# syzhang092218-source/dgppo

Hardware: AMD Instinct MI355X
Metric: env-steps/sec whole node, LidarSpread n=8 4096 envs, 1/2/4/8 GPUs (higher is better)
Workload: dtype f32

## Files before the change

dgppo_amd/csrc/gae.hip:

```cpp
#include "common.h"

__device__ inline float nanmax(float a, float b) { return (a != a || b != b) ? __builtin_nanf("") : fmaxf(a, b); }

struct GaeArgs {
  const float* costs; const float* rewards; const float* Vh; const float* Vl;
  const float* lam_pow;
  float* Qh; float* Ql;
  int B, T, AH;
  int n, nh;
  float gamma, one_minus_gamma, one_minus_lam;
};

__global__ void gae_kernel(GaeArgs a) {
  extern __shared__ float sm[];
  const int b = blockIdx.x, tid = threadIdx.x, nt = blockDim.x;
  const int T = a.T, AH = a.AH, n = a.n, nh = a.nh;
  float* rowH = sm;
  float* rowL = rowH + (T + 1) * AH;
  float* hcur = rowL + (T + 1);
  float* hdis = hcur + AH;
  const float* costs = a.costs + (size_t)b * T * AH;
  const float* Vh = a.Vh + (size_t)b * (T + 1) * AH;
  const float* Vl = a.Vl + (size_t)b * (T + 1);
  const float* rew = a.rewards + (size_t)b * T;
  for (int i = tid; i < (T + 1) * AH; i += nt) rowH[i] = 0.0f;
  for (int i = tid; i < T + 1; i += nt) rowL[i] = 0.0f;
  __syncthreads();
  for (int i = tid; i < AH; i += nt) rowH[i] = Vh[(size_t)T * AH + i];
  if (tid == 0) rowL[0] = Vl[T];
  __syncthreads();
  for (int ii = 0; ii < T; ++ii) {
    const int t = T - 1 - ii;
    for (int i = tid; i < AH; i += nt) hcur[i] = costs[(size_t)t * AH + i];
    __syncthreads();
    for (int ag = tid; ag < n; ag += nt) {
      float m = hcur[ag * nh];
      for (int h = 1; h < nh; ++h) m = nanmax(m, hcur[ag * nh + h]);
      for (int h = 0; h < nh; ++h) hdis[ag * nh + h] = a.one_minus_gamma * m;
    }
    __syncthreads();
    const float l = -rew[t];
    for (int idx = tid; idx < (ii + 1) * AH; idx += nt) {
      const int c = idx % AH;
      rowH[idx] = nanmax(hcur[c], hdis[c] + a.gamma * rowH[idx]);
    }
    for (int j = tid; j <= ii; j += nt) rowL[j] = l + a.gamma * rowL[j];
    __syncthreads();
    for (int c = tid; c < AH + 1; c += nt) {
      float acc = 0.0f;
      if (c < AH) {
        for (int j = 0; j <= ii; ++j) {
          const float cj = (j == 0) ? a.lam_pow[ii] : a.lam_pow[ii - j] * a.one_minus_lam;
          acc = fmaf(cj, rowH[j * AH + c], acc);
        }
        a.Qh[((size_t)b * T + t) * AH + c] = acc;
      } else {
        for (int j = 0; j <= ii; ++j) {
          const float cj = (j == 0) ? a.lam_pow[ii] : a.lam_pow[ii - j] * a.one_minus_lam;
          acc = fmaf(cj, rowL[j], acc);
        }
        a.Ql[(size_t)b * T + t] = acc;
      }
    }
    __syncthreads();
    for (int i = tid; i < AH; i += nt) rowH[(ii + 1) * AH + i] = Vh[(size_t)t * AH + i];
    if (tid == 0) rowL[ii + 1] = Vl[t];
    __syncthreads();
  }
}


__device__ inline float gae_row16_sum(float v) {
  v += __int_as_float(__builtin_amdgcn_update_dpp(0, __float_as_int(v), 0xB1, 0xf, 0xf, false));
  v += __int_as_float(__builtin_amdgcn_update_dpp(0, __float_as_int(v), 0x4E, 0xf, 0xf, false));
  v += __int_as_float(__builtin_amdgcn_update_dpp(0, __float_as_int(v), 0x141, 0xf, 0xf, false));
  v += __int_as_float(__builtin_amdgcn_update_dpp(0, __float_as_int(v), 0x140, 0xf, 0xf, false));
  return v;
}

template <int AHP>
__global__ void __launch_bounds__(256) gae_rows_kernel(GaeArgs a) {
  extern __shared__ float sm[];
  const int b = blockIdx.x, tid = threadIdx.x, lane = tid & 63;
  const int T = a.T, AH = a.AH, nh = a.nh;
  float* s_cost = sm;
  float* s_Vh = s_cost + T * AH;
  float* s_Vl = s_Vh + (T + 1) * AH;
  float* s_rew = s_Vl + (T + 1);
  float* s_part = s_rew + T;
  const float* costs = a.costs + (size_t)b * T * AH;
  const float* Vh = a.Vh + (size_t)b * (T + 1) * AH;
  for (int i = tid; i < T * AH; i += 256) s_cost[i] = costs[i];
  for (int i = tid; i < (T + 1) * AH; i += 256) s_Vh[i] = Vh[i];
  for (int i = tid; i < T + 1; i += 256) s_Vl[i] = a.Vl[(size_t)b * (T + 1) + i];
  for (int i = tid; i < T; i += 256) s_rew[i] = a.rewards[(size_t)b * T + i];
  __syncthreads();
  const int j = tid;
  float row[AHP];
  float rowl = 0.0f;
#pragma unroll
  for (int c = 0; c < AHP; ++c) row[c] = (j == 0 && c < AH) ? s_Vh[T * AH + c] : 0.0f;
  if (j == 0) rowl = s_Vl[T];
  for (int ii = 0; ii < T; ++ii) {
    const int t = T - 1 - ii;
    const bool act = j <= ii;
    float contrib[AHP];
    float cl = 0.0f;
    const float cj = (j == 0) ? a.lam_pow[ii] : ((j <= ii) ? a.lam_pow[ii - j] * a.one_minus_lam : 0.0f);
    if (act) {
      const float l = -s_rew[t];
      rowl = l + a.gamma * rowl;
      cl = cj * rowl;
    }
#pragma unroll
    for (int ag = 0; ag < AHP; ag += 1) {
      if (ag < AH) {
        const int agent = ag / nh;
        float m = s_cost[t * AH + agent * nh];
        for (int h = 1; h < nh; ++h) m = nanmax(m, s_cost[t * AH + agent * nh + h]);
        if (act) row[ag] = nanmax(s_cost[t * AH + ag], a.one_minus_gamma * m + a.gamma * row[ag]);
        contrib[ag] = act ? cj * row[ag] : 0.0f;
      } else {
        contrib[ag] = 0.0f;
      }
    }
#pragma unroll
    for (int c = 0; c < AHP; ++c) contrib[c] = gae_row16_sum(contrib[c]);
    cl = gae_row16_sum(cl);
    float* part = s_part + (ii & 1) * 16 * (AHP + 1);
    if ((lane & 15) == 0) {
      float* dst = part + (tid >> 4) * (AHP + 1);
#pragma unroll
      for (int c = 0; c < AHP; ++c) dst[c] = contrib[c];
      dst[AHP] = cl;
    }
    if (j == ii + 1) {
#pragma unroll
      for (int c = 0; c < AHP; ++c) row[c] = (c < AH) ? s_Vh[t * AH + c] : 0.0f;
      rowl = s_Vl[t];
    }
    __syncthreads();
    if (tid <= AH) {
      const int c = (tid < AH) ? tid : AHP;
      float q = 0.0f;
#pragma unroll
      for (int rw = 0; rw < 16; ++rw) q += part[rw * (AHP + 1) + c];
      if (tid < AH) a.Qh[((size_t)b * T + t) * AH + tid] = q;
      else a.Ql[(size_t)b * T + t] = q;
    }
  }
}

template <int NRG> __device__ inline float rg_sum(float v) {
  v += __int_as_float(__builtin_amdgcn_update_dpp(0, __float_as_int(v), 0xB1, 0xf, 0xf, false));
  v += __int_as_float(__builtin_amdgcn_update_dpp(0, __float_as_int(v), 0x4E, 0xf, 0xf, false));
  if (NRG == 8) v += __int_as_float(__builtin_amdgcn_update_dpp(0, __float_as_int(v), 0x141, 0xf, 0xf, false));
  return v;
}

template <int RPG, int NRG>
__global__ void __launch_bounds__(256) gae_cols_kernel(GaeArgs a) {
  const int T = a.T, AH = a.AH, nh = a.nh, C = AH + 1;
  const int rg = threadIdx.x % NRG;
  const long item = (long)blockIdx.x * (256 / NRG) + threadIdx.x / NRG;
  const bool valid = item < (long)a.B * C;
  const long it = valid ? item : 0;
  const int b = (int)(it / C), col = (int)(it - (long)b * C);
  const bool is_l = (col == AH);
  const int agent = is_l ? 0 : col / nh;
  const float* costs = a.costs + (size_t)b * T * AH + agent * nh;
  const float* vser = is_l ? a.Vl + (size_t)b * (T + 1) : a.Vh + (size_t)b * (T + 1) * AH + col;
  const int vstr = is_l ? 1 : AH;
  const float* rew = a.rewards + (size_t)b * T;
  const float lam = a.lam_pow[1], inv_lam = 1.0f / lam;
  float w[RPG];
  {
    float p = a.one_minus_lam;
#pragma unroll
    for (int r = 0; r < RPG; ++r) { w[r] = p; p *= inv_lam; }
    if (rg == 0) w[0] = 1.0f;
  }
  float row[RPG];
#pragma unroll
  for (int r = 0; r < RPG; ++r) row[r] = 0.0f;
  const float vT = vser[(size_t)T * vstr];
  if (rg == 0) row[0] = vT;
  float f = 1.0f;
  auto fetch = [&](int t, float& lo, float& k, float& vt) {
    vt = vser[(size_t)t * vstr];
    if (is_l) { lo = -INFINITY; k = -rew[t]; }
    else {
      const float* ct = costs + (size_t)t * AH;
      float m = ct[0];
      for (int h = 1; h < nh; ++h) m = nanmax(m, ct[h]);
      lo = ct[col - agent * nh];
      k = a.one_minus_gamma * m;
    }
  };
  float lo, k, vt;
  fetch(T - 1, lo, k, vt);
  bool poison = vT != vT;
  const int nchunk = (T + RPG - 1) / RPG;
  for (int chunk = 0; chunk < nchunk; ++chunk) {
    const bool g_le = rg <= chunk, g_lt = rg < chunk;
#pragma unroll
    for (int s = 0; s < RPG; ++s) {
      const int ii = chunk * RPG + s;
      if (ii < T) {
        const int t = T - 1 - ii;
        float lo_n = 0.0f, k_n = 0.0f, vt_n = 0.0f;
        if (t > 0) fetch(t - 1, lo_n, k_n, vt_n);
        float q = 0.0f;
#pragma unroll
        for (int r = 0; r < RPG; ++r) {
          const bool act = (r <= s) ? g_le : g_lt;
          const float nv = fmaxf(lo, fmaf(a.gamma, row[r], k));
          row[r] = act ? nv : row[r];
          q = fmaf(w[r], row[r], q);
        }
        poison = poison || (lo != lo) || (k != k);
        float tot = rg_sum<NRG>(q * f);
        tot = poison ? __builtin_nanf("") : tot;
        if (valid && rg == 0) {
          if (is_l) a.Ql[(size_t)b * T + t] = tot;
          else a.Qh[((size_t)b * T + t) * AH + col] = tot;
        }
        poison = poison || (vt != vt);
        if (g_le) f *= lam;
        const int rn = (s + 1) % RPG;
        const bool mine = rg == chunk + ((s + 1) / RPG);
#pragma unroll
        for (int r = 0; r < RPG; ++r)
          if (r == rn) row[r] = mine ? vt : row[r];
        lo = lo_n; k = k_n; vt = vt_n;
      }
    }
  }
}

template <int RPG, int NRG>
static void launch_gae_cols(const GaeArgs& a, hipStream_t st) {
  const long items = (long)a.B * (a.AH + 1);
  const int per_block = 256 / NRG;
  hipLaunchKernelGGL((gae_cols_kernel<RPG, NRG>), dim3((unsigned)((items + per_block - 1) / per_block)), dim3(256), 0, st, a);
}

extern "C" int32_t dgppo_gae(const float* costs, const float* rewards, const float* Vh, const float* Vl,
                             const float* lam_pow, float gamma, float one_minus_gamma, float one_minus_lam, float* Qh,
                             float* Ql, int32_t B, int32_t T, int32_t n, int32_t nh, void* stream) {
  DGPPO_REQUIRE(B >= 0 && T >= 1 && n >= 1 && nh >= 1, "gae: bad sizes");
  if (B == 0) return 0;
  DGPPO_REQUIRE(costs && rewards && Vh && Vl && lam_pow && Qh && Ql, "gae: NULL operand");
  GaeArgs a{costs, rewards, Vh, Vl, lam_pow, Qh, Ql, B, T, n * nh, n, nh, gamma, one_minus_gamma, one_minus_lam};
  if (T <= 256 && one_minus_lam <= 0.5f && one_minus_lam >= 0.0f) {
    hipStream_t st = (hipStream_t)stream;
    if (T <= 32) launch_gae_cols<8, 4>(a, st);
    else if (T <= 64) launch_gae_cols<16, 4>(a, st);
    else if (T <= 128) launch_gae_cols<32, 4>(a, st);
    else launch_gae_cols<32, 8>(a, st);
    DGPPO_LAUNCH_CHECK();
    return 0;
  }
  if (T + 1 <= 256 && a.AH <= 32) {
    const int ahp = a.AH <= 8 ? 8 : (a.AH <= 16 ? 16 : 32);
    const size_t fsm = sizeof(float) * ((size_t)T * a.AH + (size_t)(T + 1) * a.AH + (T + 1) + T + 2 * 16 * (ahp + 1));
    if (fsm <= 64 * 1024) {
      hipStream_t st = (hipStream_t)stream;
      if (ahp == 8) hipLaunchKernelGGL(gae_rows_kernel<8>, dim3(B), dim3(256), fsm, st, a);
      else if (ahp == 16) hipLaunchKernelGGL(gae_rows_kernel<16>, dim3(B), dim3(256), fsm, st, a);
      else hipLaunchKernelGGL(gae_rows_kernel<32>, dim3(B), dim3(256), fsm, st, a);
      DGPPO_LAUNCH_CHECK();
      return 0;
    }
  }
  const size_t smem = sizeof(float) * ((size_t)(T + 1) * a.AH + (T + 1) + 2 * a.AH);
  DGPPO_REQUIRE(smem <= 150 * 1024, "gae: T*n*nh too large for LDS (%zu B)", smem);
  if (smem > 64 * 1024)
    (void)hipFuncSetAttribute((const void*)gae_kernel, hipFuncAttributeMaxDynamicSharedMemorySize, (int)smem);
  hipLaunchKernelGGL(gae_kernel, dim3(B), dim3(256), smem, (hipStream_t)stream, a);
  DGPPO_LAUNCH_CHECK();
  return 0;
}

struct AdvArgs {
  const float* Ql; const float* Vl; const float* Vh;
  float* adv;
  float* stats;
  int B, T, n, nh;
  float inv_dt, alpha, cbf_eps, cbf_weight;
};

__global__ void adv_kernel(AdvArgs a) {
  __shared__ float red[256];
  __shared__ float s_mean, s_std;
  const int b = blockIdx.x, tid = threadIdx.x, nt = blockDim.x;
  const int T = a.T, n = a.n, nh = a.nh;
  const float* Ql = a.Ql + (size_t)b * T;
  const float* Vl = a.Vl + (size_t)b * (T + 1);
  const float* Vh = a.Vh ? a.Vh + (size_t)b * (T + 1) * n * nh : nullptr;
  float acc = 0.0f;
  for (int t = tid; t < T; t += nt) acc += Ql[t] - Vl[t];
  red[tid] = acc;
  __syncthreads();
  for (int o = nt / 2; o > 0; o >>= 1) { if (tid < o) red[tid] += red[tid + o]; __syncthreads(); }
  if (tid == 0) s_mean = red[0] / (float)T;
  __syncthreads();
  const float mean = s_mean;
  acc = 0.0f;
  for (int t = tid; t < T; t += nt) { const float d = (Ql[t] - Vl[t]) - mean; acc += d * d; }
  red[tid] = acc;
  __syncthreads();
  for (int o = nt / 2; o > 0; o >>= 1) { if (tid < o) red[tid] += red[tid + o]; __syncthreads(); }
  if (tid == 0) s_std = sqrtf(red[0] / (float)T);
  __syncthreads();
  const float denom = s_std + 1e-8f;
  float nsafe = 0.0f;
  for (int idx = tid; idx < T * n; idx += nt) {
    const int t = idx / n, ag = idx - t * n;
    const float al = ((Ql[t] - Vl[t]) - mean) / denom;
    bool safe = true;
    float amax = 0.0f;
    for (int h = 0; a.Vh != nullptr && h < nh; ++h) {
      const float v0 = Vh[((size_t)t * n + ag) * nh + h], v1 = Vh[((size_t)(t + 1) * n + ag) * nh + h];
      const float deriv = (v1 - v0) * a.inv_dt + a.alpha * v0;
      const float ac = nanmax(deriv + a.cbf_eps, 0.0f);
      amax = (h == 0) ? ac : nanmax(amax, ac);
      safe = safe && (deriv <= 0.0f);
    }
    const float A = (safe ? al : 0.0f) + amax * a.cbf_weight;
    a.adv[(size_t)b * T * n + idx] = -A;
    nsafe += safe ? 1.0f : 0.0f;
  }
  red[tid] = nsafe;
  __syncthreads();
  for (int o = nt / 2; o > 0; o >>= 1) { if (tid < o) red[tid] += red[tid + o]; __syncthreads(); }
  if (tid == 0) atomicAdd(a.stats, red[0]);
}

extern "C" int32_t dgppo_advantage(const float* Ql, const float* Vl, const float* Vh, float dt, float alpha,
                                   float cbf_eps, float cbf_weight, float* adv, float* stats, int32_t B, int32_t T,
                                   int32_t n, int32_t nh, void* stream) {
  DGPPO_REQUIRE(B >= 0 && T >= 1 && n >= 1 && nh >= 1, "advantage: bad sizes");
  if (B == 0) return 0;
  DGPPO_REQUIRE(Ql && Vl && adv && stats, "advantage: NULL operand");
  AdvArgs a{Ql, Vl, Vh, adv, stats, B, T, n, nh, 1.0f / dt, alpha, cbf_eps, cbf_weight};
  hipLaunchKernelGGL(adv_kernel, dim3(B), dim3(256), 0, (hipStream_t)stream, a);
  DGPPO_LAUNCH_CHECK();
  return 0;
}

__global__ void shaped_reward_kernel(const float* __restrict__ reward, const float* __restrict__ cost, float w,
                                     float* __restrict__ out, long rows, int n, int nh) {
  const long r = (long)blockIdx.x * blockDim.x + threadIdx.x;
  if (r >= rows) return;
  const float* c = cost + r * n * nh;
  float tot = 0.0f;
  for (int i = 0; i < n; ++i) {
    float si = 0.0f;
    for (int h = 0; h < nh; ++h) si += nanmax(c[i * nh + h], 0.0f);
    tot += si;
  }
  out[r] = reward[r] - w * tot;
}

extern "C" int32_t dgppo_shaped_reward(const float* reward, const float* cost, float cost_weight, float* out, int64_t rows,
                                       int32_t n, int32_t nh, void* stream) {
  DGPPO_REQUIRE(rows >= 0 && n >= 1 && nh >= 1, "shaped_reward: bad sizes");
  if (rows == 0) return 0;
  DGPPO_REQUIRE(reward && cost && out, "shaped_reward: NULL operand");
  hipLaunchKernelGGL(shaped_reward_kernel, dim3((unsigned)((rows + 255) / 256)), dim3(256), 0, (hipStream_t)stream, reward,
                     cost, cost_weight, out, (long)rows, n, nh);
  DGPPO_LAUNCH_CHECK();
  return 0;
}

struct AdvLagrArgs {
  const float* Ql; const float* Vl; const float* Qh; const float* Vh; const float* lagr;
  float* adv;
  float* Ah;
  int B, T, n, nh;
};

#define ADV_LAGR_MAX_COLS 192
__global__ void __launch_bounds__(256) adv_lagr_kernel(AdvLagrArgs a) {
  __shared__ float red[256];
  __shared__ float s_mean[1 + ADV_LAGR_MAX_COLS], s_den[1 + ADV_LAGR_MAX_COLS];
  const int b = blockIdx.x, tid = threadIdx.x, nt = blockDim.x;
  const int T = a.T, n = a.n, nh = a.nh, AH = n * nh;
  const float* Ql = a.Ql + (size_t)b * T;
  const float* Vl = a.Vl + (size_t)b * (T + 1);
  const float* Qh = a.Qh + (size_t)b * T * AH;
  const float* Vh = a.Vh + (size_t)b * (T + 1) * AH;
  for (int s0 = 0; s0 < 1 + AH; ++s0) {
    float acc = 0.0f;
    for (int t = tid; t < T; t += nt) acc += (s0 == 0) ? (Ql[t] - Vl[t]) : (Qh[(size_t)t * AH + s0 - 1] - Vh[(size_t)t * AH + s0 - 1]);
    red[tid] = acc;
    __syncthreads();
    for (int o = nt / 2; o > 0; o >>= 1) { if (tid < o) red[tid] += red[tid + o]; __syncthreads(); }
    const float mean = red[0] / (float)T;
    __syncthreads();
    acc = 0.0f;
    for (int t = tid; t < T; t += nt) {
      const float d = ((s0 == 0) ? (Ql[t] - Vl[t]) : (Qh[(size_t)t * AH + s0 - 1] - Vh[(size_t)t * AH + s0 - 1])) - mean;
      acc += d * d;
    }
    red[tid] = acc;
    __syncthreads();
    for (int o = nt / 2; o > 0; o >>= 1) { if (tid < o) red[tid] += red[tid + o]; __syncthreads(); }
    if (tid == 0) { s_mean[s0] = mean; s_den[s0] = sqrtf(red[0] / (float)T) + 1e-8f; }
    __syncthreads();
  }
  for (int idx = tid; idx < T * n; idx += nt) {
    const int t = idx / n, ag = idx - t * n;
    const float al = -(((Ql[t] - Vl[t]) - s_mean[0]) / s_den[0]);
    float acc = 0.0f;
    for (int h = 0; h < nh; ++h) {
      const int c = ag * nh + h;
      const float ah = ((Qh[(size_t)t * AH + c] - Vh[(size_t)t * AH + c]) - s_mean[1 + c]) / s_den[1 + c];
      a.Ah[((size_t)b * T + t) * AH + c] = ah;
      acc += ah * a.lagr[c];
    }
    a.adv[(size_t)b * T * n + idx] = al - acc / (float)nh;
  }
}

extern "C" int32_t dgppo_advantage_lagr(const float* Ql, const float* Vl, const float* Qh, const float* Vh,
                                        const float* lagr, float* adv, float* Ah, int32_t B, int32_t T, int32_t n,
                                        int32_t nh, void* stream) {
  DGPPO_REQUIRE(B >= 0 && T >= 1 && n >= 1 && nh >= 1 && (long)n * nh <= ADV_LAGR_MAX_COLS,
                "advantage_lagr: bad sizes (n * nh <= 192)");
  if (B == 0) return 0;
  DGPPO_REQUIRE(Ql && Vl && Qh && Vh && lagr && adv && Ah, "advantage_lagr: NULL operand");
  AdvLagrArgs a{Ql, Vl, Qh, Vh, lagr, adv, Ah, B, T, n, nh};
  hipLaunchKernelGGL(adv_lagr_kernel, dim3(B), dim3(256), 0, (hipStream_t)stream, a);
  DGPPO_LAUNCH_CHECK();
  return 0;
}

__global__ void __launch_bounds__(256) lagr_sum_kernel(const float* __restrict__ lp_new, const float* __restrict__ lp_old,
                                                       const float* __restrict__ Vh, const float* __restrict__ Ah,
                                                       float* __restrict__ sums, long rows, int n, int nh, int T,
                                                       long vh_env_stride, float one_minus_gamma) {
  extern __shared__ float s_acc[];
  for (int c = threadIdx.x; c < n * nh; c += blockDim.x) s_acc[c] = 0.0f;
  __syncthreads();
  for (long r = (long)blockIdx.x * blockDim.x + threadIdx.x; r < rows; r += (long)gridDim.x * blockDim.x) {
    const int ag = (int)(r % n);
    const long bt = r / n, e = bt / T, t = bt - e * T;
    const float ratio = expf(lp_new[r] - lp_old[r]);
    for (int h = 0; h < nh; ++h) {
      const float vh = Vh[e * vh_env_stride + (t * n + ag) * nh + h];
      atomicAdd(&s_acc[ag * nh + h], vh * one_minus_gamma + ratio * Ah[r * nh + h]);
    }
  }
  __syncthreads();
  for (int c = threadIdx.x; c < n * nh; c += blockDim.x) atomicAdd(&sums[c], s_acc[c]);
}

__global__ void lagr_apply_kernel(float* __restrict__ lagr, float* __restrict__ sums, int count, float inv_bt, float lr) {
  const int c = blockIdx.x * blockDim.x + threadIdx.x;
  if (c >= count) return;
  const float delta = -(sums[c] * inv_bt);
  lagr[c] = fmaxf(lagr[c] - delta * lr, 0.0f);
  sums[c] = 0.0f;
}

extern "C" int32_t dgppo_lagr_update(const float* lp_new, const float* lp_old, const float* Vh, int64_t vh_env_stride,
                                     const float* Ah, float* lagr, float* sums, int32_t n_env, int32_t T, int32_t n,
                                     int32_t nh, float one_minus_gamma, float lr, void* stream) {
  DGPPO_REQUIRE(n_env >= 1 && T >= 1 && n >= 1 && nh >= 1 && n * nh <= 1024, "lagr_update: bad sizes");
  DGPPO_REQUIRE(lp_new && lp_old && Vh && Ah && lagr && sums, "lagr_update: NULL operand");
  const long rows = (long)n_env * T * n;
  const int grid = (int)((rows + 255) / 256 < 512 ? (rows + 255) / 256 : 512);
  hipLaunchKernelGGL(lagr_sum_kernel, dim3(grid), dim3(256), sizeof(float) * n * nh, (hipStream_t)stream, lp_new, lp_old, Vh,
                     Ah, sums, rows, n, nh, T, (long)vh_env_stride, one_minus_gamma);
  hipLaunchKernelGGL(lagr_apply_kernel, dim3((n * nh + 63) / 64), dim3(64), 0, (hipStream_t)stream, lagr, sums, n * nh,
                     1.0f / (float)((long)n_env * T), lr);
  DGPPO_LAUNCH_CHECK();
  return 0;
}

extern "C" int32_t dgppo_lagr_sums(const float* lp_new, const float* lp_old, const float* Vh, int64_t vh_env_stride,
                                   const float* Ah, float* sums, int32_t n_env, int32_t T, int32_t n, int32_t nh,
                                   float one_minus_gamma, void* stream) {
  DGPPO_REQUIRE(n_env >= 1 && T >= 1 && n >= 1 && nh >= 1 && n * nh <= 1024, "lagr_sums: bad sizes");
  DGPPO_REQUIRE(lp_new && lp_old && Vh && Ah && sums, "lagr_sums: NULL operand");
  const long rows = (long)n_env * T * n;
  const int grid = (int)((rows + 255) / 256 < 512 ? (rows + 255) / 256 : 512);
  hipLaunchKernelGGL(lagr_sum_kernel, dim3(grid), dim3(256), sizeof(float) * n * nh, (hipStream_t)stream, lp_new, lp_old, Vh,
                     Ah, sums, rows, n, nh, T, (long)vh_env_stride, one_minus_gamma);
  DGPPO_LAUNCH_CHECK();
  return 0;
}

extern "C" int32_t dgppo_lagr_apply(float* lagr, float* sums, int32_t count, int64_t rows_total, float lr, void* stream) {
  DGPPO_REQUIRE(count >= 1 && count <= 1024 && rows_total >= 1, "lagr_apply: bad sizes");
  DGPPO_REQUIRE(lagr && sums, "lagr_apply: NULL operand");
  hipLaunchKernelGGL(lagr_apply_kernel, dim3((count + 63) / 64), dim3(64), 0, (hipStream_t)stream, lagr, sums, count,
                     1.0f / (float)rows_total, lr);
  DGPPO_LAUNCH_CHECK();
  return 0;
}

__global__ void relu_fwd_kernel(const float* __restrict__ x, float* __restrict__ out, long count) {
  const long i = (long)blockIdx.x * blockDim.x + threadIdx.x;
  if (i < count) out[i] = nanmax(x[i], 0.0f);
}

extern "C" int32_t dgppo_relu_fwd(const float* x, float* out, int64_t count, void* stream) {
  DGPPO_REQUIRE(count >= 0, "relu_fwd: count < 0");
  if (count == 0) return 0;
  DGPPO_REQUIRE(x && out, "relu_fwd: NULL operand");
  hipLaunchKernelGGL(relu_fwd_kernel, dim3((unsigned)((count + 255) / 256)), dim3(256), 0, (hipStream_t)stream, x, out,
                     (long)count);
  DGPPO_LAUNCH_CHECK();
  return 0;
}
```

dgppo_amd/csrc/graph_feats.hip:

```cpp
#include "graph_topo.h"

struct FeatArgs {
  dgppo_env_cfg cfg;
  Topo t;
  const float* agent; long agent_se, agent_st;
  const float* goal;
  const float* obst;
  const float* hits; long hits_se, hits_st;
  const int32_t* env_ids;
  int n_env, n_time;
  float* Xa;
  float* Xo;
  float* efeat;
  float* emask;
  int Fp;
  int vecX, vecM;
  uint32_t rcp_fp, rcp_fq, rcp_S;
};

#define GF_PF 8
#define GF_WAVE_SYNC()                                  \
  do {                                                  \
    __builtin_amdgcn_fence(__ATOMIC_SEQ_CST, "wavefront"); \
    __builtin_amdgcn_wave_barrier();                    \
  } while (0)

struct FeatRec { const float *ag, *go, *ob; };

template <int SD>
__device__ inline float4 feat4(const float* s) {
  if constexpr (SD == 5) {
    float vx = __fmul_rn(s[4], s[2]), vy = __fmul_rn(s[4], s[3]);
    asm volatile("" : "+v"(vx), "+v"(vy));
    return make_float4(s[0], s[1], vx, vy);
  } else {
    return make_float4(s[0], s[1], s[2], s[3]);
  }
}

template <int SD>
__global__ void __launch_bounds__(256) graph_feats_kernel(FeatArgs a) {
  extern __shared__ float sm[];
  const dgppo_env_cfg& c = a.cfg;
  const Topo& t = a.t;
  const int lane = threadIdx.x & 63;
  const int wv = __builtin_amdgcn_readfirstlane(threadIdx.x >> 6), wpb = blockDim.x >> 6;
  const int n = t.n, ng = t.ng, S = t.S, Fp = a.Fp;
  const int n_on = t.Ns - n - ng;
  const int nA = n * SD, nG = ng * SD, nO = n_on * (t.lidar ? 2 : SD), R = nA + nG + nO;
  float* s_ag = sm + (size_t)wv * R;
  float* s_go = s_ag + nA;
  float* s_ob = s_go + nG;
  const long G = (long)a.n_env * a.n_time, stride = (long)gridDim.x * wpb;
  long g = (long)blockIdx.x * wpb + wv;
  if (g >= G) return;
  auto env_of = [&](long gg) { const int e = (int)gg / a.n_time; return a.env_ids ? (int)a.env_ids[e] : e; };
  auto locate = [&](long gg, int env) {
    const int tt = (int)gg % a.n_time;
    FeatRec p;
    p.ag = a.agent + (size_t)env * a.agent_se + (size_t)tt * a.agent_st;
    p.go = a.goal + (size_t)env * nG;
    p.ob = nullptr;
    if (nO > 0) p.ob = t.lidar ? a.hits + (size_t)env * a.hits_se + (size_t)tt * a.hits_st : a.obst + (size_t)env * nO;
    return p;
  };
  auto fetch = [&](const FeatRec& p, int i) { return i < nA ? p.ag[i] : (i < nA + nG ? p.go[i - nA] : p.ob[i - nA - nG]); };
  float r0, r1, r2, r3, r4, r5, r6, r7;
  static_assert(GF_PF == 8, "one register per prefetched dword");
#define GF_EACH(OP) OP(r0, 0) OP(r1, 1) OP(r2, 2) OP(r3, 3) OP(r4, 4) OP(r5, 5) OP(r6, 6) OP(r7, 7)
#define GF_REQUEST(r, j) { const int i = lane + 64 * j; r = 0.0f; if (i < R) r = fetch(p, i); }
#define GF_COMMIT(r, j)  { const int i = lane + 64 * j; if (i < R) s_ag[i] = r; }
  FeatRec p = locate(g, env_of(g));
  GF_EACH(GF_REQUEST)
  long gn = g + stride;
  int env_n = gn < G ? env_of(gn) : 0;
  for (;;) {
    GF_EACH(GF_COMMIT)
    for (int i = GF_PF * 64 + lane; i < R; i += 64) s_ag[i] = fetch(p, i);
    GF_WAVE_SYNC();
    const bool more = gn < G;
    if (more) {
      p = locate(gn, env_n);
      GF_EACH(GF_REQUEST)
      if (gn + stride < G) env_n = env_of(gn + stride);
    }
    auto node_src = [&](int nd, const float*& src, int& ns, int& one) {
      if (nd < n) { src = s_ag + nd * SD; ns = SD; one = SD + 2; }
      else if (nd < n + ng) { src = s_go + (nd - n) * SD; ns = SD; one = SD + 1; }
      else if (t.lidar) { src = s_ob + (nd - n - ng) * 2; ns = 2; one = SD; }
      else { src = s_ob + (nd - n - ng) * SD; ns = SD; one = SD; }
    };
    if (a.vecX) {
      const int Fq = Fp >> 2;
      for (int q = lane; q < t.Ns * Fq; q += 64) {
        const int nd = (int)__umulhi((uint32_t)q, a.rcp_fq), col0 = (q - nd * Fq) * 4;
        const float* src; int ns, one;
        node_src(nd, src, ns, one);
        float v[4];
#pragma unroll
        for (int k = 0; k < 4; ++k) {
          const int col = col0 + k;
          v[k] = (col < ns) ? src[col] : ((col == one) ? 1.0f : 0.0f);
        }
        float* dst = (nd < n) ? a.Xa + ((size_t)g * n + nd) * Fp + col0 : a.Xo + ((size_t)g * (t.Ns - n) + (nd - n)) * Fp + col0;
        *reinterpret_cast<float4*>(dst) = make_float4(v[0], v[1], v[2], v[3]);
      }
    } else {
      for (int idx = lane; idx < t.Ns * Fp; idx += 64) {
        const int nd = (int)__umulhi((uint32_t)idx, a.rcp_fp), col = idx - nd * Fp;
        const float* src; int ns, one;
        node_src(nd, src, ns, one);
        const float v = (col < ns) ? src[col] : ((col == one) ? 1.0f : 0.0f);
        if (nd < n) a.Xa[((size_t)g * n + nd) * Fp + col] = v;
        else a.Xo[((size_t)g * (t.Ns - n) + (nd - n)) * Fp + col] = v;
      }
    }
    const int nE = n * S;
    for (int base = 0; base < nE; base += 64) {
      const int idx = base + lane;
      bool mask = false;
      if (idx < nE) {
        const int i = (int)__umulhi((uint32_t)idx, a.rcp_S), s = idx - i * S;
        float4 f;
        const float4 fi = feat4<SD>(s_ag + i * SD);
        const float px = s_ag[i * SD], py = s_ag[i * SD + 1];
        if (s < n) {
          const float4 fj = feat4<SD>(s_ag + s * SD);
          f = make_float4(__fsub_rn(fi.x, fj.x), __fsub_rn(fi.y, fj.y), __fsub_rn(fi.z, fj.z), __fsub_rn(fi.w, fj.w));
          float d = __fadd_rn(dist_rn(__fsub_rn(px, s_ag[s * SD]), __fsub_rn(py, s_ag[s * SD + 1])), (i == s) ? c.eye_offset : 0.0f);
          mask = d < c.comm_radius;
        } else if (s < n + t.gs) {
          const int gi = t.spread ? (s - n) : i;
          const float4 fg = feat4<SD>(s_go + gi * SD);
          f = make_float4(__fsub_rn(fi.x, fg.x), __fsub_rn(fi.y, fg.y), __fsub_rn(fi.z, fg.z), __fsub_rn(fi.w, fg.w));
          mask = true;
        } else {
          const int m = s - n - t.gs;
          if (t.lidar) {
            const float* hp = s_ob + (i * t.per + m) * 2;
            const float lx = __fsub_rn(px, hp[0]), ly = __fsub_rn(py, hp[1]);
            f = make_float4(lx, ly, 0.0f, 0.0f);
            mask = dist_rn(lx, ly) < c.lidar_mask_radius;
          } else {
            const float* xo = s_ob + m * SD;
            const float* xi = s_ag + i * SD;
            f = make_float4(__fsub_rn(xi[0], xo[0]), __fsub_rn(xi[1], xo[1]), __fsub_rn(xi[2], xo[2]), __fsub_rn(xi[3], xo[3]));
            mask = dist_rn(__fsub_rn(xi[0], xo[0]), __fsub_rn(xi[1], xo[1])) < c.obs_mask_radius;
          }
        }
        reinterpret_cast<float4*>(a.efeat)[(size_t)g * nE + idx] = f;
        if (!a.vecM) a.emask[(size_t)g * nE + idx] = mask ? 1.0f : 0.0f;
      }
      if (a.vecM) {
        const unsigned long long bits = __ballot(mask);
        const int i4 = base + 4 * lane;
        if (lane < 16 && i4 < nE) {
          const unsigned b = (unsigned)(bits >> (4 * lane));
          *reinterpret_cast<float4*>(a.emask + (size_t)g * nE + i4) =
              make_float4((b & 1u) ? 1.0f : 0.0f, (b & 2u) ? 1.0f : 0.0f, (b & 4u) ? 1.0f : 0.0f, (b & 8u) ? 1.0f : 0.0f);
        }
      }
    }
    GF_WAVE_SYNC();
    if (!more) break;
    g = gn;
    gn += stride;
  }
#undef GF_EACH
#undef GF_REQUEST
#undef GF_COMMIT
}

static int feats_grid_cap(const void* fn, int wpb, size_t smem) {
  static thread_local const void* k_fn = nullptr;
  static thread_local int k_wpb = 0, k_cap = 0;
  static thread_local size_t k_smem = 0;
  if (fn == k_fn && wpb == k_wpb && smem == k_smem) return k_cap;
  int per_cu = 0, dev = 0, cus = 256;
  if (hipOccupancyMaxActiveBlocksPerMultiprocessor(&per_cu, fn, 64 * wpb, smem) != hipSuccess || per_cu < 1) per_cu = 1;
  if (hipGetDevice(&dev) != hipSuccess ||
      hipDeviceGetAttribute(&cus, hipDeviceAttributeMultiprocessorCount, dev) != hipSuccess || cus < 1) cus = 256;
  k_fn = fn; k_wpb = wpb; k_smem = smem; k_cap = per_cu * cus;
  return k_cap;
}

extern "C" int32_t dgppo_graph_feats(const dgppo_env_cfg* cfg, const float* agent, int64_t agent_se, int64_t agent_st,
                                     const float* goal, const float* obst, const float* hits, int64_t hits_se,
                                     int64_t hits_st, const int32_t* env_ids, int32_t n_env, int32_t n_time, float* Xa,
                                     float* Xo, float* efeat, float* emask, int32_t Fp, void* stream) {
  int32_t rc = dgppo_validate_cfg(cfg);
  if (rc) return rc;
  DGPPO_REFUSE_VMAS(cfg, "dgppo_graph_feats", "dgppo_vmas_graph_feats");
  DGPPO_REQUIRE(n_env >= 0 && n_time >= 0, "graph_feats: negative counts");
  if (n_env == 0 || n_time == 0) return 0;
  DGPPO_REQUIRE(agent && goal && Xa && efeat && emask, "graph_feats: NULL operand");
  DGPPO_REQUIRE(Fp >= cfg->node_dim && Fp <= 32, "graph_feats: Fp must be in [node_dim, 32]");
  FeatArgs a;
  a.cfg = *cfg; a.t = make_topo(*cfg);
  const int n_on = a.t.Ns - a.t.n - a.t.ng;
  DGPPO_REQUIRE(n_on == 0 || Xo, "graph_feats: Xo is NULL");
  DGPPO_REQUIRE(a.t.Ns == a.t.n || Xo, "graph_feats: Xo is NULL");
  if (n_on > 0) {
    if (a.t.lidar) DGPPO_REQUIRE(hits, "graph_feats: hits is NULL");
    else DGPPO_REQUIRE(obst, "graph_feats: obst is NULL");
  }
  DGPPO_REQUIRE(((uintptr_t)efeat & 15) == 0, "graph_feats: efeat must be 16-byte aligned");
  a.agent = agent; a.agent_se = agent_se; a.agent_st = agent_st; a.goal = goal; a.obst = obst;
  a.hits = hits; a.hits_se = hits_se; a.hits_st = hits_st; a.env_ids = env_ids; a.n_env = n_env; a.n_time = n_time;
  a.Xa = Xa; a.Xo = Xo; a.efeat = efeat; a.emask = emask; a.Fp = Fp;
  a.rcp_fp = (uint32_t)((0x100000000ull + (uint64_t)Fp - 1) / (uint64_t)Fp);
  a.rcp_S = (uint32_t)((0x100000000ull + (uint64_t)a.t.S - 1) / (uint64_t)a.t.S);
  DGPPO_REQUIRE(Fp >= 2 && a.t.S >= 2 && (long)a.t.Ns * Fp < 65536 && (long)a.t.n * a.t.S < 65536, "graph_feats: sizes out of range");
  a.vecX = (Fp % 4 == 0 && ((uintptr_t)Xa & 15) == 0 && ((uintptr_t)Xo & 15) == 0) ? 1 : 0;
  a.vecM = ((a.t.n * a.t.S) % 4 == 0 && ((uintptr_t)emask & 15) == 0) ? 1 : 0;
  a.rcp_fq = a.vecX ? (uint32_t)((0x100000000ull + (uint64_t)(Fp / 4) - 1) / (uint64_t)(Fp / 4)) : 0u;
  const int SD = cfg->state_dim;
  const size_t rec = sizeof(float) * ((size_t)a.t.n * SD + (size_t)a.t.ng * SD + (size_t)n_on * (a.t.lidar ? 2 : SD));
  int wpb = 4;
  while (wpb > 1 && rec * wpb > 65536) wpb >>= 1;
  const long G = (long)n_env * n_time;
  const void* fn = SD == 5 ? reinterpret_cast<const void*>(&graph_feats_kernel<5>) : reinterpret_cast<const void*>(&graph_feats_kernel<4>);
  const int cap = feats_grid_cap(fn, wpb, rec * wpb);
  const long wgs = (G + wpb - 1) / wpb;
  const dim3 grid((unsigned)(wgs < cap ? wgs : cap)), block(64 * wpb);
  if (SD == 5) hipLaunchKernelGGL(graph_feats_kernel<5>, grid, block, rec * wpb, (hipStream_t)stream, a);
  else hipLaunchKernelGGL(graph_feats_kernel<4>, grid, block, rec * wpb, (hipStream_t)stream, a);
  DGPPO_LAUNCH_CHECK();
  return 0;
}
```

dgppo_amd/engine.py:

```python
from __future__ import annotations

import dataclasses
from typing import Callable, Dict, Optional

import numpy as np
import os
import torch

from . import _native as N
from . import nets
from . import ops_algo as OA
from . import ops_env as OE
from . import ops_nn as K
from .utils import checkpoint as CK


@dataclasses.dataclass
class Hyper:
    gamma: float = 0.99
    gae_lambda: float = 0.95
    clip_eps: float = 0.25
    coef_ent: float = 1e-2
    max_grad_norm: float = 2.0
    lr_actor: float = 3e-4
    lr_Vl: float = 1e-3
    lr_Vh: float = 1e-3
    batch_size: int = 16384
    rnn_step: int = 16
    alpha: float = 10.0
    cbf_eps: float = 1e-2
    cbf_weight: float = 1.0
    cbf_schedule: bool = True
    train_steps: int = 100000
    actor_gnn_layers: int = 2
    Vl_gnn_layers: int = 2
    Vh_gnn_layers: int = 1
    use_rnn: bool = True
    use_lstm: bool = False
    rnn_layers: int = 1
    lagr_init: float = 0.78
    lr_lagr: float = 1e-7
    cost_weight: float = 0.0
    cost_schedule: bool = False


class RolloutData:

    def __init__(self, cfg: N.EnvCfg, B: int, T: int, device, stochastic: bool, carry_dim: int = nets.HID):
        n = cfg.n_agents
        self.cfg, self.B, self.T, self.stochastic = cfg, B, T, stochastic
        z = lambda *s: torch.empty(*s, device=device)
        step, env = OE.record_fields(cfg)
        self.step_tm = {k: z(T + 1, B, *shape) for k, shape in step.items()}
        self.env = {k: z(B, *shape) for k, shape in env.items()}
        self.step: Dict[str, torch.Tensor] = {}
        for k in OE.STEP_FIELDS:
            setattr(self, k + "_tm", self.step_tm.get(k))
            setattr(self, k, None)
        for k in OE.ENV_FIELDS:
            setattr(self, k, self.env.get(k))
        self.action_tm = z(T, B, n, 2)
        self.log_pi_tm = z(T, B, n) if stochastic else None
        self.rnn_tm = z(T + 1, B, n, carry_dim)
        self.reward_tm = z(T, B)
        self.cost_tm = z(T, B, n, cfg.n_cost)
        self._env_major = False
        views = {k: v.unbind(0) for k, v in self.step_tm.items()}
        self.states_tm = [OE.State({k: v[t] for k, v in views.items()}, self.env) for t in range(T + 1)]

    def finalize(self):
        if self._env_major:
            return self

        def tr(name, x):
            if x is None:
                return None
            cur = getattr(self, name, None)
            want = (x.shape[1], x.shape[0]) + tuple(x.shape[2:])
            if cur is None or tuple(cur.shape) != want:
                cur = torch.empty(want, device=x.device, dtype=x.dtype)
            cur.copy_(x.transpose(0, 1))
            return cur
        for k, v in self.step_tm.items():
            self.step[k] = tr(k, v)
            setattr(self, k, self.step[k])
        self.actions = tr("actions", self.action_tm)
        self.log_pis = tr("log_pis", self.log_pi_tm) if self.stochastic else None
        T, x = self.T, self.rnn_tm
        want = (x.shape[1], T + 2) + tuple(x.shape[2:])
        cur = getattr(self, "_rnn_em", None)
        if cur is None or tuple(cur.shape) != want:
            cur = torch.empty(want, device=x.device, dtype=x.dtype)
        cur[:, :T + 1].copy_(x.transpose(0, 1))
        self._rnn_em = cur
        self.rnn_states = self._rnn_em[:, :T] if self.stochastic else self._rnn_em[:, 1:T + 1]
        self.rewards = tr("rewards", self.reward_tm)
        self.costs = tr("costs", self.cost_tm)
        self._env_major = True
        return self


class OptState:
    def __init__(self, n: int, device):
        self.m = torch.zeros(n, device=device)
        self.v = torch.zeros(n, device=device)
        self.state = torch.zeros(N.OPT_STATE_FLOATS, device=device)


class Engine:
    def __init__(self, cfg: N.EnvCfg, hyper: Hyper, device, T: int = 128,
                 allreduce: Optional[Callable[[torch.Tensor], None]] = None, world: int = 1, prepass_graphs: int = 1 << 20,
                 use_graphs: bool = False, multi_stream: bool = False, algo: str = "dgppo", rank: int = 0,
                 fused_step: bool = True, lean_attn0: bool = True):
        self.cfg, self.hp, self.device, self.T = cfg, hyper, device, T
        assert algo in ("dgppo", "informarl", "hcbfcrpo", "informarl_lagr"), algo
        self.algo = algo
        self.use_graphs = use_graphs and os.environ.get("DGPPO_HIPGRAPH", "1") != "0"
        self.multi_stream = multi_stream and os.environ.get("DGPPO_MULTI_STREAM", "1") != "0"
        self._side_streams = None
        self.fused_step = bool(fused_step) and OE.act_step_feats_supported(cfg, nets.input_width(cfg), nets.H_HEADS)
        self.lean_attn0 = bool(lean_attn0)
        self._ro_cache: Dict[tuple, dict] = {}
        self._upd_graph: dict = {}
        self.n_cost = cfg.n_cost
        spec = [("policy", "policy", hyper.actor_gnn_layers, 2), ("Vl", "Vl", hyper.Vl_gnn_layers, 1)]
        if algo == "dgppo":
            spec.append(("Vh", "Vh", hyper.Vh_gnn_layers, self.n_cost))
        elif algo == "informarl_lagr":
            spec.append(("Vh", "Vhg", hyper.Vh_gnn_layers, self.n_cost))
        def rnn_kw(name):
            if not hyper.use_rnn:
                return dict(rnn="none", rnn_layers=0)
            if name == "Vh" and algo == "dgppo":
                return dict(rnn="gru", rnn_layers=1)
            return dict(rnn="lstm" if hyper.use_lstm else "gru", rnn_layers=hyper.rnn_layers)
        sizes = [nets.make_layout(kind, cfg.node_dim, layers, n_out, **rnn_kw(k)).size for k, kind, layers, n_out in spec]
        offs, tot = [], 0
        for sz in sizes:
            offs.append(tot)
            tot += (sz + 3) // 4 * 4
        self.flat_grads = torch.zeros(tot + 4 * 8, device=device)
        self.n_reduced = tot + 3 * 8
        self.stats = self.flat_grads[tot:tot + 32].view(4, 8)
        built = {k: nets.Net(kind, cfg, layers, n_out, device, grads=self.flat_grads[o:o + sz], lean_attn0=self.lean_attn0, **rnn_kw(k))
                 for (k, kind, layers, n_out), o, sz in zip(spec, offs, sizes)}
        if algo == "informarl_lagr":
            self.lagr = torch.full((cfg.n_agents, self.n_cost), float(hyper.lagr_init), device=device)
            self.lagr_sums = torch.zeros(cfg.n_agents * self.n_cost, device=device)
        self.policy, self.Vl, self.Vh = built["policy"], built["Vl"], built.get("Vh")
        self.HC = self.policy.carry_dim
        self.opt = {k: OptState(net.layout.size, device) for k, net in self.nets.items()}
        self.arena = nets.Arena(device)
        self.allreduce = allreduce
        self.world, self.rank = int(world), int(rank)
        assert self.world >= 1 and (allreduce is not None or self.world == 1), "world > 1 needs an allreduce"
        assert 0 <= self.rank < self.world, f"rank {rank} outside world {world}"
        self.prepass_graphs = int(os.environ.get("DGPPO_PREPASS_GRAPHS", prepass_graphs))
        self.lam_pow = OA.lam_pow_table(hyper.gae_lambda, T, device)
        self.eps_hat = torch.zeros(cfg.n_agents, 2, device=device)
        self.reset_failed = torch.zeros(1, dtype=torch.int32, device=device)
        self.grad_hook: Optional[Callable[[str, nets.Net, int], None]] = None
        self._mb = 0

    @property
    def nets(self) -> Dict[str, nets.Net]:
        d = {"policy": self.policy, "Vl": self.Vl}
        if self.Vh is not None:
            d["Vh"] = self.Vh
        return d

    def set_entropy_noise(self, seed: int):
        OE.randn(seed, 0, self.eps_hat.view(-1))

    _CFG_IDENTITY = ("kind", "n_agents", "n_obs", "n_rays", "top_k", "node_dim", "n_cost")

    def _identity(self) -> dict:
        ident = {"algo": CK.encode_str(self.algo)}
        ident.update({f"cfg.{k}": int(getattr(self.cfg, k)) for k in self._CFG_IDENTITY})
        for f in dataclasses.fields(Hyper):
            v = getattr(self.hp, f.name)
            ident[f"hyper.{f.name}"] = int(v) if isinstance(v, (bool, int)) else float(v)
        ident["T"], ident["world"] = int(self.T), int(self.world)
        ident.update({f"size.{k}": int(net.layout.size) for k, net in self.nets.items()})
        return ident

    def _state_tensors(self) -> Dict[str, torch.Tensor]:
        t = {}
        for k, net in self.nets.items():
            opt = self.opt[k]
            t.update({f"{k}/params": net.params, f"{k}/m": opt.m, f"{k}/v": opt.v, f"{k}/state": opt.state})
        t["eps_hat"] = self.eps_hat
        if self.algo == "informarl_lagr":
            t["lagr"] = self.lagr
        return t

    def state_dict(self) -> dict:
        out = {"identity": self._identity()}
        for path, x in self._state_tensors().items():
            node = out
            *dirs, leaf = path.split("/")
            for d in dirs:
                node = node.setdefault(d, {})
            node[leaf] = x.detach().cpu().numpy().copy()
        return out

    def load_state_dict(self, d: dict) -> None:
        mine, theirs = self._identity(), d.get("identity", {})
        show = lambda v: repr(CK.decode_str(v)) if isinstance(v, np.ndarray) else repr(v)
        for k, v in mine.items():
            if k not in theirs:
                raise ValueError(f"state dict does not fit this engine: it has no identity field '{k}'")
            if not np.array_equal(np.asarray(v), np.asarray(theirs[k])):
                raise ValueError(f"state dict does not fit this engine: '{k}' is {show(theirs[k])} there, {show(v)} here")
        src = {}
        for path, x in self._state_tensors().items():
            node = d
            for part in path.split("/"):
                node = node.get(part) if isinstance(node, dict) else None
            if not isinstance(node, np.ndarray) or node.dtype != np.float32 or node.shape != tuple(x.shape):
                raise ValueError(f"state dict does not fit this engine: '{path}' is not a float32 array of shape {tuple(x.shape)}")
            src[path] = node
        for path, x in self._state_tensors().items():
            x.copy_(torch.from_numpy(src[path]).to(self.device))
        for net in self.nets.values():
            net.prepare()

    def _feats(self, tag, st: OE.State, n_env, n_time=1, slots=1, env_ids=None):
        f = nets.GraphFeats(self.cfg, n_env * n_time, self.arena, tag)
        return f.compute_record(st.step, slots, st.env, env_ids, n_env, n_time)

    def _rollout_steps(self, ro: RolloutData, eps, B: int, stochastic: bool, start: int = 0):
        cfg, T, n = self.cfg, ro.T, self.cfg.n_agents
        tag = "ro" if stochastic else "rod"
        if self.fused_step:
            pol, R = self.policy, B * n
            feats = self._feats(tag, ro.states_tm[start], B)
            Mcat, cvec = pol.pp("gnn0.Mcat"), pol.pp("gnn0.cvec")
            qt0 = pol.arena.get(f"{tag}.qt0", R, Mcat.shape[1])
            K.dense_fwd(feats.Xa, Mcat, cvec, qt0)
            for t in range(start, T):
                act = pol.forward(feats, n_seq=R, T=1, h0=ro.rnn_tm[t].view(R, self.HC), tag=tag,
                                  hs_out=ro.rnn_tm[t + 1].view(R, self.HC), train=False, qt0=qt0)
                nxt = dict(Xa=feats.Xa, Xo=feats.Xo, efeat=feats.efeat, emask=feats.emask, Fp=feats.Fp, Mcat=Mcat, cvec=cvec,
                           qt0=qt0, H=nets.H_HEADS) if t + 1 < T else {}
                OE.act_step_feats(cfg, ro.states_tm[t], act["ms"], eps[t] if stochastic else None, ro.action_tm[t],
                                  ro.log_pi_tm[t] if stochastic else None, ro.states_tm[t + 1], ro.reward_tm[t], ro.cost_tm[t],
                                  **nxt)
                feats.edges_from_rows = cfg.state_dim == 4
            return
        for t in range(start, T):
            feats = self._feats(tag, ro.states_tm[t], B)
            act = self.policy.forward(feats, n_seq=B * n, T=1, h0=ro.rnn_tm[t].view(B * n, self.HC), tag=tag,
                                      hs_out=ro.rnn_tm[t + 1].view(B * n, self.HC), train=False)
            a_t = ro.action_tm[t].view(B * n, 2)
            if stochastic:
                K.policy_head(act["ms"], eps[t], None, a_t, ro.log_pi_tm[t].view(B * n), None, n, 0)
            else:
                K.policy_head(act["ms"], None, None, a_t, None, None, n, 1)
            OE.step(cfg, ro.states_tm[t], ro.action_tm[t], ro.states_tm[t + 1], ro.reward_tm[t], ro.cost_tm[t])

    def rollout(self, seeds: torch.Tensor, stochastic: bool, noise_seed: int = 0) -> RolloutData:
        cfg, T = self.cfg, self.T
        B = int(seeds.shape[0])
        n = cfg.n_agents
        slot = None
        if self.use_graphs:
            slot = self._ro_cache.setdefault((B, stochastic), {"ro": None, "graph": None, "gen": -1, "calls": 0})
            if slot["ro"] is None:
                slot["ro"] = RolloutData(cfg, B, T, self.device, stochastic, self.HC)
            ro = slot["ro"]
            ro._env_major = False
        else:
            ro = RolloutData(cfg, B, T, self.device, stochastic, self.HC)
        OE.reset(cfg, seeds, ro.states_tm[0], self.reset_failed)
        ro.rnn_tm[0].zero_()
        eps = None
        if stochastic:
            eps = self.arena.get("ro.eps", T, B * n, 2)
            OE.randn_rows(noise_seed, eps.view(T, B * n * 2), self.world * B * n * 2, self.rank * B * n * 2)
        if slot is None:
            self._rollout_steps(ro, eps, B, stochastic)
            return ro
        slot["calls"] += 1
        if slot["graph"] is not None and slot["gen"] != self._arena_generation():
            slot["graph"] = None
        if slot["graph"] is not None:
            slot["graph"].replay()
            K.FLOPS[0] += slot.get("flops", 0.0)
            return ro
        f0 = K.FLOPS[0]
        self._rollout_steps(ro, eps, B, stochastic)
        slot["flops"] = K.FLOPS[0] - f0
        if not slot.get("failed", False):
            graph = torch.cuda.CUDAGraph()
            try:
                f1 = K.FLOPS[0]
                with torch.cuda.graph(graph, capture_error_mode="thread_local"):
                    self._rollout_steps(ro, eps, B, stochastic)
                K.FLOPS[0] = f1 + slot["flops"]
                slot["graph"], slot["gen"] = graph, self._arena_generation()
                graph.replay()
            except Exception as ex:
                slot["failed"] = True
                torch.cuda.synchronize()
                print(f"[dgppo_amd] HIP-graph capture of the rollout loop failed ({type(ex).__name__}: {ex}); "
                      f"continuing with eager launches", flush=True)
        return ro

    def _update_generation(self) -> int:
        return self.arena.generation + sum(net.arena.generation + net.ws_arena.generation for net in self.nets.values())

    def _arena_generation(self) -> int:
        return self.arena.generation + self.policy.arena.generation

    def rollout_pair(self, seeds: torch.Tensor, det_seeds: torch.Tensor, noise_seed: int = 0):
        if not (self.multi_stream and self.device.type == "cuda"):
            return self.rollout(seeds, True, noise_seed), self.rollout(det_seeds, False)
        main = torch.cuda.current_stream(self.device)
        s0, s1 = self._net_streams()[:2]
        out = [None, None]
        for k, (st, sd, stoch) in enumerate(((s0, seeds, True), (s1, det_seeds, False))):
            st.wait_stream(main)
            with torch.cuda.stream(st):
                out[k] = self.rollout(sd, stoch, noise_seed if stoch else 0)
        main.wait_stream(s0)
        main.wait_stream(s1)
        return out[0], out[1]

    def _block_feats(self, tag, ro: RolloutData, e0, Eb, t0, n_time, env_ids=None):
        envs = slice(e0, None) if env_ids is None else slice(None)
        st = OE.State({k: v[envs, t0] for k, v in ro.step.items()}, {k: v[envs] for k, v in ro.env.items()})
        return self._feats(tag, st, Eb, n_time, self.T + 1, env_ids)

    def _vh_carry(self, ro: RolloutData, e0: int, Eb: int) -> torch.Tensor:
        return ro.rnn_states[e0:e0 + Eb][..., :nets.HID]

    def _final_carry(self, ro: RolloutData, e0: int, Eb: int) -> torch.Tensor:
        T, n, HC = self.T, self.cfg.n_agents, self.HC
        fin = self._block_feats("fin", ro, e0, Eb, T, 1)
        h_last = self.arena.get("pre.hlast", Eb * n, HC)
        h_last.view(Eb, n, HC).copy_(ro.rnn_states[e0:e0 + Eb, T - 1])
        hstar = self.arena.get("pre.hstar", Eb * n, HC)
        self.policy.forward(fin, n_seq=Eb * n, T=1, h0=h_last, tag="fin", hs_out=hstar, train=False)
        return hstar

    def values_prepass(self, ro: RolloutData, want_Vl: bool, want_Vh: bool = True):
        cfg, T, B = self.cfg, self.T, ro.B
        n, nh, H = cfg.n_agents, self.n_cost, nets.HID
        kind = "ro" if ro.stochastic else "det"
        Vl_buf = self.arena.get(f"tg.Vl.{kind}", B, T + 1) if want_Vl else None
        Vh_buf = self.arena.get(f"tg.Vh.{kind}", B, T + 1, n, nh) if want_Vh else None
        block = max(1, min(B, self.prepass_graphs // (T + 1)))
        for e0 in range(0, B, block):
            Eb = min(block, B - e0)
            feats = self._block_feats("pre", ro, e0, Eb, 0, T + 1)
            if want_Vl:
                act = self.Vl.forward(feats, n_seq=Eb, T=T + 1, h0=None, tag="pre", train=False)
                Vl_buf[e0:e0 + Eb].copy_(act["v"].view(Eb, T + 1))
            if not want_Vh:
                continue
            HC = self.HC
            hstar = self._final_carry(ro, e0, Eb)
            if not self.hp.use_rnn:
                h0 = None
            elif HC == H:
                s0 = 0 if ro.stochastic else 1
                ro._rnn_em[e0:e0 + Eb, s0 + T].copy_(hstar.view(Eb, n, H))
                h0 = K.H0Blocks(ro._rnn_em[e0, s0], (T + 1) * n, (T + 2) * n * H, Eb)
            else:
                h0_all = self.arena.get("pre.h0all", Eb, T + 1, n, H)
                h0_all[:, :T].copy_(self._vh_carry(ro, e0, Eb))
                h0_all[:, T].copy_(hstar.view(Eb, n, HC)[..., :H])
                h0 = h0_all.view(-1, H)
            act = self.Vh.forward(feats, n_seq=Eb * (T + 1) * n, T=1, h0=h0, tag="pre", train=False)
            Vh_buf[e0:e0 + Eb].copy_(act["v"].view(Eb, T + 1, n, nh))
        return Vl_buf, Vh_buf

    def require_landscape(self, what: str = "vh_landscape"):
        if self.algo != "dgppo":
            why = {"informarl_lagr": "its constraint-value net carries its own scan state, which needs a sequence pass first"}
            raise ValueError(f"{what}: algo '{self.algo}' is not supported: "
                             + why.get(self.algo, "it has no constraint-value network"))
        if self.cfg.is_vmas:
            raise ValueError(f"{what}: VMASReverseTransport is not supported")

    def vh_landscape(self, ro: RolloutData, env_index: int, agent_id: int, frame_ids, xs, ys,
                     events: Optional[list] = None) -> torch.Tensor:
        self.require_landscape()
        cfg, T = self.cfg, self.T
        n, nh, H = cfg.n_agents, self.n_cost, nets.HID
        ro.finalize()
        if not 0 <= int(env_index) < ro.B:
            raise ValueError(f"vh_landscape: env_index {env_index} outside [0, {ro.B})")
        if not 0 <= int(agent_id) < n:
            raise ValueError(f"vh_landscape: agent_id {agent_id} outside [0, {n})")
        frames = np.asarray(frame_ids, dtype=np.int64).reshape(-1)
        if frames.size == 0 or frames.min() < 0 or frames.max() >= T:
            raise ValueError(f"vh_landscape: frame_ids must be a non-empty subset of [0, {T})")
        xs, ys = K.sweep_axis(xs, "xs", self.device), K.sweep_axis(ys, "ys", self.device)
        nx, ny, F = int(xs.numel()), int(ys.numel()), int(frames.size)
        e = int(env_index)
        step = {k: v[e] for k, v in ro.step.items()}
        env = {k: v[e] for k, v in ro.env.items()}
        rc, rs = OE._rays(cfg, self.device)
        carry = self._vh_carry(ro, e, 1)[0] if self.hp.use_rnn else None
        out = torch.empty(F, ny, nx, n, nh, device=self.device)
        ids_dev = torch.from_numpy(frames.astype(np.int32)).to(self.device)
        cap = max(1, self.prepass_graphs)
        fb = max(1, cap // (ny * nx))
        yb = ny if cap >= ny * nx else max(1, cap // nx)
        xb = nx if cap >= nx else cap
        for f0 in range(0, F, fb):
            f1 = min(F, f0 + fb)
            fr = frames[f0:f1]
            for y0 in range(0, ny, yb):
                y1 = min(ny, y0 + yb)
                for x0 in range(0, nx, xb):
                    x1 = min(nx, x0 + xb)
                    P = (y1 - y0) * (x1 - x0)
                    Gb = (f1 - f0) * P
                    feats = nets.GraphFeats(cfg, Gb, self.arena, "land")
                    ev = [torch.cuda.Event(enable_timing=True) for _ in range(3)] if events is not None else None
                    if ev:
                        ev[0].record()
                    feats.compute_sweep(step, env, ids_dev[f0:f1], f1 - f0, agent_id, xs[x0:x1], ys[y0:y1], rc, rs,
                                        frame_max=int(fr.max()))
                    if ev:
                        ev[1].record()
                    h0 = None
                    if carry is not None:
                        h0 = self.arena.get("land.h0", Gb * n, H)
                        for j, t in enumerate(fr):
                            h0.view(f1 - f0, P, n, H)[j].copy_(carry[int(t)].unsqueeze(0).expand(P, n, H))
                    act = self.Vh.forward(feats, n_seq=Gb * n, T=1, h0=h0, tag="land", train=False)
                    out[f0:f1, y0:y1, x0:x1].copy_(act["v"].view(f1 - f0, y1 - y0, x1 - x0, n, nh))
                    if ev:
                        ev[2].record()
                        events.append(tuple(ev))
        return out

    def cost_landscape(self, ro: RolloutData, env_index: int, agent_id: int, frame_ids, xs, ys) -> torch.Tensor:
        cfg, T = self.cfg, self.T
        if cfg.is_vmas:
            raise ValueError("cost_landscape: VMASReverseTransport is not supported")
        n = cfg.n_agents
        ro.finalize()
        if not 0 <= int(env_index) < ro.B:
            raise ValueError(f"cost_landscape: env_index {env_index} outside [0, {ro.B})")
        if not 0 <= int(agent_id) < n:
            raise ValueError(f"cost_landscape: agent_id {agent_id} outside [0, {n})")
        frames = np.asarray(frame_ids, dtype=np.int64).reshape(-1)
        if frames.size == 0 or frames.min() < 0 or frames.max() >= T:
            raise ValueError(f"cost_landscape: frame_ids must be a non-empty subset of [0, {T})")
        xs, ys = K.sweep_axis(xs, "xs", self.device), K.sweep_axis(ys, "ys", self.device)
        nx, ny, F = int(xs.numel()), int(ys.numel()), int(frames.size)
        e = int(env_index)
        step = {k: v[e] for k, v in ro.step.items()}
        env = {k: v[e] for k, v in ro.env.items()}
        rc, rs = OE._rays(cfg, self.device)
        out = torch.empty(F, ny, nx, n, self.n_cost, device=self.device)
        K.cost_sweep(cfg, step["agent"], n * cfg.state_dim, env.get("obst"), step.get("hits"), n * cfg.top_k * 2, rc, rs,
                     frames, F, int(agent_id), xs, ys, out.view(F * ny * nx, n, self.n_cost))
        return out

    def rollout_landscape(self, ro: RolloutData, env_index: int, agent_id: int, frame_ids, xs, ys, horizon: int,
                          events: Optional[list] = None, records: Optional[list] = None):
        cfg, T = self.cfg, self.T
        if cfg.is_vmas:
            raise ValueError("rollout_landscape: VMASReverseTransport is not supported")
        n, nh, HC = cfg.n_agents, self.n_cost, self.HC
        ro.finalize()
        if not 0 <= int(env_index) < ro.B:
            raise ValueError(f"rollout_landscape: env_index {env_index} outside [0, {ro.B})")
        if not 0 <= int(agent_id) < n:
            raise ValueError(f"rollout_landscape: agent_id {agent_id} outside [0, {n})")
        frames = np.asarray(frame_ids, dtype=np.int64).reshape(-1)
        if frames.size == 0 or frames.min() < 0 or frames.max() >= T:
            raise ValueError(f"rollout_landscape: frame_ids must be a non-empty subset of [0, {T})")
        horizon = int(horizon)
        if horizon < 1:
            raise ValueError(f"rollout_landscape: horizon must be >= 1 (got {horizon})")
        xs, ys = K.sweep_axis(xs, "xs", self.device), K.sweep_axis(ys, "ys", self.device)
        nx, ny, F = int(xs.numel()), int(ys.numel()), int(frames.size)
        e = int(env_index)
        step = {k: v[e] for k, v in ro.step.items()}
        env = {k: v[e] for k, v in ro.env.items()}
        carry = ro._rnn_em[e] if self.hp.use_rnn else None
        value = torch.empty(F, ny, nx, n, nh, device=self.device)
        worst = torch.empty(F, ny, nx, n, nh, device=self.device)
        ids_dev = torch.from_numpy(frames.astype(np.int32)).to(self.device)
        cap = max(1, self.prepass_graphs // (horizon + 1))
        fb = max(1, cap // (ny * nx))
        yb = ny if cap >= ny * nx else max(1, cap // nx)
        xb = nx if cap >= nx else cap
        recs: Dict[int, RolloutData] = {}
        for f0 in range(0, F, fb):
            f1 = min(F, f0 + fb)
            fr = frames[f0:f1]
            for y0 in range(0, ny, yb):
                y1 = min(ny, y0 + yb)
                for x0 in range(0, nx, xb):
                    x1 = min(nx, x0 + xb)
                    Gb = (f1 - f0) * (y1 - y0) * (x1 - x0)
                    rec = recs.get(Gb) if records is None else None
                    if rec is None:
                        rec = recs[Gb] = RolloutData(cfg, Gb, horizon, self.device, False, HC)
                    rec._env_major = False
                    ev = [torch.cuda.Event(enable_timing=True) for _ in range(4)] if events is not None else None
                    if ev:
                        ev[0].record()
                    if carry is None:
                        rec.rnn_tm[0].zero_()
                    OE.sweep_fork(cfg, step, env, ids_dev[f0:f1], f1 - f0, int(agent_id), xs[x0:x1], ys[y0:y1], rec.states_tm[0],
                                  carry, n * HC, rec.rnn_tm[0].view(Gb * n, HC) if carry is not None else None,
                                  frame_max=int(fr.max()))
                    if ev:
                        ev[1].record()
                    self._rollout_steps(rec, None, Gb, False)
                    if ev:
                        ev[2].record()
                    val = self.arena.get("rl.value", Gb, n, nh)
                    wor = self.arena.get("rl.worst", Gb, n, nh)
                    OA.constraint_return(rec.cost_tm, self.hp.gamma, val, wor)
                    value[f0:f1, y0:y1, x0:x1].copy_(val.view(f1 - f0, y1 - y0, x1 - x0, n, nh))
                    worst[f0:f1, y0:y1, x0:x1].copy_(wor.view(f1 - f0, y1 - y0, x1 - x0, n, nh))
                    if ev:
                        ev[3].record()
                        events.append(tuple(ev))
                    if records is not None:
                        records.append((f0, f1, y0, y1, x0, x1, rec.finalize()))
        return value, worst

    def action_landscape(self, ro: RolloutData, env_index: int, agent_id: int, frame_ids, us, vs,
                         events: Optional[list] = None):
        self.require_landscape("action_landscape")
        cfg, T = self.cfg, self.T
        n, nh, H = cfg.n_agents, self.n_cost, nets.HID
        ro.finalize()
        if not 0 <= int(env_index) < ro.B:
            raise ValueError(f"action_landscape: env_index {env_index} outside [0, {ro.B})")
        if not 0 <= int(agent_id) < n:
            raise ValueError(f"action_landscape: agent_id {agent_id} outside [0, {n})")
        frames = np.asarray(frame_ids, dtype=np.int64).reshape(-1)
        if frames.size == 0 or frames.min() < 0 or frames.max() >= T:
            raise ValueError(f"action_landscape: frame_ids must be a non-empty subset of [0, {T})")
        us, vs = K.sweep_axis(us, "us", self.device), K.sweep_axis(vs, "vs", self.device)
        nu, nv, F = int(us.numel()), int(vs.numel()), int(frames.size)
        e = int(env_index)
        ids_dev = torch.from_numpy(frames.astype(np.int32)).to(self.device)
        _, Vh_all = self.values_prepass(ro, want_Vl=False)
        Vh = Vh_all[e].index_select(0, ids_dev.long())
        carry = None
        if self.hp.use_rnn:
            carry = torch.empty(T, n, H, device=self.device)
            carry[:T - 1].copy_(self._vh_carry(ro, e, 1)[0, 1:])
            if int(frames.max()) == T - 1:
                carry[T - 1].copy_(self._final_carry(ro, e, 1).view(n, self.HC)[:, :H])
        step = {k: v[e] for k, v in ro.step.items()}
        env = {k: v[e] for k, v in ro.env.items()}
        Vh_next = torch.empty(F, nv, nu, n, nh, device=self.device)
        cap = max(1, self.prepass_graphs)
        fb = max(1, cap // (nv * nu))
        vb = nv if cap >= nv * nu else max(1, cap // nu)
        ub = nu if cap >= nu else cap
        for f0 in range(0, F, fb):
            f1 = min(F, f0 + fb)
            fr = frames[f0:f1]
            for v0 in range(0, nv, vb):
                v1 = min(nv, v0 + vb)
                for u0 in range(0, nu, ub):
                    u1 = min(nu, u0 + ub)
                    P = (v1 - v0) * (u1 - u0)
                    Gb = (f1 - f0) * P
                    feats = nets.GraphFeats(cfg, Gb, self.arena, "act")
                    ev = [torch.cuda.Event(enable_timing=True) for _ in range(3)] if events is not None else None
                    if ev:
                        ev[0].record()
                    feats.compute_action_sweep(step, env, ids_dev[f0:f1], f1 - f0, agent_id, us[u0:u1], vs[v0:v1],
                                               frame_max=int(fr.max()))
                    if ev:
                        ev[1].record()
                    h0 = None
                    if carry is not None:
                        h0 = self.arena.get("act.h0", Gb * n, H)
                        for j, t in enumerate(fr):
                            h0.view(f1 - f0, P, n, H)[j].copy_(carry[int(t)].unsqueeze(0).expand(P, n, H))
                    act = self.Vh.forward(feats, n_seq=Gb * n, T=1, h0=h0, tag="act", train=False)
                    Vh_next[f0:f1, v0:v1, u0:u1].copy_(act["v"].view(f1 - f0, v1 - v0, u1 - u0, n, nh))
                    if ev:
                        ev[2].record()
                        events.append(tuple(ev))
        Vh_b = Vh.view(F, 1, 1, n, nh)
        cbf = (Vh_next - Vh_b) / float(cfg.dt) + float(self.hp.alpha) * Vh_b
        return cbf, Vh_next, Vh.clone()

    def action_rollout_landscape(self, ro: RolloutData, env_index: int, agent_id: int, frame_ids, us, vs, horizon: int,
                                 events: Optional[list] = None, records: Optional[list] = None):
        cfg, T = self.cfg, self.T
        if cfg.is_vmas:
            raise ValueError("action_rollout_landscape: VMASReverseTransport is not supported")
        n, nh, HC = cfg.n_agents, self.n_cost, self.HC
        ro.finalize()
        if not 0 <= int(env_index) < ro.B:
            raise ValueError(f"action_rollout_landscape: env_index {env_index} outside [0, {ro.B})")
        if not 0 <= int(agent_id) < n:
            raise ValueError(f"action_rollout_landscape: agent_id {agent_id} outside [0, {n})")
        frames = np.asarray(frame_ids, dtype=np.int64).reshape(-1)
        if frames.size == 0 or frames.min() < 0 or frames.max() >= T:
            raise ValueError(f"action_rollout_landscape: frame_ids must be a non-empty subset of [0, {T})")
        horizon = int(horizon)
        if horizon < 1:
            raise ValueError(f"action_rollout_landscape: horizon must be >= 1 (got {horizon})")
        us, vs = K.sweep_axis(us, "us", self.device), K.sweep_axis(vs, "vs", self.device)
        nu, nv, F = int(us.numel()), int(vs.numel()), int(frames.size)
        e = int(env_index)
        step = {k: v[e] for k, v in ro.step.items()}
        env = {k: v[e] for k, v in ro.env.items()}
        actions = ro.actions[e]
        carry = ro._rnn_em[e, 1:] if self.hp.use_rnn else None
        if carry is not None and int(frames.max()) == T - 1:
            ro._rnn_em[e, T].copy_(ro.rnn_tm[T, e])
        value = torch.empty(F, nv, nu, n, nh, device=self.device)
        worst = torch.empty(F, nv, nu, n, nh, device=self.device)
        ids_dev = torch.from_numpy(frames.astype(np.int32)).to(self.device)
        cap = max(1, self.prepass_graphs // (horizon + 2))
        fb = max(1, cap // (nv * nu))
        vb = nv if cap >= nv * nu else max(1, cap // nu)
        ub = nu if cap >= nu else cap
        recs: Dict[int, RolloutData] = {}
        for f0 in range(0, F, fb):
            f1 = min(F, f0 + fb)
            fr = frames[f0:f1]
            for v0 in range(0, nv, vb):
                v1 = min(nv, v0 + vb)
                for u0 in range(0, nu, ub):
                    u1 = min(nu, u0 + ub)
                    Gb = (f1 - f0) * (v1 - v0) * (u1 - u0)
                    rec = recs.get(Gb) if records is None else None
                    if rec is None:
                        rec = recs[Gb] = RolloutData(cfg, Gb, horizon + 1, self.device, False, HC)
                    ev = [torch.cuda.Event(enable_timing=True) for _ in range(4)] if events is not None else None
                    if ev:
                        ev[0].record()
                    if carry is None:
                        rec.rnn_tm[1].zero_()
                    OE.action_sweep_fork(cfg, step, env, actions, ids_dev[f0:f1], f1 - f0, int(agent_id), us[u0:u1], vs[v0:v1],
                                         rec.states_tm[0], rec.action_tm[0], carry, n * HC,
                                         rec.rnn_tm[1].view(Gb * n, HC) if carry is not None else None, frame_max=int(fr.max()))
                    OE.step(cfg, rec.states_tm[0], rec.action_tm[0], rec.states_tm[1], rec.reward_tm[0], rec.cost_tm[0])
                    if ev:
                        ev[1].record()
                    self._rollout_steps(rec, None, Gb, False, start=1)
                    if ev:
                        ev[2].record()
                    val = self.arena.get("arl.value", Gb, n, nh)
                    wor = self.arena.get("arl.worst", Gb, n, nh)
                    OA.constraint_return(rec.cost_tm[1:horizon + 1], self.hp.gamma, val, wor)
                    value[f0:f1, v0:v1, u0:u1].copy_(val.view(f1 - f0, v1 - v0, u1 - u0, n, nh))
                    worst[f0:f1, v0:v1, u0:u1].copy_(wor.view(f1 - f0, v1 - v0, u1 - u0, n, nh))
                    if ev:
                        ev[3].record()
                        events.append(tuple(ev))
                    if records is not None:
                        records.append((f0, f1, v0, v1, u0, u1, rec))
        return value, worst

    def rollout_shielded(self, seeds: torch.Tensor, us, vs, margin: float = 0.0, events: Optional[list] = None):
        self.require_landscape("rollout_shielded")
        cfg, T = self.cfg, self.T
        n, nh, H, HC = cfg.n_agents, self.n_cost, nets.HID, self.HC
        us, vs = K.sweep_axis(us, "us", self.device), K.sweep_axis(vs, "vs", self.device)
        margin = float(margin)
        if not np.isfinite(margin):
            raise ValueError("rollout_shielded: margin must be finite")
        nu, nv = int(us.numel()), int(vs.numel())
        P = 1 + nu * nv
        B = int(seeds.shape[0])
        dev = self.device
        ro = RolloutData(cfg, B, T, dev, False, HC)
        OE.reset(cfg, seeds, ro.states_tm[0], self.reset_failed)
        ro.rnn_tm[0].zero_()
        log = dict(policy_action=torch.empty(T, B, n, 2, device=dev), index=torch.empty(T, B, n, dtype=torch.int32, device=dev),
                   flag=torch.empty(T, B, n, dtype=torch.int32, device=dev), h=torch.empty(T, B, n, P, device=dev),
                   Vh=torch.empty(T, B, n, nh, device=dev))
        use_rnn = self.hp.use_rnn
        block = max(1, min(B, max(1, self.prepass_graphs) // (n * P)))
        dt, alpha = float(cfg.dt), float(self.hp.alpha)

        def mark(ev):
            if ev is not None:
                ev.append(torch.cuda.Event(enable_timing=True))
                ev[-1].record()
        for t in range(T):
            st, nst = ro.states_tm[t], ro.states_tm[t + 1]
            ev = [] if events is not None else None
            mark(ev)
            feats = self._feats("sh", st, B)
            h_next = ro.rnn_tm[t + 1].view(B * n, HC)
            act = self.policy.forward(feats, n_seq=B * n, T=1, h0=ro.rnn_tm[t].view(B * n, HC), tag="sh", hs_out=h_next,
                                      train=False)
            a_pol = log["policy_action"][t]
            K.policy_head(act["ms"], None, None, a_pol.view(B * n, 2), None, None, n, 1)
            h0 = None
            if use_rnn:
                h0 = h_next
                if HC != H:
                    h0 = self.arena.get("sh.h0", B * n, H)
                    h0.copy_(h_next[:, :H])
            v = self.Vh.forward(feats, n_seq=B * n, T=1, h0=h0, tag="sh", train=False)["v"]
            Vh_t = log["Vh"][t]
            Vh_t.copy_(v.view(B, n, nh))
            mark(ev)
            OE.step(cfg, st, a_pol, nst, ro.reward_tm[t], ro.cost_tm[t])
            cl0 = None
            if use_rnn:
                cprime = self.arena.get("sh.cprime", B * n, HC)
                self.policy.forward(self._feats("sh", nst, B), n_seq=B * n, T=1, h0=h_next, tag="sh", hs_out=cprime, train=False)
                cl0 = cprime.view(B, n, HC)[..., :H]
            mark(ev)
            for e0 in range(0, B, block):
                Eb = min(block, B - e0)
                sl = slice(e0, e0 + Eb)
                Gb = Eb * n * P
                cut = lambda s: OE.State({k: x[sl] for k, x in s.step.items()}, {k: x[sl] for k, x in s.env.items()})
                wf = nets.GraphFeats(cfg, Gb, self.arena, "shw").compute_team_action_sweep(cut(st), cut(nst), a_pol[sl], us, vs)
                mark(ev)
                hw = None
                if use_rnn:
                    hw = self.arena.get("shw.h0", Gb * n, H)
                    hw.view(Eb, n * P, n, H).copy_(cl0[sl].unsqueeze(1).expand(Eb, n * P, n, H))
                vn = self.Vh.forward(wf, n_seq=Gb * n, T=1, h0=hw, tag="shw", train=False)["v"]
                mark(ev)
                K.shield_select(vn.view(Gb * n, nh), Vh_t[sl], a_pol[sl], us, vs, dt, alpha, margin, ro.action_tm[t][sl],
                                log["index"][t][sl], log["flag"][t][sl], log["h"][t][sl])
                mark(ev)
            OE.step(cfg, st, ro.action_tm[t], nst, ro.reward_tm[t], ro.cost_tm[t])
            mark(ev)
            if ev is not None:
                events.append(tuple(ev))
        return ro, log

    def lookahead_select(self, st: OE.State, carry_next, a_pol, us, vs, horizon: int, margin: float, action, index, flag, s,
                         records: Optional[list] = None, t: int = 0, mark: Optional[Callable[[], None]] = None):
        cfg = self.cfg
        if cfg.is_vmas:
            raise ValueError("lookahead_select: VMASReverseTransport is not supported")
        n, HC = cfg.n_agents, self.HC
        H = int(horizon)
        if H < 1:
            raise ValueError(f"lookahead_select: horizon must be >= 1 (got {horizon})")
        margin = float(margin)
        if not np.isfinite(margin):
            raise ValueError("lookahead_select: margin must be finite")
        if self.hp.use_rnn and carry_next is None:
            raise ValueError("lookahead_select: this engine's policy has a recurrent cell: carry_next is required")
        if not self.hp.use_rnn:
            carry_next = None
        B = int(a_pol.shape[0])
        P = 1 + int(us.numel()) * int(vs.numel())
        block = max(1, min(B, max(1, self.prepass_graphs) // (n * P * (H + 2))))
        cache = self._la_records = getattr(self, "_la_records", {})
        for e0 in range(0, B, block):
            Eb = min(block, B - e0)
            sl = slice(e0, e0 + Eb)
            G = Eb * n * P
            rec = cache.get((G, H)) if records is None else None
            if rec is None:
                rec = RolloutData(cfg, G, H + 1, self.device, False, HC)
                if records is None:
                    if len(cache) >= 2:
                        cache.clear()
                    cache[(G, H)] = rec
            cut = OE.State({k: x[sl] for k, x in st.step.items()}, {k: x[sl] for k, x in st.env.items()})
            if carry_next is None:
                rec.rnn_tm[1].zero_()
            OE.team_action_fork(cfg, cut, a_pol[sl], us, vs, rec.states_tm[0], rec.action_tm[0],
                                carry_next[e0 * n:(e0 + Eb) * n] if carry_next is not None else None,
                                rec.rnn_tm[1].view(G * n, HC) if carry_next is not None else None)
            OE.step(cfg, rec.states_tm[0], rec.action_tm[0], rec.states_tm[1], rec.reward_tm[0], rec.cost_tm[0])
            if mark:
                mark()
            self._rollout_steps(rec, None, G, False, start=1)
            if mark:
                mark()
            K.lookahead_select(rec.cost_tm[1:H + 1], a_pol[sl], us, vs, margin, action[sl], index[sl], flag[sl], s[sl])
            if mark:
                mark()
            if records is not None:
                records.append((int(t), e0, Eb, rec))

    def rollout_lookahead_shielded(self, seeds: torch.Tensor, us, vs, horizon: int, margin: float = 0.0,
                                   events: Optional[list] = None, records: Optional[list] = None):
        cfg, T = self.cfg, self.T
        if cfg.is_vmas:
            raise ValueError("rollout_lookahead_shielded: VMASReverseTransport is not supported")
        n, HC = cfg.n_agents, self.HC
        H = int(horizon)
        if H < 1:
            raise ValueError(f"rollout_lookahead_shielded: horizon must be >= 1 (got {horizon})")
        margin = float(margin)
        if not np.isfinite(margin):
            raise ValueError("rollout_lookahead_shielded: margin must be finite")
        us, vs = K.sweep_axis(us, "us", self.device), K.sweep_axis(vs, "vs", self.device)
        P = 1 + int(us.numel()) * int(vs.numel())
        B = int(seeds.shape[0])
        dev = self.device
        ro = RolloutData(cfg, B, T, dev, False, HC)
        OE.reset(cfg, seeds, ro.states_tm[0], self.reset_failed)
        ro.rnn_tm[0].zero_()
        log = dict(policy_action=torch.empty(T, B, n, 2, device=dev), index=torch.empty(T, B, n, dtype=torch.int32, device=dev),
                   flag=torch.empty(T, B, n, dtype=torch.int32, device=dev), s=torch.empty(T, B, n, P, device=dev))
        for t in range(T):
            st = ro.states_tm[t]
            ev = [] if events is not None else None

            def mark():
                if ev is not None:
                    ev.append(torch.cuda.Event(enable_timing=True))
                    ev[-1].record()
            mark()
            feats = self._feats("la", st, B)
            h_next = ro.rnn_tm[t + 1].view(B * n, HC)
            act = self.policy.forward(feats, n_seq=B * n, T=1, h0=ro.rnn_tm[t].view(B * n, HC), tag="la", hs_out=h_next,
                                      train=False)
            a_pol = log["policy_action"][t]
            K.policy_head(act["ms"], None, None, a_pol.view(B * n, 2), None, None, n, 1)
            mark()
            self.lookahead_select(st, h_next if self.hp.use_rnn else None, a_pol, us, vs, H, margin, ro.action_tm[t],
                                  log["index"][t], log["flag"][t], log["s"][t], records=records, t=t, mark=mark)
            OE.step(cfg, st, ro.action_tm[t], ro.states_tm[t + 1], ro.reward_tm[t], ro.cost_tm[t])
            mark()
            if ev is not None:
                events.append(tuple(ev))
        return ro, log

    def cbf_weight_at(self, step: int) -> float:
        hp = self.hp
        w = hp.cbf_weight
        if hp.cbf_schedule:
            if step >= int(hp.train_steps * 0.5):
                w *= 2
            if step >= int(hp.train_steps * 0.75):
                w *= 2
        return w

    def cost_weight_at(self, step: int) -> float:
        hp = self.hp
        w = hp.cost_weight
        if hp.cost_schedule:
            if step >= int(hp.train_steps * 0.5):
                w *= 5
            if step >= int(hp.train_steps * 0.75):
                w *= 5
        return w

    def targets_hcbfcrpo(self, ro: RolloutData, step: int):
        cfg, T, B, hp = self.cfg, self.T, ro.B, self.hp
        n, nh, dev = cfg.n_agents, self.n_cost, self.device
        Vl, _ = self.values_prepass(ro, want_Vl=True, want_Vh=False)
        fin = OE.State({k: v[:, T].contiguous() for k, v in ro.step.items()}, ro.env)
        A = self.arena
        fin_cost = A.get("tg.fin_cost", B, n, nh)
        OE.step(cfg, fin, torch.zeros(B, n, 2, device=dev), fin.like(), torch.empty(B, device=dev), fin_cost)
        Vh = A.get("tg.Vh.crafted", B, T + 1, n, nh)
        Vh[:, :T].copy_(ro.costs)
        Vh[:, T].copy_(fin_cost)
        Qh = A.get("tg.Qh", B, T, n, nh)
        Ql = A.get("tg.Ql", B, T)
        OA.gae(ro.costs, ro.rewards, Vh, Vl, self.lam_pow, hp.gamma, hp.gae_lambda, Qh, Ql)
        adv = A.get("tg.adv", B, T, n)
        self.stats.zero_()
        OA.advantage(Ql, Vl, Vh, cfg.dt, hp.alpha, hp.cbf_eps, self.cbf_weight_at(step), adv, self.stats[3])
        return dict(Vl=Vl, Vh=Vh, Ql=Ql, Qh=Qh, adv=adv)

    def targets_informarl(self, ro: RolloutData, step: int):
        cfg, T, B, hp = self.cfg, self.T, ro.B, self.hp
        n, nh, dev = cfg.n_agents, self.n_cost, self.device
        Vl, _ = self.values_prepass(ro, want_Vl=True, want_Vh=False)
        A = self.arena
        Vh = A.get("tg.Vh.bcast", B, T + 1, n, nh)
        Vh.copy_(Vl.view(B, T + 1, 1, 1).expand(B, T + 1, n, nh))
        shaped = A.get("tg.shaped", B, T)
        OA.shaped_reward(ro.rewards, ro.costs, self.cost_weight_at(step), shaped)
        Qh = A.get("tg.Qh", B, T, n, nh)
        Ql = A.get("tg.Ql", B, T)
        OA.gae(ro.costs, shaped, Vh, Vl, self.lam_pow, hp.gamma, hp.gae_lambda, Qh, Ql)
        adv = A.get("tg.adv", B, T, n)
        self.stats.zero_()
        OA.advantage(Ql, Vl, None, cfg.dt, 0.0, 0.0, 0.0, adv, self.stats[3])
        return dict(Vl=Vl, Ql=Ql, Qh=Qh, adv=adv)

    def targets_lagr(self, ro: RolloutData, step: int):
        cfg, T, B, hp = self.cfg, self.T, ro.B, self.hp
        n, nh, A = cfg.n_agents, self.n_cost, self.arena
        Vl, _ = self.values_prepass(ro, want_Vl=True, want_Vh=False)
        Vh = A.get("tg.Vh.lagr", B, T + 1, n, nh)
        block = max(1, min(B, self.prepass_graphs // (T + 1)))
        for e0 in range(0, B, block):
            Eb = min(block, B - e0)
            feats = self._block_feats("pre", ro, e0, Eb, 0, T + 1)
            act = self.Vh.forward(feats, n_seq=Eb * n, T=T + 1, h0=None, tag="pre", train=False)
            Vh[e0:e0 + Eb].copy_(act["v"].view(Eb, T + 1, n, nh))
        cpos = A.get("tg.costs_pos", B, T, n, nh)
        OA.relu_fwd(ro.costs, cpos)
        Qh = A.get("tg.Qh", B, T, n, nh)
        Ql = A.get("tg.Ql", B, T)
        OA.gae(cpos, ro.rewards, Vh, Vl, self.lam_pow, hp.gamma, hp.gae_lambda, Qh, Ql)
        adv = A.get("tg.adv", B, T, n)
        Ah = A.get("tg.Ah", B, T, n, nh)
        self.stats.zero_()
        OA.advantage_lagr(Ql, Vl, Qh, Vh, self.lagr, adv, Ah)
        return dict(Vl=Vl, Vh=Vh, Ql=Ql, Qh=Qh, adv=adv, Ah=Ah)

    def _net_streams(self):
        if self._side_streams is None:
            self._side_streams = [torch.cuda.Stream(self.device) for _ in range(3)]
        return self._side_streams

    def _opt_step(self, name: str, lr: float):
        net, opt = self.nets[name], self.opt[name]
        if self.grad_hook is not None:
            self.grad_hook(name, net, self._mb)
        OA.clip_adam_step(net.params, net.grads, opt.m, opt.v, opt.state, lr, self.hp.max_grad_norm,
                          grad_scale=1.0 / self.world)
        net.prepare()

    def targets(self, ro: RolloutData, det: RolloutData, step: int):
        cfg, T, B, hp = self.cfg, self.T, ro.B, self.hp
        n, nh = cfg.n_agents, self.n_cost
        Vl, Vh = self.values_prepass(ro, want_Vl=True)
        _, Vh_det = self.values_prepass(det, want_Vl=False)
        A = self.arena
        Qh = A.get("tg.Qh", B, T, n, nh)
        Ql = A.get("tg.Ql", B, T)
        OA.gae(ro.costs, ro.rewards, Vh, Vl, self.lam_pow, hp.gamma, hp.gae_lambda, Qh, Ql)
        Qh_det = A.get("tg.Qh_det", B, T, n, nh)
        Ql_det = A.get("tg.Ql_det", B, T)
        OA.gae(det.costs, det.rewards, Vh_det, Vl, self.lam_pow, hp.gamma, hp.gae_lambda, Qh_det, Ql_det)
        adv = A.get("tg.adv", B, T, n)
        self.stats.zero_()
        OA.advantage(Ql, Vl, Vh, cfg.dt, hp.alpha, hp.cbf_eps, self.cbf_weight_at(step), adv, self.stats[3])
        return dict(Vl=Vl, Vh=Vh, Vh_det=Vh_det, Ql=Ql, Qh=Qh, Qh_det=Qh_det, adv=adv)

    def update(self, ro: RolloutData, det: RolloutData, step: int, perm: np.ndarray) -> dict:
        cfg, T, B, hp = self.cfg, self.T, ro.B, self.hp
        n, nh, H = cfg.n_agents, self.n_cost, nets.HID
        informarl = self.algo in ("informarl", "hcbfcrpo")
        lagr = self.algo == "informarl_lagr"
        import time as _time
        th = [_time.perf_counter()]
        ro.finalize()
        if self.algo == "dgppo":
            det.finalize()
        assert B * T >= hp.batch_size, "n_env_train * T must be >= batch_size (dgppo.py:153)"
        Eb = hp.batch_size // T
        assert B % Eb == 0 and T % hp.rnn_step == 0, "B % (batch_size // T) == 0 and T % rnn_step == 0 required (SURVEY A.11)"
        C = T // hp.rnn_step
        tg = (self.targets_informarl(ro, step) if self.algo == "informarl" else
              self.targets_hcbfcrpo(ro, step) if self.algo == "hcbfcrpo" else
              self.targets_lagr(ro, step) if lagr else self.targets(ro, det, step))
        th.append(_time.perf_counter())
        perm = np.asarray(perm)
        assert perm.size == 0 or (0 <= int(perm.min()) and int(perm.max()) < B), "perm holds env ids outside [0, B)"
        idx_all = torch.from_numpy(np.ascontiguousarray(perm.astype(np.int32))).to(self.device)
        n_mb = B // Eb
        G = Eb * T
        R = G * n
        is_cuda = self.device.type == "cuda"
        reduce = self.allreduce is not None
        A = self.arena
        mb_idx32 = A.get("mb.idx32", Eb, dtype=torch.int32)
        Ql_mb = A.get("mb.Ql", Eb, T)
        act_mb = A.get("mb.act", Eb, T, n, 2)
        lp_old_mb = A.get("mb.lp_old", Eb, T, n)
        adv_mb = A.get("mb.adv", Eb, T, n)
        if self.algo == "dgppo":
            h0_det = A.get("mb.h0_det", Eb, T, n, H)
            Qh_det_mb = A.get("mb.Qh_det", Eb, T, n, nh)
        if lagr:
            Qh_mb = A.get("mb.Qh", Eb, T, n, nh)
            Vh_mb = A.get("mb.Vh", Eb, T + 1, n, nh)
            Ah_mb = A.get("mb.Ah", Eb, T, n, nh)

        ctx = {}

        def lagr_step(apply_now: bool):
            full = self.policy.forward(ctx["feats"], n_seq=Eb * n, T=T, h0=None, tag="lg", train=False)
            lp_full = A.get("mb.lp_full", R)
            K.policy_head(full["ms"], self.eps_hat, act_mb.view(R, 2), None, lp_full, A.get("mb.ent_full", R), n, 2)
            if apply_now:
                OA.lagr_update(lp_full.view(Eb, T, n), lp_old_mb, Vh_mb, Ah_mb, self.lagr, self.lagr_sums, hp.gamma, hp.lr_lagr)
            else:
                OA.lagr_sums(lp_full.view(Eb, T, n), lp_old_mb, Vh_mb, Ah_mb, self.lagr_sums, hp.gamma)

        def body_pre():
            main = torch.cuda.current_stream(self.device) if is_cuda else None
            side = self._net_streams() if (self.multi_stream and main is not None) else None
            self.stats[:3].zero_()
            feats = ctx["feats"] = self._block_feats("mb", ro, 0, Eb, 0, T, env_ids=mb_idx32)
            pairs = [(tg["Ql"], Ql_mb)]
            if self.algo == "dgppo":
                feats_det = self._block_feats("mbd", det, 0, Eb, 0, T, env_ids=mb_idx32)
                full = None
                if self.HC == H:
                    pairs.append((det.rnn_states, h0_det))
                else:
                    full = A.get("mb.h0_det_full", Eb, T, n, self.HC)
                    pairs.append((det.rnn_states, full))
                pairs.append((tg["Qh_det"], Qh_det_mb))
            if lagr:
                pairs += [(tg["Qh"], Qh_mb), (tg["Vh"], Vh_mb), (tg["Ah"], Ah_mb)]
            pairs += [(ro.actions, act_mb), (ro.log_pis, lp_old_mb), (tg["adv"], adv_mb)]
            K.gather_rows(pairs, mb_idx32)
            if self.algo == "dgppo" and full is not None:
                h0_det.copy_(full[..., :H])

            def update_Vl():
                act = self.Vl.forward(feats, n_seq=Eb * C, T=hp.rnn_step, h0=None, tag="tr")
                dv = A.get("mb.dv", G, 1)
                K.value_loss(act["v"], Ql_mb.view(G, 1), dv, self.stats[0])
                self.Vl.zero_grads()
                self.Vl.backward(act, dv)
                if not reduce:
                    self._opt_step("Vl", hp.lr_Vl)

            def update_Vh():
                if lagr:
                    act = self.Vh.forward(feats, n_seq=Eb * C * n, T=hp.rnn_step, h0=None, tag="tr")
                    target = Qh_mb
                else:
                    act = self.Vh.forward(feats_det, n_seq=R, T=1, h0=h0_det.view(R, H) if hp.use_rnn else None, tag="tr")
                    target = Qh_det_mb
                dvh = A.get("mb.dvh", R, nh)
                K.value_loss(act["v"], target.view(R, nh), dvh, self.stats[1])
                self.Vh.zero_grads()
                self.Vh.backward(act, dvh)
                if not reduce:
                    self._opt_step("Vh", hp.lr_Vh)

            def update_policy():
                act = self.policy.forward(feats, n_seq=Eb * C * n, T=hp.rnn_step, h0=None, tag="tr")
                lp = A.get("mb.lp", R)
                ent = A.get("mb.ent", R)
                dms = A.get("mb.dms", R, 4)
                K.policy_head(act["ms"], self.eps_hat, act_mb.view(R, 2), None, lp, ent, n, 2, lp_old_mb.view(R),
                              adv_mb.view(R), dms, self.stats[2], hp.clip_eps, hp.coef_ent)
                self.policy.zero_grads()
                self.policy.backward(act, dms)
                if not reduce:
                    self._opt_step("policy", hp.lr_actor)
                if lagr and not reduce:
                    lagr_step(apply_now=True)

            if informarl:
                update_Vh = lambda: None
            if side is None:
                update_Vl(); update_Vh(); update_policy()
            else:
                ready = main.record_event()
                for fn, st in ((update_policy, side[0]), (update_Vl, side[1]), (update_Vh, side[2])):
                    with torch.cuda.stream(st):
                        st.wait_event(ready)
                        fn()
                for st in side:
                    main.wait_stream(st)

        def body_post():
            self._opt_step("Vl", hp.lr_Vl)
            if not informarl:
                self._opt_step("Vh", hp.lr_Vh)
            self._opt_step("policy", hp.lr_actor)
            if lagr:
                lagr_step(apply_now=False)

        def exchange_lagr():
            self.allreduce(self.lagr_sums)
            OA.lagr_apply(self.lagr, self.lagr_sums, self.world * Eb * T, hp.lr_lagr)

        def exchange():
            self.allreduce(self.flat_grads[:self.n_reduced])

        def step_body():
            body_pre()
            if reduce:
                exchange()
                body_post()
                if lagr:
                    exchange_lagr()

        slot = None
        if self.use_graphs and is_cuda and self.grad_hook is None:
            key = (self.algo, B, Eb, ro.agent.data_ptr(), det.agent.data_ptr() if det is not None else 0,
                   tg["adv"].data_ptr(), tg["Ql"].data_ptr(), mb_idx32.data_ptr(), self._update_generation())
            slot = self._upd_graph
            if slot.get("key") != key:
                slot.clear()
                slot["key"] = key
        for mb in range(n_mb):
            self._mb = mb
            mb_idx32.copy_(idx_all[mb * Eb:(mb + 1) * Eb])
            if slot is not None and slot.get("graph") is not None:
                slot["graph"].replay()
                if reduce:
                    exchange()
                    slot["graph_post"].replay()
                    if lagr:
                        exchange_lagr()
                K.FLOPS[0] += slot["flops"]
                continue
            f0 = K.FLOPS[0]
            step_body()
            if slot is not None and not slot.get("failed", False):
                slot["flops"] = K.FLOPS[0] - f0
                if slot.get("key")[-1] != self._update_generation():
                    slot["key"] = slot["key"][:-1] + (self._update_generation(),)
                    continue
                graph = torch.cuda.CUDAGraph()
                try:
                    f1 = K.FLOPS[0]
                    with torch.cuda.graph(graph, capture_error_mode="thread_local"):
                        body_pre()
                    if reduce:
                        gpost = torch.cuda.CUDAGraph()
                        with torch.cuda.graph(gpost, capture_error_mode="thread_local"):
                            body_post()
                        slot["graph_post"] = gpost
                    K.FLOPS[0] = f1
                    slot["graph"] = graph
                except Exception as ex:
                    slot["failed"] = True
                    torch.cuda.synchronize()
                    print(f"[dgppo_amd] HIP-graph capture of the minibatch step failed ({type(ex).__name__}: {ex}); "
                          f"continuing with eager launches", flush=True)
        th.append(_time.perf_counter())
        self._last = dict(Ql_mb=Ql_mb, G=G, R=R, nh=nh, B=B, Qh_mb=Qh_mb if lagr else None)
        out = self.info(ro)
        th.append(_time.perf_counter())
        self.host_ms = {"issue_targets": 1e3 * (th[1] - th[0]), "issue_minibatches": 1e3 * (th[2] - th[1]),
                        "wait_device": 1e3 * (th[3] - th[2])}
        return out

    def info(self, ro: RolloutData) -> dict:
        from . import dist as D
        L = self._last
        s = self.stats.cpu().numpy().copy()
        n_bad = int(self.reset_failed.item())
        if n_bad:
            self.reset_failed.zero_()
            raise RuntimeError(f"env reset: {n_bad} environment(s) of the last rollouts got no valid scene within the kernels' "
                               f"rejection-loop bounds (too many agents / obstacles for the area?) — the batch is invalid")
        s[:3] /= self.world
        G, R, nh, B = L["G"], L["R"], L["nh"], L["B"]
        o = {k: self.opt[k].state[:8].cpu().numpy() for k in self.opt}
        pol_loss = s[2, 0] / R - self.hp.coef_ent * s[2, 1] / R
        lagr = self.algo == "informarl_lagr"
        ext = [float(L["Ql_mb"].max()), -float(L["Ql_mb"].min()), -float(ro.log_pis.min())]
        if lagr:
            ext += [float(L["Qh_mb"].max()), -float(L["Qh_mb"].min())]
        ext = D.host_allreduce(np.asarray(ext, np.float64), "max", self.world)
        safe = float(D.host_allreduce(np.asarray([s[3, 0]], np.float64), "sum", self.world)[0])
        out = {
            "Vl/loss": float(s[0, 0] / G), "Vl/grad_norm": float(o["Vl"][4]), "Vl/has_nan": float(o["Vl"][5]),
            "Vl/max_target": float(ext[0]), "Vl/min_target": float(-ext[1]),
            "policy/loss": float(pol_loss), "policy/grad_norm": float(o["policy"][4]), "policy/has_nan": float(o["policy"][5]),
            "policy/log_pi_min": float(-ext[2]), "policy/clip_frac": float(s[2, 2] / R),
            "policy/entropy": float(s[2, 1] / R), "policy/total_variation_dist": float(0.5 * s[2, 3] / R),
        }
        if lagr:
            out.update({"Vh/loss": float(s[1, 0] / (R * nh)), "Vh/grad_norm": float(o["Vh"][4]), "Vh/has_nan": float(o["Vh"][5]),
                        "Vh/max_target": float(ext[3]), "Vh/min_target": float(-ext[4]),
                        "policy/lagr_mean": float(self.lagr.mean())})
        if self.algo == "dgppo":
            out.update({"Vh/loss_Vh": float(s[1, 0] / (R * nh)), "Vh/grad_Vh_norm": float(o["Vh"][4]),
                        "Vh/grad_Vh_has_nan": float(o["Vh"][5])})
        if self.algo in ("dgppo", "hcbfcrpo"):
            out["eval/safe_data"] = safe / (self.world * B * self.T * self.cfg.n_agents)
        return out
```

dgppo_amd/nets.py:

```python
from __future__ import annotations

import math
from typing import Dict, List, Optional, Tuple

import numpy as np
import torch

from . import _native as N
from . import ops_nn as K

H_HEADS = 3
MSG_DIM = 32
OUT_DIM = 64
HID = 64


def _ceil4(x):
    return (x + 3) // 4 * 4


class Layout:
    def __init__(self):
        self.entries: Dict[str, Tuple[int, Tuple[int, ...]]] = {}
        self.size = 0

    def add(self, name, *shape):
        n = int(np.prod(shape))
        self.size = (self.size + 3) // 4 * 4
        self.entries[name] = (self.size, tuple(shape))
        self.size += n

    def view(self, flat: torch.Tensor, name: str) -> torch.Tensor:
        off, shape = self.entries[name]
        return flat[off:off + math.prod(shape)].view(shape)


def make_layout(kind: str, node_dim: int, gnn_layers: int, n_out: int, rnn: str = "gru", rnn_layers: int = 1) -> Layout:
    L = Layout()
    f = node_dim
    for l in range(gnn_layers):
        d = OUT_DIM if l == gnn_layers - 1 else MSG_DIM
        hd = H_HEADS * d
        for nm, shp in (("Wq", (f, hd)), ("bq", (hd,)), ("Wk", (f, hd)), ("bk", (hd,)), ("Wv", (f, hd)), ("bv", (hd,)),
                        ("We", (4, hd)), ("Wu", (f, d)), ("bu", (d,))):
            L.add(f"gnn{l}.{nm}", *shp)
        f = d
    for i in (1, 2):
        L.add(f"mlp.W{i}", 2 * HID if (kind == "Vhg" and i == 1) else HID, HID)
        L.add(f"mlp.b{i}", HID)
        L.add(f"mlp.g{i}", HID)
        L.add(f"mlp.be{i}", HID)
    assert rnn in ("gru", "lstm", "none"), rnn
    for l in range(rnn_layers if rnn == "lstm" else 0):
        L.add(f"lstm{l}.Wi", HID, 4 * HID)
        L.add(f"lstm{l}.Wh", HID, 4 * HID)
        L.add(f"lstm{l}.bh", 4 * HID)
    for l in range(rnn_layers if rnn == "gru" else 0):
        pre = "gru" if l == 0 else f"gru{l}"
        L.add(f"{pre}.Wi", HID, 3 * HID)
        L.add(f"{pre}.bi", 3 * HID)
        L.add(f"{pre}.Wh", HID, 3 * HID)
        L.add(f"{pre}.bhn", HID)
    if kind == "policy":
        L.add("head.Ws", HID, HID)
        L.add("head.bs", HID)
        L.add("head.Wms", HID, 2 * n_out)
        L.add("head.bms", 2 * n_out)
    else:
        L.add("head.Wo", HID, n_out)
        L.add("head.bo", n_out)
    return L


class Arena:

    def __init__(self, device):
        self.device = device
        self.bufs: Dict[str, torch.Tensor] = {}
        self.generation = 0

    def get(self, name: str, *shape, dtype=torch.float32, zero=False) -> torch.Tensor:
        n = math.prod(shape)
        b = self.bufs.get(name)
        if b is None or b.numel() < n or b.dtype != dtype:
            if b is not None:
                self.generation += 1
            b = torch.empty(max(n, 1), dtype=dtype, device=self.device)
            self.bufs[name] = b
        v = b[:n].view(shape)
        if zero:
            v.zero_()
        return v


class GraphFeats:

    def __init__(self, cfg: N.EnvCfg, G: int, arena: Arena, tag: str):
        self.cfg, self.G = cfg, G
        n, S = cfg.n_agents, cfg.fan_in
        self.n_other = cfg.num_nodes - 1 - n
        self.Fp = input_width(cfg)
        self.Xa = arena.get(f"{tag}.Xa0", G * n, self.Fp)
        self.Xo = arena.get(f"{tag}.Xo0", max(G * self.n_other, 1), self.Fp)[:G * self.n_other]
        self.efeat = arena.get(f"{tag}.efeat", G * n, S, 4)
        self.emask = arena.get(f"{tag}.emask", G * n, S)
        self.edges_from_rows = False

    def compute(self, agent, agent_se, agent_st, goal, obst, hits, hits_se, hits_st, env_ids, n_env, n_time):
        assert n_env * n_time == self.G
        K.graph_feats(self.cfg, agent, agent_se, agent_st, goal, obst, hits, hits_se, hits_st, env_ids, n_env, n_time,
                      self.Xa, self.Xo if self.n_other > 0 else None, self.efeat, self.emask, self.Fp)
        self.edges_from_rows = self.cfg.state_dim == 4
        return self

    def compute_record(self, step, slots: int, env, env_ids, n_env, n_time):
        cfg, n = self.cfg, self.cfg.n_agents
        se, st = slots, int(slots > 1)
        if cfg.is_vmas:
            return self.compute_vmas(step["agent"], se * n * 4, st * n * 4, step["body"], se * 4, st * 4, env["scene"], env_ids,
                                     n_env, n_time)
        ia, ih = n * cfg.state_dim, n * cfg.top_k * 2
        return self.compute(step["agent"], se * ia, st * ia, env["goal"], env.get("obst"), step.get("hits"), se * ih, st * ih,
                            env_ids, n_env, n_time)

    def compute_sweep(self, step, env, frame_ids, n_frames, agent_id, xs, ys, ray_cos=None, ray_sin=None, hits_out=None,
                      frame_max=None):
        cfg, n = self.cfg, self.cfg.n_agents
        if cfg.is_vmas:
            raise ValueError("compute_sweep: VMASReverseTransport has no sweep entry point")
        K.graph_feats_sweep(cfg, step["agent"], n * cfg.state_dim, env["goal"], env.get("obst"), step.get("hits"),
                            n * cfg.top_k * 2, ray_cos, ray_sin, frame_ids, n_frames, agent_id, xs, ys, self.Xa,
                            self.Xo if self.n_other > 0 else None, self.efeat, self.emask, self.Fp, hits_out, frame_max)
        self.edges_from_rows = False
        return self

    def compute_action_sweep(self, step, env, frame_ids, n_frames, agent_id, us, vs, frame_max=None):
        cfg, n = self.cfg, self.cfg.n_agents
        if cfg.is_vmas:
            raise ValueError("compute_action_sweep: VMASReverseTransport has no sweep entry point")
        K.graph_feats_action_sweep(cfg, step["agent"], n * cfg.state_dim, env["goal"], env.get("obst"), step.get("hits"),
                                   n * cfg.top_k * 2, frame_ids, n_frames, agent_id, us, vs, self.Xa,
                                   self.Xo if self.n_other > 0 else None, self.efeat, self.emask, self.Fp, frame_max)
        self.edges_from_rows = False
        return self

    def compute_team_action_sweep(self, st, nst, a_pol, us, vs):
        if self.cfg.is_vmas:
            raise ValueError("compute_team_action_sweep: VMASReverseTransport has no sweep entry point")
        K.graph_feats_team_action_sweep(self.cfg, st.step["agent"], nst.step["agent"], st.env["goal"], st.env.get("obst"),
                                        nst.step.get("hits"), a_pol, us, vs, self.Xa, self.Xo if self.n_other > 0 else None,
                                        self.efeat, self.emask, self.Fp)
        self.edges_from_rows = False
        return self

    def compute_vmas(self, agent, agent_se, agent_st, body, body_se, body_st, scene, env_ids, n_env, n_time):
        assert n_env * n_time == self.G
        K.vmas_graph_feats(self.cfg, agent, agent_se, agent_st, body, body_se, body_st, scene, env_ids, n_env, n_time,
                           self.Xa, self.efeat, self.emask, self.Fp)
        self.edges_from_rows = False
        return self


def input_width(cfg: N.EnvCfg) -> int:
    return _ceil4(cfg.node_dim) if cfg.is_vmas else 8


class Net:

    def __init__(self, kind: str, cfg: N.EnvCfg, gnn_layers: int, n_out: int, device, grads: Optional[torch.Tensor] = None,
                 rnn: str = "gru", rnn_layers: int = 1, lean_attn0: bool = True):
        assert kind in ("policy", "Vl", "Vh", "Vhg")
        self.kind, self.cfg, self.gnn_layers, self.n_out, self.device = kind, cfg, gnn_layers, n_out, device
        self.rnn, self.rnn_layers = rnn, (rnn_layers if rnn != "none" else 0)
        self.lean_attn0 = bool(lean_attn0) and K.attn_rows_supported(cfg, input_width(cfg), H_HEADS)
        self.carry_dim = HID * max(self.rnn_layers, 1) * (2 if rnn == "lstm" else 1)
        self.layout = make_layout(kind, cfg.node_dim, gnn_layers, n_out, rnn, rnn_layers)
        self.params = torch.zeros(self.layout.size, device=device)
        if grads is None:
            grads = torch.zeros(self.layout.size, device=device)
        assert grads.shape == (self.layout.size,) and grads.is_contiguous() and grads.data_ptr() % 16 == 0
        self.grads = grads
        self.arena = Arena(device)
        self.ws_arena = Arena(device)
        self._views: Dict[tuple, torch.Tensor] = {}
        self.dims = []
        f = cfg.node_dim
        for l in range(gnn_layers):
            d = OUT_DIM if l == gnn_layers - 1 else MSG_DIM
            fp = input_width(cfg) if l == 0 else f
            kp = _ceil4(fp + H_HEADS * (fp + 4) + 1)
            self.dims.append((f, fp, d, kp))
            f = d
        self.prep_layout = Layout()
        for l, (f, fp, d, kp) in enumerate(self.dims):
            self.prep_layout.add(f"gnn{l}.Mcat", fp, H_HEADS * fp)
            self.prep_layout.add(f"gnn{l}.cvec", H_HEADS * fp)
            self.prep_layout.add(f"gnn{l}.Wout", kp, d)
        self.prep = torch.zeros(self.prep_layout.size, device=device)
        self.prep_grads = torch.zeros(self.prep_layout.size, device=device)

    def _cached(self, kind: str, layout, flat, name):
        key = (kind, name)
        v = self._views.get(key)
        if v is None:
            v = self._views[key] = layout.view(flat, name)
        return v

    def p(self, name):
        return self._cached("p", self.layout, self.params, name)

    def g(self, name):
        return self._cached("g", self.layout, self.grads, name)

    def pp(self, name):
        return self._cached("pp", self.prep_layout, self.prep, name)

    def pg(self, name):
        return self._cached("pg", self.prep_layout, self.prep_grads, name)

    def prepare(self):
        for l, (f, fp, d, kp) in enumerate(self.dims):
            q = lambda nm: self.p(f"gnn{l}.{nm}")
            K.gnn_prep(q("Wq"), q("bq"), q("Wk"), q("Wv"), q("bv"), q("We"), q("Wu"), self.pp(f"gnn{l}.Mcat"),
                       self.pp(f"gnn{l}.cvec"), self.pp(f"gnn{l}.Wout"), f, fp, d, H_HEADS, kp)

    def _xo_fusable(self, l: int) -> bool:
        if l != 0 or self.gnn_layers != 2:
            return False
        key = "_xo_ok"
        if not hasattr(self, key):
            f1, fp1, d1, kp1 = self.dims[1]
            setattr(self, key, self.dims[0][1] == 8 and self.dims[0][2] == 32 and fp1 == 32 and
                    K.attn_xo_supported(self.cfg, fp1, H_HEADS, kp1))
        return getattr(self, key)

    def zero_grads(self):
        self.grads.zero_()

    def forward(self, feats: GraphFeats, n_seq: int, T: int, h0: Optional[torch.Tensor], tag: str = "f",
                hs_out: Optional[torch.Tensor] = None, train: bool = True, qt0: Optional[torch.Tensor] = None):
        cfg, G, A = self.cfg, feats.G, self.arena
        n = cfg.n_agents
        R = G * n
        Ro = G * feats.n_other
        act = {"feats": feats, "G": G, "n_seq": n_seq, "T": T}
        Xa, Xo = feats.Xa, feats.Xo
        xo_fused = None
        for l, (f, fp, d, kp) in enumerate(self.dims):
            if l == 0 and qt0 is not None:
                assert tuple(qt0.shape) == (R, H_HEADS * fp), (tuple(qt0.shape), R, H_HEADS * fp)
                qt = qt0
            else:
                qt = A.get(f"{tag}.qt{l}", R, H_HEADS * fp)
                K.dense_fwd(Xa, self.pp(f"gnn{l}.Mcat"), self.pp(f"gnn{l}.cvec"), qt)
            zcat = A.get(f"{tag}.zcat{l}", R, kp)
            lean = l == 0 and self.lean_attn0 and feats.edges_from_rows
            attn = A.get(f"{tag}.attn{l}", R, cfg.fan_in, H_HEADS) if train and not lean else None
            if lean:
                K.attn_fwd_rows(cfg, fp, H_HEADS, kp, qt, Xa, Xo if Ro > 0 else None, feats.emask, zcat, None, G)
            elif xo_fused is not None:
                K.attn_fwd_xo(cfg, fp, H_HEADS, kp, qt, Xa, xo_fused[0], xo_fused[1], xo_fused[2], feats.efeat, feats.emask, zcat, attn, G)
            else:
                K.attn_fwd(cfg, fp, H_HEADS, kp, qt, Xa, Xo if Ro > 0 else None, feats.efeat, feats.emask, zcat, attn, G)
            act[f"xo_fused{l}"] = xo_fused
            xo_fused = None
            Xa_n = A.get(f"{tag}.Xa{l + 1}", R, d)
            K.dense_fwd(zcat, self.pp(f"gnn{l}.Wout"), self.p(f"gnn{l}.bu"), Xa_n, act=1)
            act[f"Xa{l}"], act[f"Xo{l}"], act[f"qt{l}"], act[f"zcat{l}"], act[f"attn{l}"] = Xa, Xo, qt, zcat, attn
            act[f"lean{l}"] = lean
            if l < self.gnn_layers - 1 and Ro > 0:
                if self._xo_fusable(l):
                    xo_fused = (Xo, self.pp(f"gnn{l}.Wout")[:fp], self.p(f"gnn{l}.bu"))
                    Xo = None
                else:
                    Xo_n = A.get(f"{tag}.Xo{l + 1}", Ro, d)
                    K.dense_fwd(Xo, self.pp(f"gnn{l}.Wout")[:fp], self.p(f"gnn{l}.bu"), Xo_n, act=1)
                    Xo = Xo_n
            Xa = Xa_n
        act[f"Xa{self.gnn_layers}"] = Xa
        if self.kind == "Vl":
            pooled = A.get(f"{tag}.pool", G, OUT_DIM)
            K.mean_agents(Xa, pooled, G, n, OUT_DIM)
            x, Rh, n_inner = pooled, G, 1
        else:
            x, Rh, n_inner = Xa, R, n
        if self.kind == "Vhg":
            pooled = A.get(f"{tag}.pool", G, OUT_DIM)
            K.mean_agents(Xa, pooled, G, n, OUT_DIM)
            xcat = A.get(f"{tag}.xcat", R, 2 * OUT_DIM)
            xcat[:, :OUT_DIM].copy_(Xa)
            xcat.view(G, n, 2 * OUT_DIM)[:, :, OUT_DIM:].copy_(pooled.view(G, 1, OUT_DIM).expand(G, n, OUT_DIM))
            x = xcat
        act["Rh"], act["n_inner"], act["mlp_in"] = Rh, n_inner, x
        gi = A.get(f"{tag}.gi", Rh, 3 * HID)
        if self.kind == "Vhg" or self.rnn != "gru":
            sv = {nm: A.get(f"{tag}.{nm}", Rh, w) for nm, w in (("p1", HID), ("y1", HID), ("st1", 2), ("p2", HID), ("y2", HID), ("st2", 2))}
            K.dense_fwd(x, self.p("mlp.W1"), self.p("mlp.b1"), sv["p1"])
            K.ln_relu_fwd(sv["p1"], self.p("mlp.g1"), self.p("mlp.be1"), sv["y1"], sv["st1"])
            K.dense_fwd(sv["y1"], self.p("mlp.W2"), self.p("mlp.b2"), sv["p2"])
            K.ln_relu_fwd(sv["p2"], self.p("mlp.g2"), self.p("mlp.be2"), sv["y2"], sv["st2"])
            if self.rnn == "gru":
                K.dense_fwd(sv["y2"], self.p("gru.Wi"), self.p("gru.bi"), gi)
            act.update(sv)
        else:
            saves = None
            if train:
                saves = tuple(A.get(f"{tag}.{nm}{i}", Rh, w) for i in (1, 2) for nm, w in (("p", HID), ("y", HID), ("st", 2)))
                for i in (1, 2):
                    act[f"p{i}"], act[f"y{i}"], act[f"st{i}"] = saves[3 * (i - 1):3 * i]
            K.mlp_gi_fwd(x, self.p("mlp.W1"), self.p("mlp.b1"), self.p("mlp.g1"), self.p("mlp.be1"), self.p("mlp.W2"),
                         self.p("mlp.b2"), self.p("mlp.g2"), self.p("mlp.be2"), self.p("gru.Wi"), self.p("gru.bi"), gi, saves)
        assert n_seq * T == Rh, (n_seq, T, Rh)
        L, CD = self.rnn_layers, self.carry_dim
        h0_blocks = isinstance(h0, K.H0Blocks)
        if h0_blocks:
            assert self.rnn == "gru" and L == 1 and T == 1 and not train and self.kind != "policy", \
                "a blocked h0 serves the one-cell GRU value nets' T = 1 inference pass"
        elif h0 is not None:
            assert tuple(h0.shape) == (n_seq, CD), (tuple(h0.shape), n_seq, CD)
        if hs_out is not None:
            assert tuple(hs_out.shape) == (Rh, CD), (tuple(hs_out.shape), Rh, CD)
        act["gi"] = gi
        simple = (self.rnn == "gru" and L == 1)
        if simple:
            hs = hs_out if hs_out is not None else A.get(f"{tag}.hs", Rh, HID)
            hprev_is_h0 = train and T == 1 and h0 is not None and self.kind != "policy"
            hprev = A.get(f"{tag}.hprev", Rh, HID) if (train and not hprev_is_h0) else None
            gates = A.get(f"{tag}.gates", Rh, 4 * HID) if train else None
            feat = hs
            act["hs"], act["hprev"], act["gates"] = hs, hprev, gates
        fused_tail = (simple and T == 1 and self.kind == "policy")
        if simple and not fused_tail:
            if h0_blocks:
                K.gru_fwd_h0_blocks(gi, self.p("gru.Wh"), self.p("gru.bhn"), h0, hs, hprev, gates, n_seq, T, n_inner)
            else:
                K.gru_fwd(gi, self.p("gru.Wh"), self.p("gru.bhn"), h0, hs, hprev, gates, n_seq, T, n_inner)
            if hprev_is_h0:
                act["hprev"] = act["h0"] = h0
        if self.rnn == "none":
            feat = act["y2"]
            if hs_out is not None:
                if h0 is not None and T == 1:
                    hs_out.copy_(h0)
                else:
                    hs_out.zero_()
        elif self.rnn == "lstm":
            x_l = act["y2"]
            act["stack"] = []
            for l in range(L):
                zi = A.get(f"{tag}.zi{l}", Rh, 4 * HID)
                for half in (slice(0, 2 * HID), slice(2 * HID, 4 * HID)):
                    K.dense_fwd(x_l, self.p(f"lstm{l}.Wi")[:, half], None, zi[:, half])
                c0_l = h0_l = None
                if h0 is not None:
                    c0_l, h0_l = A.get(f"{tag}.c0_{l}", n_seq, HID), A.get(f"{tag}.h0_{l}", n_seq, HID)
                    c0_l.copy_(h0[:, (2 * l) * HID:(2 * l + 1) * HID])
                    h0_l.copy_(h0[:, (2 * l + 1) * HID:(2 * l + 2) * HID])
                cs_l, hs_l = A.get(f"{tag}.cs{l}", Rh, HID), A.get(f"{tag}.hs{l}", Rh, HID)
                cprev_l = A.get(f"{tag}.cprev{l}", Rh, HID) if train else None
                hprev_l = A.get(f"{tag}.hprev{l}", Rh, HID) if train else None
                gates_l = A.get(f"{tag}.gates{l}", Rh, 4 * HID) if train else None
                K.lstm_fwd(zi, self.p(f"lstm{l}.Wh"), self.p(f"lstm{l}.bh"), c0_l, h0_l, cs_l, hs_l, cprev_l, hprev_l, gates_l,
                           n_seq, T, n_inner)
                if hs_out is not None:
                    hs_out[:, (2 * l) * HID:(2 * l + 1) * HID].copy_(cs_l)
                    hs_out[:, (2 * l + 1) * HID:(2 * l + 2) * HID].copy_(hs_l)
                act["stack"].append(dict(x=x_l, hs=hs_l, cprev=cprev_l, hprev=hprev_l, gates=gates_l))
                x_l = hs_l
            feat = x_l
        elif not simple:
            x_l = None
            act["stack"] = []
            for l in range(L):
                pre = "gru" if l == 0 else f"gru{l}"
                gi_l = gi if l == 0 else A.get(f"{tag}.gi{l}", Rh, 3 * HID)
                if l > 0:
                    K.dense_fwd(x_l, self.p(f"{pre}.Wi"), self.p(f"{pre}.bi"), gi_l)
                h0_l = None
                if h0 is not None:
                    h0_l = A.get(f"{tag}.h0_{l}", n_seq, HID)
                    h0_l.copy_(h0[:, l * HID:(l + 1) * HID])
                hs_l = A.get(f"{tag}.hs{l}", Rh, HID)
                hprev_l = A.get(f"{tag}.hprev{l}", Rh, HID) if train else None
                gates_l = A.get(f"{tag}.gates{l}", Rh, 4 * HID) if train else None
                K.gru_fwd(gi_l, self.p(f"{pre}.Wh"), self.p(f"{pre}.bhn"), h0_l, hs_l, hprev_l, gates_l, n_seq, T, n_inner)
                if hs_out is not None:
                    hs_out[:, l * HID:(l + 1) * HID].copy_(hs_l)
                act["stack"].append(dict(x=x_l, gi=gi_l, hs=hs_l, hprev=hprev_l, gates=gates_l))
                x_l = hs_l
            feat = x_l
        act["feat"] = feat
        if self.kind == "policy":
            u = A.get(f"{tag}.u", Rh, HID) if (train or not fused_tail) else None
            ms = A.get(f"{tag}.ms", Rh, 4)
            if fused_tail:
                K.gru1_head_fwd(gi, self.p("gru.Wh"), self.p("gru.bhn"), h0, self.p("head.Ws"), self.p("head.bs"),
                                self.p("head.Wms"), self.p("head.bms"), hs, hprev, gates, u, ms)
            else:
                K.dense_fwd(feat, self.p("head.Ws"), self.p("head.bs"), u)
                K.dense_fwd(u, self.p("head.Wms"), self.p("head.bms"), ms)
            act["u"], act["ms"] = u, ms
        else:
            v = A.get(f"{tag}.v", Rh, self.n_out)
            K.dense_fwd(feat, self.p("head.Wo"), self.p("head.bo"), v)
            act["v"] = v
        return act

    def backward(self, act, dout: torch.Tensor, tag: str = "b"):
        A = self.arena
        ws_floats = getattr(self, "_bwdw_floats", 16 << 20)

        def _alloc(n_floats):
            self._bwdw_floats = max(ws_floats, n_floats)
            return self.ws_arena.get(f"{tag}.bwdw_ws", self._bwdw_floats)
        batch = K.BwdWBatch(self.device, _alloc) if dout.is_cuda else None
        if batch is not None:
            batch.__enter__()
        try:
            self._backward_body(act, dout, tag)
        except BaseException:
            if batch is not None:
                batch.__exit__(RuntimeError, None, None)
            raise
        if batch is not None:
            batch.__exit__(None, None, None)
        for l, (f, fp, d, kp) in enumerate(self.dims):
            q = lambda nm: self.p(f"gnn{l}.{nm}")
            gq = lambda nm: self.g(f"gnn{l}.{nm}")
            K.gnn_unprep(self.pg(f"gnn{l}.Mcat"), self.pg(f"gnn{l}.cvec"), self.pg(f"gnn{l}.Wout"), q("Wq"), q("bq"), q("Wk"),
                         gq("Wq"), gq("bq"), gq("Wk"), gq("Wv"), gq("bv"), gq("We"), gq("Wu"), f, fp, d, H_HEADS, kp)
        self.prep_grads.zero_()

    @staticmethod
    def _gru_t1_in_pass(act, T, row_operands) -> bool:
        return (T == 1 and act.get("h0") is not None and act["hprev"] is act["h0"]
                and all(t.is_cuda and t.data_ptr() % 16 == 0 for t in row_operands))

    def _backward_body(self, act, dout: torch.Tensor, tag: str):
        cfg, A = self.cfg, self.arena
        G, Rh, n_inner, n_seq, T = act["G"], act["Rh"], act["n_inner"], act["n_seq"], act["T"]
        n = cfg.n_agents
        R = G * n
        feats: GraphFeats = act["feats"]
        Ro = G * feats.n_other
        feat = act["feat"]
        fused_trunk = self.rnn == "gru" and self.rnn_layers == 1 and self.kind != "Vhg" and dout.is_cuda
        dgi0 = None
        dhs = A.get(f"{tag}.dhs", Rh, HID)
        if dout.is_cuda:
            if self.kind == "policy":
                K.head_bwd(feat, act["u"], dout, self.p("head.Ws"), self.p("head.Wms"), dhs, self.g("head.Ws"), self.g("head.bs"),
                           self.g("head.Wms"), self.g("head.bms"))
            else:
                K.head_bwd(feat, None, dout, self.p("head.Wo"), None, dhs, self.g("head.Wo"), self.g("head.bo"))
        elif self.kind == "policy":
            K.dense_bwd_w(act["u"], dout, self.g("head.Wms"), self.g("head.bms"))
            du = A.get(f"{tag}.du", Rh, HID)
            K.dense_fwd(dout, self.p("head.Wms"), None, du, trans_w=True)
            K.dense_bwd_w(feat, du, self.g("head.Ws"), self.g("head.bs"))
            K.dense_fwd(du, self.p("head.Ws"), None, dhs, trans_w=True)
        else:
            K.dense_bwd_w(feat, dout, self.g("head.Wo"), self.g("head.bo"))
            K.dense_fwd(dout, self.p("head.Wo"), None, dhs, trans_w=True)
        if self.rnn == "none":
            dy = dhs
        elif self.rnn == "lstm":
            stack = act["stack"]
            for l in range(len(stack) - 1, -1, -1):
                st = stack[l]
                dz = A.get(f"{tag}.dz_lstm{l}", Rh, 4 * HID)
                K.lstm_bwd(dhs, self.p(f"lstm{l}.Wh"), st["cprev"], st["gates"], dz, n_seq, T, n_inner)
                for half in (slice(0, 2 * HID), slice(2 * HID, 4 * HID)):
                    K.dense_bwd_w(st["hprev"], dz[:, half], self.g(f"lstm{l}.Wh")[:, half], self.g(f"lstm{l}.bh")[half])
                    K.dense_bwd_w(st["x"], dz[:, half], self.g(f"lstm{l}.Wi")[:, half], None)
                dx = A.get(f"{tag}.dy" if l == 0 else f"{tag}.dx{l}", Rh, HID)
                K.dense_fwd(dz, self.p(f"lstm{l}.Wi"), None, dx, trans_w=True)
                dhs = dx
            dy = dhs
        else:
            stack = act.get("stack") or [dict(x=None, gi=act["gi"], hs=act["hs"], hprev=act["hprev"], gates=act["gates"])]
            if act.get("stack") is None and dout.is_cuda:
                st = stack[0]
                dgi = A.get(f"{tag}.dgi0", Rh, 3 * HID)
                gW = (self.g("gru.Wi"), self.g("gru.bi"), self.g("gru.Wh"), self.g("gru.bhn"))
                if self._gru_t1_in_pass(act, T, (act["y2"], st["hprev"], dhs, st["gates"], dgi)):
                    K.gru_bwd_w_t1(act["y2"], st["hprev"], dhs, st["gates"], dgi, *gW)
                else:
                    dhn = A.get(f"{tag}.dhn0", Rh, HID)
                    K.gru_bwd_dhn(dhs, self.p("gru.Wh"), st["hprev"], st["gates"], dgi, dhn, n_seq, T, n_inner)
                    K.gru_bwd_w(act["y2"], st["hprev"], dgi, dhn, *gW)
                if fused_trunk:
                    dgi0 = dgi
                else:
                    dhs = A.get(f"{tag}.dy", Rh, HID)
                    K.dense_fwd(dgi, self.p("gru.Wi"), None, dhs, trans_w=True)
                stack = []
            for l in range(len(stack) - 1, -1, -1):
                st = stack[l]
                pre = "gru" if l == 0 else f"gru{l}"
                dgi = A.get(f"{tag}.dgi{l}", Rh, 3 * HID)
                dgh = A.get(f"{tag}.dgh{l}", Rh, 3 * HID)
                K.gru_bwd(dhs, self.p(f"{pre}.Wh"), st["hprev"], st["gates"], dgi, dgh, n_seq, T, n_inner)
                K.dense_bwd_w(st["hprev"], dgh[:, :2 * HID], self.g(f"{pre}.Wh")[:, :2 * HID], None)
                K.dense_bwd_w(st["hprev"], dgh[:, 2 * HID:], self.g(f"{pre}.Wh")[:, 2 * HID:], self.g(f"{pre}.bhn"))
                x_l = act["y2"] if l == 0 else st["x"]
                K.dense_bwd_w(x_l, dgi, self.g(f"{pre}.Wi"), self.g(f"{pre}.bi"))
                if l == 0 and fused_trunk:
                    dgi0 = dgi
                    break
                dx = A.get(f"{tag}.dy" if l == 0 else f"{tag}.dx{l}", Rh, HID)
                K.dense_fwd(dgi, self.p(f"{pre}.Wi"), None, dx, trans_w=True)
                dhs = dx
            dy = dhs
        x_in = {1: act["mlp_in"], 2: act["y1"]}
        top = act[f"Xa{self.gnn_layers}"]
        if fused_trunk:
            dy = A.get(f"{tag}.dyy1", Rh, HID)
            K.mlp_gi_bwd_w(dgi0, self.p("gru.Wi"), self.p("mlp.W2"), self.p("mlp.W1"), self.p("mlp.g2"), self.p("mlp.g1"),
                           act["p2"], act["y2"], act["st2"], act["p1"], act["y1"], act["st1"], x_in[1],
                           top if self.kind in ("policy", "Vh") else None, dy,
                           self.g("mlp.g2"), self.g("mlp.be2"), self.g("mlp.g1"), self.g("mlp.be1"),
                           self.g("mlp.W2"), self.g("mlp.b2"), self.g("mlp.W1"), self.g("mlp.b1"))
        for i in (() if fused_trunk else (2, 1)):
            dpre = A.get(f"{tag}.dpre{i}", Rh, HID)
            K.ln_relu_bwd(act[f"p{i}"], act[f"y{i}"], act[f"st{i}"], self.p(f"mlp.g{i}"), dy, dpre, self.g(f"mlp.g{i}"),
                          self.g(f"mlp.be{i}"))
            K.dense_bwd_w(x_in[i], dpre, self.g(f"mlp.W{i}"), self.g(f"mlp.b{i}"))
            dy = A.get(f"{tag}.dyy{i}", Rh, HID if not (self.kind == "Vhg" and i == 1) else 2 * HID)
            K.dense_fwd(dpre, self.p(f"mlp.W{i}"), None, dy, trans_w=True,
                        relu_mask=top if (i == 1 and self.kind in ("policy", "Vh")) else None)
        if self.kind == "Vl":
            dXa = A.get(f"{tag}.dXaL", R, OUT_DIM)
            K.mean_agents(dy, dXa, G, n, OUT_DIM, backward=True, relu_mask=top)
        elif self.kind == "Vhg":
            dXa = A.get(f"{tag}.dXaL", R, OUT_DIM)
            dXa.copy_(dy[:, :OUT_DIM])
            dglob = A.get(f"{tag}.dglob", R, OUT_DIM)
            dglob.copy_(dy[:, OUT_DIM:])
            dpool = A.get(f"{tag}.dpool", G, OUT_DIM)
            K.mean_agents(dglob, dpool, G, n, OUT_DIM)
            K.mean_agents(dpool, dXa, G, n, OUT_DIM, backward=2, relu_mask=top)
        else:
            dXa = dy
        dXo = None
        for l in range(self.gnn_layers - 1, -1, -1):
            f, fp, d, kp = self.dims[l]
            dz = A.get(f"{tag}.dz{l}", R, kp)
            K.dense_bwd_xw(act[f"zcat{l}"], dXa, self.pp(f"gnn{l}.Wout"), dz, self.pg(f"gnn{l}.Wout"), self.g(f"gnn{l}.bu"))
            if dXo is not None:
                K.dense_bwd_w(act[f"Xo{l}"], dXo, self.pg(f"gnn{l}.Wout")[:fp], self.g(f"gnn{l}.bu"))
            dqt = A.get(f"{tag}.dqt{l}", R, H_HEADS * fp)
            need_dx = l > 0
            dXa_l = A.get(f"{tag}.dXa{l}", R, fp) if need_dx else None
            dXo_prev = dXo
            dXo_l = A.get(f"{tag}.dXo{l}", Ro, fp) if (need_dx and Ro > 0) else None
            more_dXo = dXo_prev is not None and dXo_l is not None
            xf = act.get(f"xo_fused{l}")
            if act.get(f"lean{l}"):
                K.attn_bwd_rows(cfg, fp, H_HEADS, kp, dz, None, act[f"qt{l}"], feats.emask, act[f"Xa{l}"],
                                act[f"Xo{l}"] if Ro > 0 else None, dqt, G)
            elif xf is not None and dXa_l is not None and not more_dXo:
                ws = A.get(f"{tag}.xo_ws", K.attn_xo_workspace_floats(G), 1).view(-1)
                K.attn_bwd_xo_dw(cfg, fp, H_HEADS, kp, dz, act[f"attn{l}"], act[f"qt{l}"], act[f"Xa{l}"], xf[0], xf[1], xf[2],
                                 feats.efeat, dqt, dXa_l, self.pg(f"gnn{l - 1}.Wout")[:self.dims[l - 1][1]], self.g(f"gnn{l - 1}.bu"), ws, G)
                dXo_l = None
            elif xf is not None:
                K.attn_bwd_xo(cfg, fp, H_HEADS, kp, dz, act[f"attn{l}"], act[f"qt{l}"], act[f"Xa{l}"], xf[0], xf[1], xf[2],
                              feats.efeat, dqt, dXa_l, dXo_l, G, relu_xo=(dXo_l is not None and not more_dXo))
            else:
                K.attn_bwd(cfg, fp, H_HEADS, kp, dz, act[f"attn{l}"], act[f"qt{l}"], act[f"Xa{l}"],
                           act[f"Xo{l}"] if Ro > 0 else None, feats.efeat, dqt, dXa_l, dXo_l, G,
                           relu_xo=(dXo_l is not None and not more_dXo))
            if need_dx:
                K.dense_bwd_xw(act[f"Xa{l}"], dqt, self.pp(f"gnn{l}.Mcat"), dXa_l, self.pg(f"gnn{l}.Mcat"), self.pg(f"gnn{l}.cvec"),
                               accumulate_mask=True)
            else:
                K.dense_bwd_w(act[f"Xa{l}"], dqt, self.pg(f"gnn{l}.Mcat"), self.pg(f"gnn{l}.cvec"))
            if need_dx:
                if more_dXo:
                    K.dense_fwd(dXo_prev, self.pp(f"gnn{l}.Wout")[:fp], None, dXo_l, accumulate=True, trans_w=True,
                                relu_mask=act[f"Xo{l}"])
            dXa, dXo = dXa_l, dXo_l

    def load_tree(self, tree: dict):
        t = tree["params"]
        to = lambda x: torch.as_tensor(np.asarray(x), dtype=torch.float32).to(self.device)
        if self.kind == "policy":
            base, gnn, head_name = t["PolicyNet_0"], t["PolicyNet_0"]["GraphTransformerGNN_0"], "PolicyGNNHead"
        else:
            base, gnn, head_name = t, t["GraphTransformerGNN_0"], "ValueGNNHead"
        for l in range(self.gnn_layers):
            gl = gnn[f"GraphTransformer_{l}"]
            for nm, dn, key in (("Wq", "Dense_0", "kernel"), ("bq", "Dense_0", "bias"), ("Wk", "Dense_1", "kernel"),
                                ("bk", "Dense_1", "bias"), ("Wv", "Dense_2", "kernel"), ("bv", "Dense_2", "bias"),
                                ("We", "Dense_3", "kernel"), ("Wu", "Dense_4", "kernel"), ("bu", "Dense_4", "bias")):
                self.p(f"gnn{l}.{nm}").copy_(to(gl[dn][key]))
        hd = base[head_name]
        for i in (1, 2):
            self.p(f"mlp.W{i}").copy_(to(hd[f"Dense_{i - 1}"]["kernel"]))
            self.p(f"mlp.b{i}").copy_(to(hd[f"Dense_{i - 1}"]["bias"]))
            self.p(f"mlp.g{i}").copy_(to(hd[f"LayerNorm_{i - 1}"]["scale"]))
            self.p(f"mlp.be{i}").copy_(to(hd[f"LayerNorm_{i - 1}"]["bias"]))
        for l in range(self.rnn_layers if self.rnn == "lstm" else 0):
            lc = base["RNN_0"][f"LSTMCell_{3 * l + 2}"]
            self.p(f"lstm{l}.Wi").copy_(torch.cat([to(lc[k]["kernel"]) for k in ("ii", "if", "ig", "io")], dim=1))
            self.p(f"lstm{l}.Wh").copy_(torch.cat([to(lc[k]["kernel"]) for k in ("hi", "hf", "hg", "ho")], dim=1))
            self.p(f"lstm{l}.bh").copy_(torch.cat([to(lc[k]["bias"]) for k in ("hi", "hf", "hg", "ho")]))
        for l in range(self.rnn_layers if self.rnn == "gru" else 0):
            pre = "gru" if l == 0 else f"gru{l}"
            gr = base["RNN_0"][f"GRUCell_{2 * l + 1}"]
            self.p(f"{pre}.Wi").copy_(torch.cat([to(gr[k]["kernel"]) for k in ("ir", "iz", "in")], dim=1))
            self.p(f"{pre}.bi").copy_(torch.cat([to(gr[k]["bias"]) for k in ("ir", "iz", "in")]))
            self.p(f"{pre}.Wh").copy_(torch.cat([to(gr[k]["kernel"]) for k in ("hr", "hz", "hn")], dim=1))
            self.p(f"{pre}.bhn").copy_(to(gr["hn"]["bias"]))
        if self.kind == "policy":
            self.p("head.Ws").copy_(to(t["ScaleHid"]["kernel"]))
            self.p("head.bs").copy_(to(t["ScaleHid"]["bias"]))
            self.p("head.Wms").copy_(torch.cat([to(t["OutputDenseMean"]["kernel"]), to(t["OutputDenseStdTrans"]["kernel"])], 1))
            self.p("head.bms").copy_(torch.cat([to(t["OutputDenseMean"]["bias"]), to(t["OutputDenseStdTrans"]["bias"])]))
        else:
            self.p("head.Wo").copy_(to(t["Dense_0"]["kernel"]))
            self.p("head.bo").copy_(to(t["Dense_0"]["bias"]))
        self.prepare()

    def to_tree(self, flat: Optional[torch.Tensor] = None) -> dict:
        flat = self.params if flat is None else flat
        v = lambda nm: self.layout.view(flat, nm).detach().cpu().numpy().copy()
        gnn = {}
        for l in range(self.gnn_layers):
            gnn[f"GraphTransformer_{l}"] = {
                "Dense_0": {"kernel": v(f"gnn{l}.Wq"), "bias": v(f"gnn{l}.bq")},
                "Dense_1": {"kernel": v(f"gnn{l}.Wk"), "bias": v(f"gnn{l}.bk")},
                "Dense_2": {"kernel": v(f"gnn{l}.Wv"), "bias": v(f"gnn{l}.bv")},
                "Dense_3": {"kernel": v(f"gnn{l}.We")},
                "Dense_4": {"kernel": v(f"gnn{l}.Wu"), "bias": v(f"gnn{l}.bu")},
            }
        head = {}
        for i in (1, 2):
            head[f"Dense_{i - 1}"] = {"kernel": v(f"mlp.W{i}"), "bias": v(f"mlp.b{i}")}
            head[f"LayerNorm_{i - 1}"] = {"scale": v(f"mlp.g{i}"), "bias": v(f"mlp.be{i}")}
        rnn = {}
        for l in range(self.rnn_layers if self.rnn == "lstm" else 0):
            Wi, Wh, bh = v(f"lstm{l}.Wi"), v(f"lstm{l}.Wh"), v(f"lstm{l}.bh")
            cell = {}
            for q, g_ in enumerate("ifgo"):
                cell["i" + g_] = {"kernel": Wi[:, q * 64:(q + 1) * 64]}
                cell["h" + g_] = {"kernel": Wh[:, q * 64:(q + 1) * 64], "bias": bh[q * 64:(q + 1) * 64]}
            rnn[f"LSTMCell_{3 * l + 2}"] = cell
        for l in range(self.rnn_layers if self.rnn == "gru" else 0):
            pre = "gru" if l == 0 else f"gru{l}"
            Wi, bi, Wh = v(f"{pre}.Wi"), v(f"{pre}.bi"), v(f"{pre}.Wh")
            rnn[f"GRUCell_{2 * l + 1}"] = {
                "ir": {"kernel": Wi[:, :64], "bias": bi[:64]}, "iz": {"kernel": Wi[:, 64:128], "bias": bi[64:128]},
                "in": {"kernel": Wi[:, 128:], "bias": bi[128:]}, "hr": {"kernel": Wh[:, :64]}, "hz": {"kernel": Wh[:, 64:128]},
                "hn": {"kernel": Wh[:, 128:], "bias": v(f"{pre}.bhn")}}
        if self.kind == "policy":
            Wms, bms = v("head.Wms"), v("head.bms")
            k = self.n_out
            return {"params": {
                "PolicyNet_0": dict({"GraphTransformerGNN_0": gnn, "PolicyGNNHead": head}, **({"RNN_0": rnn} if rnn else {})),
                "ScaleHid": {"kernel": v("head.Ws"), "bias": v("head.bs")},
                "OutputDenseMean": {"kernel": Wms[:, :k], "bias": bms[:k]},
                "OutputDenseStdTrans": {"kernel": Wms[:, k:], "bias": bms[k:]}}}
        return {"params": dict({"GraphTransformerGNN_0": gnn, "ValueGNNHead": head, "Dense_0": {"kernel": v("head.Wo"), "bias": v("head.bo")}},
                               **({"RNN_0": rnn} if rnn else {}))}
```

dgppo_amd/ops_algo.py:

```python
from __future__ import annotations

import ctypes as C

import numpy as np
import torch

from . import _native as N


def lam_pow_table(gae_lambda: float, T: int, device) -> torch.Tensor:
    return torch.from_numpy((np.float64(gae_lambda) ** np.arange(T + 1)).astype(np.float32)).to(device)


def gae(costs, rewards, Vh, Vl, lam_pow, gamma: float, gae_lambda: float, Qh, Ql):
    B, T, n, nh = costs.shape
    N.expect_shape(rewards, (B, T), "rewards")
    N.expect_shape(Vh, (B, T + 1, n, nh), "Vh")
    N.expect_shape(Vl, (B, T + 1), "Vl")
    N.expect_shape(lam_pow, (T + 1,), "lam_pow")
    N.expect_shape(Qh, (B, T, n, nh), "Qh")
    N.expect_shape(Ql, (B, T), "Ql")
    rc = N.lib().dgppo_gae(N.ptr(costs), N.ptr(rewards), N.ptr(Vh), N.ptr(Vl), N.ptr(lam_pow), C.c_float(gamma),
                           C.c_float(1 - gamma), C.c_float(1 - gae_lambda), N.ptr(Qh), N.ptr(Ql), B, T, n, nh,
                           N.stream_ptr())
    N.check(rc, "dgppo_gae")


def constraint_return(cost_tm, gamma: float, value, worst):
    if cost_tm.ndim != 4:
        raise ValueError(f"constraint_return: cost_tm must be [K, G, n, nh], got {tuple(cost_tm.shape)}")
    K_, G, n, nh = cost_tm.shape
    if K_ < 1:
        raise ValueError("constraint_return: K must be >= 1")
    if not cost_tm[0].is_contiguous():
        raise ValueError("constraint_return: every step of cost_tm must be dense")
    N.expect_shape(value, (G, n, nh), "value")
    N.expect_shape(worst, (G, n, nh), "worst")
    rc = N.lib().dgppo_constraint_return(N.ptr(cost_tm[0], name="cost"), int(cost_tm.stride(0)), K_, G, n, nh, float(gamma),
                                         float(1 - gamma), N.ptr(value, name="value"), N.ptr(worst, name="worst"),
                                         N.stream_ptr())
    N.check(rc, "dgppo_constraint_return")


def shaped_reward(reward, cost, cost_weight: float, out):
    B, T, n, nh = cost.shape
    N.expect_shape(reward, (B, T), "reward")
    N.expect_shape(out, (B, T), "out")
    rc = N.lib().dgppo_shaped_reward(N.ptr(reward), N.ptr(cost), C.c_float(cost_weight), N.ptr(out), C.c_int64(B * T), n, nh,
                                     N.stream_ptr())
    N.check(rc, "dgppo_shaped_reward")


def advantage(Ql, Vl, Vh, dt, alpha, cbf_eps, cbf_weight, adv, stats):
    if Vh is None:
        B, T, n = adv.shape
        nh = 1
    else:
        B, T1, n, nh = Vh.shape
        T = T1 - 1
    N.expect_shape(Ql, (B, T), "Ql")
    N.expect_shape(Vl, (B, T + 1), "Vl")
    N.expect_shape(adv, (B, T, n), "adv")
    rc = N.lib().dgppo_advantage(N.ptr(Ql), N.ptr(Vl), N.ptr(Vh), C.c_float(dt), C.c_float(alpha), C.c_float(cbf_eps),
                                 C.c_float(cbf_weight), N.ptr(adv), N.ptr(stats), B, T, n, nh, N.stream_ptr())
    N.check(rc, "dgppo_advantage")


def clip_adam_step(params, grads, m, v, state, lr, max_norm, b1=0.9, b2=0.999, eps=1e-8, grad_scale=1.0):
    n = params.numel()
    for t, nm in ((grads, "grads"), (m, "m"), (v, "v")):
        N.expect_shape(t, (n,), nm)
    N.expect_shape(state, (N.OPT_STATE_FLOATS,), "state")
    rc = N.lib().dgppo_clip_adam_step(N.ptr(params), N.ptr(grads), N.ptr(m), N.ptr(v), C.c_int64(n), N.ptr(state),
                                      C.c_float(lr), C.c_float(b1), C.c_float(b2), C.c_float(eps), C.c_float(max_norm),
                                      C.c_float(grad_scale), N.stream_ptr())
    N.check(rc, "dgppo_clip_adam_step")


def advantage_lagr(Ql, Vl, Qh, Vh, lagr, adv, Ah):
    B, T, n, nh = Qh.shape
    N.expect_shape(Ql, (B, T), "Ql"); N.expect_shape(Vl, (B, T + 1), "Vl"); N.expect_shape(Vh, (B, T + 1, n, nh), "Vh")
    N.expect_shape(lagr, (n, nh), "lagr"); N.expect_shape(adv, (B, T, n), "adv"); N.expect_shape(Ah, (B, T, n, nh), "Ah")
    rc = N.lib().dgppo_advantage_lagr(N.ptr(Ql), N.ptr(Vl), N.ptr(Qh), N.ptr(Vh), N.ptr(lagr), N.ptr(adv), N.ptr(Ah), B, T, n, nh,
                                      N.stream_ptr())
    N.check(rc, "dgppo_advantage_lagr")


def lagr_update(lp_new, lp_old, Vh_mb, Ah_mb, lagr, sums, gamma: float, lr: float):
    Eb, T, n, nh = Ah_mb.shape
    N.expect_shape(lp_new, (Eb, T, n), "lp_new"); N.expect_shape(lp_old, (Eb, T, n), "lp_old")
    N.expect_shape(Vh_mb, (Eb, T + 1, n, nh), "Vh"); N.expect_shape(lagr, (n, nh), "lagr"); N.expect_shape(sums, (n * nh,), "sums")
    rc = N.lib().dgppo_lagr_update(N.ptr(lp_new), N.ptr(lp_old), N.ptr(Vh_mb), C.c_int64((T + 1) * n * nh), N.ptr(Ah_mb),
                                   N.ptr(lagr), N.ptr(sums), Eb, T, n, nh, C.c_float(1.0 - gamma), C.c_float(lr), N.stream_ptr())
    N.check(rc, "dgppo_lagr_update")


def lagr_sums(lp_new, lp_old, Vh_mb, Ah_mb, sums, gamma: float):
    Eb, T, n, nh = Ah_mb.shape
    N.expect_shape(lp_new, (Eb, T, n), "lp_new"); N.expect_shape(lp_old, (Eb, T, n), "lp_old")
    N.expect_shape(Vh_mb, (Eb, T + 1, n, nh), "Vh"); N.expect_shape(sums, (n * nh,), "sums")
    rc = N.lib().dgppo_lagr_sums(N.ptr(lp_new), N.ptr(lp_old), N.ptr(Vh_mb), C.c_int64((T + 1) * n * nh), N.ptr(Ah_mb),
                                 N.ptr(sums), Eb, T, n, nh, C.c_float(1.0 - gamma), N.stream_ptr())
    N.check(rc, "dgppo_lagr_sums")


def lagr_apply(lagr, sums, rows_total: int, lr: float):
    N.expect_shape(sums, (lagr.numel(),), "sums")
    rc = N.lib().dgppo_lagr_apply(N.ptr(lagr), N.ptr(sums), lagr.numel(), C.c_int64(rows_total), C.c_float(lr), N.stream_ptr())
    N.check(rc, "dgppo_lagr_apply")


def relu_fwd(x, out):
    rc = N.lib().dgppo_relu_fwd(N.ptr(x), N.ptr(out), C.c_int64(x.numel()), N.stream_ptr())
    N.check(rc, "dgppo_relu_fwd")
```

dgppo_amd/ops_nn.py:

```python
from __future__ import annotations

import ctypes as C
from typing import Optional

import numpy as np
import torch

from . import _native as N

FLOPS = [0.0]


def _mat(t: torch.Tensor, name: str):
    if t.dim() != 2:
        raise ValueError(f"{name} must be 2-D, got {tuple(t.shape)}")
    if not t.is_cuda:
        raise RuntimeError(f"{name} must live on the GPU (the HIP path has no CPU fallback)")
    if t.dtype != torch.float32:
        raise TypeError(f"{name} must be float32")
    if t.shape[1] > 1 and t.stride(1) != 1:
        raise ValueError(f"{name} must have unit inner stride")
    ld = t.stride(0) if t.shape[0] > 1 else max(t.shape[1], t.stride(0))
    return C.c_void_p(t.data_ptr()), int(ld), int(t.shape[0]), int(t.shape[1])


def _p(t: Optional[torch.Tensor], name="tensor", dtype=torch.float32):
    return N.ptr(t, dtype, name)


def dense_fwd(X, W, bias, Y, act: int = 0, accumulate: bool = False, trans_w: bool = False, relu_mask=None):
    xp, ldx, M, K = _mat(X, "X")
    wp, ldw, wr, wc = _mat(W, "W")
    yp, ldy, My, Ncol = _mat(Y, "Y")
    Kw, Nw = (wc, wr) if trans_w else (wr, wc)
    if Kw != K or Nw != Ncol or My != M:
        raise ValueError(f"dense_fwd: shape mismatch X{tuple(X.shape)} W{tuple(W.shape)} trans={trans_w} Y{tuple(Y.shape)}")
    if bias is not None:
        N.expect_shape(bias, (Ncol,), "bias")
    mp, ldm = C.c_void_p(0), 0
    if relu_mask is not None:
        mp, ldm, Mm, Nm = _mat(relu_mask, "relu_mask")
        if (Mm, Nm) != (M, Ncol):
            raise ValueError(f"dense_fwd: relu_mask {tuple(relu_mask.shape)} does not match Y {tuple(Y.shape)}")
    FLOPS[0] += 2.0 * M * K * Ncol
    rc = N.lib().dgppo_dense_fwd(xp, ldx, wp, ldw, _p(bias, "bias"), yp, ldy, M, K, Ncol, int(act), int(accumulate),
                                 int(trans_w), mp, ldm, N.stream_ptr())
    N.check(rc, "dgppo_dense_fwd")


def mlp_gi_fwd(X, W1, b1, g1, be1, W2, b2, g2, be2, Wi, bi, gi, saves=None):
    xp, ldx, M, K = _mat(X, "X")
    if K != 64:
        raise ValueError(f"mlp_gi_fwd: X must be [M, 64], got {tuple(X.shape)}")
    for t, shp, nm in ((W1, (64, 64), "W1"), (W2, (64, 64), "W2"), (Wi, (64, 192), "Wi"), (b1, (64,), "b1"), (g1, (64,), "g1"),
                       (be1, (64,), "be1"), (b2, (64,), "b2"), (g2, (64,), "g2"), (be2, (64,), "be2"), (bi, (192,), "bi"),
                       (gi, (M, 192), "gi")):
        N.expect_shape(t, shp, nm)
    sv = [None] * 6
    if saves is not None:
        for t, shp, nm in zip(saves, ((M, 64), (M, 64), (M, 2), (M, 64), (M, 64), (M, 2)), ("p1", "y1", "st1", "p2", "y2", "st2")):
            N.expect_shape(t, shp, nm)
        sv = list(saves)
    FLOPS[0] += 2.0 * M * (64 * 64 * 2 + 64 * 192)
    rc = N.lib().dgppo_mlp_gi_fwd(xp, ldx, _p(W1), _p(b1), _p(g1), _p(be1), _p(W2), _p(b2), _p(g2), _p(be2), _p(Wi), _p(bi),
                                  *[_p(t) for t in sv], _p(gi), M, N.stream_ptr())
    N.check(rc, "dgppo_mlp_gi_fwd")


def mlp_gi_bwd(dgi, Wi, W2, W1, g2, g1, p2, y2, st2, p1, y1, st1, relu_mask, dpre2, dpre1, dx, dg2, db2, dg1, db1):
    M = dgi.shape[0]
    N.expect_shape(dgi, (M, 192), "dgi")
    for t, shp, nm in ((Wi, (64, 192), "Wi"), (W2, (64, 64), "W2"), (W1, (64, 64), "W1"), (g2, (64,), "g2"), (g1, (64,), "g1"),
                       (p2, (M, 64), "p2"), (y2, (M, 64), "y2"), (st2, (M, 2), "st2"), (p1, (M, 64), "p1"), (y1, (M, 64), "y1"),
                       (st1, (M, 2), "st1"), (dpre2, (M, 64), "dpre2"), (dpre1, (M, 64), "dpre1"), (dx, (M, 64), "dx"),
                       (dg2, (64,), "dg2"), (db2, (64,), "db2"), (dg1, (64,), "dg1"), (db1, (64,), "db1")):
        N.expect_shape(t, shp, nm)
    mp, ldm = (None, 0)
    if relu_mask is not None:
        mp, ldm, Mm, Km = _mat(relu_mask, "relu_mask")
        if (Mm, Km) != (M, 64):
            raise ValueError(f"mlp_gi_bwd: relu_mask must be [M, 64], got {tuple(relu_mask.shape)}")
    FLOPS[0] += 2.0 * M * (64 * 64 * 2 + 64 * 192)
    rc = N.lib().dgppo_mlp_gi_bwd(_p(dgi), _p(Wi), _p(W2), _p(W1), _p(g2), _p(g1), _p(p2), _p(y2), _p(st2), _p(p1), _p(y1), _p(st1),
                                  mp if mp is not None else C.c_void_p(0), ldm, _p(dpre2), _p(dpre1), _p(dx), 64,
                                  _p(dg2), _p(db2), _p(dg1), _p(db1), M, N.stream_ptr())
    N.check(rc, "dgppo_mlp_gi_bwd")


def gru1_head_fwd(gi, Wh, bhn, h0, W1, b1, W2, b2, hs, hprev, gates, u, out):
    M = gi.shape[0]
    n_out = out.shape[1]
    N.expect_shape(gi, (M, 192), "gi"); N.expect_shape(Wh, (64, 192), "Wh"); N.expect_shape(bhn, (64,), "bhn")
    N.expect_shape(hs, (M, 64), "hs"); N.expect_shape(out, (M, n_out), "out")
    if h0 is not None:
        N.expect_shape(h0, (M, 64), "h0")
    if W2 is not None:
        N.expect_shape(W1, (64, 64), "W1"); N.expect_shape(b1, (64,), "b1")
        N.expect_shape(W2, (64, n_out), "W2"); N.expect_shape(b2, (n_out,), "b2")
    else:
        N.expect_shape(W1, (64, n_out), "W1"); N.expect_shape(b1, (n_out,), "b1")
    for t, shp, nm in ((hprev, (M, 64), "hprev"), (gates, (M, 256), "gates"), (u, (M, 64), "u")):
        if t is not None:
            N.expect_shape(t, shp, nm)
    FLOPS[0] += 2.0 * M * (64 * 192 + (64 * 64 + 64 * n_out if W2 is not None else 64 * n_out))
    rc = N.lib().dgppo_gru1_head_fwd(_p(gi), _p(Wh), _p(bhn), _p(h0), _p(W1), _p(b1), _p(W2), _p(b2), _p(hs), _p(hprev),
                                     _p(gates), _p(u), _p(out), M, n_out, N.stream_ptr())
    N.check(rc, "dgppo_gru1_head_fwd")


_WS: dict = {}


def _bwd_w_workspace(device, K: int, Ncol: int) -> torch.Tensor:
    lib = N.lib()
    lib.dgppo_dense_bwd_w_workspace_bytes.restype = C.c_int64
    need = int(lib.dgppo_dense_bwd_w_workspace_bytes(C.c_int32(K), C.c_int32(Ncol)))
    need = min(need, 64 << 20)
    key = (device.index, torch.cuda.current_stream(device).cuda_stream)
    ws = _WS.get(key)
    if ws is None or ws.numel() * 4 < need:
        ws = torch.empty(need // 4, dtype=torch.float32, device=device)
        _WS[key] = ws
    return ws


class ReduceDesc(C.Structure):
    _fields_ = [("part", C.c_void_p), ("dW", C.c_void_p), ("db", C.c_void_p), ("part_stride", C.c_int32), ("slabs", C.c_int32),
                ("ldw", C.c_int32), ("K", C.c_int32), ("N", C.c_int32), ("pending", C.c_int32)]


class BwdWBatch:
    _active = {}

    def __init__(self, device, alloc):
        self.device, self.alloc = device, alloc
        self.key = None
        self.descs = []
        self.offset = 0
        self.ws = None

    def __enter__(self):
        self.key = (self.device.index, torch.cuda.current_stream(self.device).cuda_stream)
        if self.key in BwdWBatch._active:
            raise RuntimeError("BwdWBatch: nested batches on one stream")
        BwdWBatch._active[self.key] = self
        return self

    def region(self, nbytes: int):
        nbytes = (nbytes + 255) & ~255
        if self.ws is None or self.ws.numel() * 4 < self.offset + nbytes:
            if self.descs:
                self.flush()
            self.ws = self.alloc(max(self.offset + nbytes, 2 * (self.ws.numel() * 4 if self.ws is not None else 0)) // 4)
        view = self.ws[self.offset // 4:(self.offset + nbytes) // 4]
        self.offset += nbytes
        return view

    def flush(self):
        if self.descs:
            arr = (ReduceDesc * len(self.descs))(*self.descs)
            N.check(N.lib().dgppo_dense_bwd_w_reduce_batch(arr, C.c_int32(len(self.descs)), N.stream_ptr()),
                    "dgppo_dense_bwd_w_reduce_batch")
        self.descs = []
        self.offset = 0

    def __exit__(self, *exc):
        try:
            if exc[0] is None:
                self.flush()
        finally:
            BwdWBatch._active.pop(self.key, None)
        return False


def dense_bwd_w(X, dY, dW, db=None):
    xp, ldx, M, K = _mat(X, "X")
    yp, ldy, My, Ncol = _mat(dY, "dY")
    wp, ldw, Kw, Nw = _mat(dW, "dW")
    if My != M or Kw != K or Nw != Ncol:
        raise ValueError(f"dense_bwd_w: shape mismatch X{tuple(X.shape)} dY{tuple(dY.shape)} dW{tuple(dW.shape)}")
    if db is not None:
        N.expect_shape(db, (Ncol,), "db")
    FLOPS[0] += 2.0 * M * K * Ncol
    batch = BwdWBatch._active.get((X.device.index, torch.cuda.current_stream(X.device).cuda_stream)) if X.is_cuda else None
    if batch is not None:
        lib = N.lib()
        lib.dgppo_dense_bwd_w_workspace_bytes.restype = C.c_int64
        need = min(int(lib.dgppo_dense_bwd_w_workspace_bytes(C.c_int32(K), C.c_int32(Ncol))), 64 << 20)
        ws = batch.region(need)
        d = ReduceDesc()
        rc = lib.dgppo_dense_bwd_w_deferred(xp, ldx, yp, ldy, wp, ldw, _p(db, "db"), M, K, Ncol, _p(ws, "workspace"),
                                            C.c_int64(ws.numel() * 4), C.byref(d), N.stream_ptr())
        N.check(rc, "dgppo_dense_bwd_w_deferred")
        if d.pending:
            batch.descs.append(d)
        return
    ws = _bwd_w_workspace(X.device, K, Ncol)
    rc = N.lib().dgppo_dense_bwd_w(xp, ldx, yp, ldy, wp, ldw, _p(db, "db"), M, K, Ncol, _p(ws, "workspace"),
                                   C.c_int64(ws.numel() * 4), N.stream_ptr())
    N.check(rc, "dgppo_dense_bwd_w")


def dense_bwd_xw(X, dY, W, dX, dW, db=None, accumulate_mask: bool = False):
    xp, ldx, M, K = _mat(X, "X")
    yp, ldy, My, Ncol = _mat(dY, "dY")
    pp, ldp, Kp, Np = _mat(W, "W")
    dxp, lddx, Mx, Kx = _mat(dX, "dX")
    wp, ldw, Kw, Nw = _mat(dW, "dW")
    if My != M or (Kw, Nw) != (K, Ncol) or (Kp, Np) != (K, Ncol) or (Mx, Kx) != (M, K):
        raise ValueError(f"dense_bwd_xw: shape mismatch X{tuple(X.shape)} dY{tuple(dY.shape)} W{tuple(W.shape)} "
                         f"dX{tuple(dX.shape)} dW{tuple(dW.shape)}")
    if db is not None:
        N.expect_shape(db, (Ncol,), "db")
    FLOPS[0] += 4.0 * M * K * Ncol
    batch = BwdWBatch._active.get((X.device.index, torch.cuda.current_stream(X.device).cuda_stream))
    lib = N.lib()
    if batch is not None:
        lib.dgppo_dense_bwd_w_workspace_bytes.restype = C.c_int64
        ws = batch.region(min(int(lib.dgppo_dense_bwd_w_workspace_bytes(C.c_int32(K), C.c_int32(Ncol))), 64 << 20))
        d = ReduceDesc()
        pend = C.byref(d)
    else:
        ws = _bwd_w_workspace(X.device, K, Ncol)
        pend = None
    rc = lib.dgppo_dense_bwd_xw(xp, ldx, yp, ldy, pp, ldp, dxp, lddx, int(bool(accumulate_mask)), wp, ldw, _p(db, "db"), M, K,
                                Ncol, _p(ws, "workspace"), C.c_int64(ws.numel() * 4), pend, N.stream_ptr())
    N.check(rc, "dgppo_dense_bwd_xw")
    if batch is not None and d.pending:
        batch.descs.append(d)


def _check_strided(fn: str, name: str, t_, se: int, st: int, inner: tuple, env_ids, n_env: int, n_time: int):
    if not (t_.is_cuda and t_.dtype == torch.float32):
        raise ValueError(f"{fn}: {name} must be a float32 CUDA tensor")
    want, acc = [], 1
    for d in reversed(inner):
        want.append(acc)
        acc *= d
    if tuple(t_.shape[-len(inner):]) != tuple(inner) or list(t_.stride()[-len(inner):]) != want[::-1]:
        raise ValueError(f"{fn}: the trailing {inner} block of {name} must be dense (got shape {tuple(t_.shape)}, "
                         f"strides {t_.stride()})")
    avail = t_.untyped_storage().nbytes() // 4 - t_.storage_offset()
    if env_ids is None and (n_env - 1) * se + (n_time - 1) * st + acc > avail:
        raise ValueError(f"{fn}: {name}: the strides reach beyond its storage")


def graph_feats(cfg: N.EnvCfg, agent, agent_se, agent_st, goal, obst, hits, hits_se, hits_st, env_ids, n_env, n_time,
                Xa, Xo, efeat, emask, Fp):
    G = n_env * n_time
    n, S = cfg.n_agents, cfg.fan_in
    n_other = cfg.num_nodes - 1 - n
    N.expect_shape(Xa, (G * n, Fp), "Xa")
    if n_other > 0:
        N.expect_shape(Xo, (G * n_other, Fp), "Xo")
    N.expect_shape(efeat, (G * n, S, 4), "efeat")
    N.expect_shape(emask, (G * n, S), "emask")
    _check_strided("graph_feats", "agent", agent, agent_se, agent_st, (n, cfg.state_dim), env_ids, n_env, n_time)
    if hits is not None:
        _check_strided("graph_feats", "hits", hits, hits_se, hits_st, (n, cfg.top_k, 2), env_ids, n_env, n_time)
    rc = N.lib().dgppo_graph_feats(
        C.byref(cfg), C.c_void_p(agent.data_ptr()), C.c_int64(agent_se), C.c_int64(agent_st), _p(goal, "goal"),
        _p(obst, "obst") if (obst is not None and not cfg.is_lidar) else C.c_void_p(0),
        C.c_void_p(hits.data_ptr()) if hits is not None else C.c_void_p(0), C.c_int64(hits_se), C.c_int64(hits_st),
        _p(env_ids, "env_ids", torch.int32), C.c_int32(n_env), C.c_int32(n_time), _p(Xa, "Xa"), _p(Xo, "Xo"),
        _p(efeat, "efeat"), _p(emask, "emask"), C.c_int32(Fp), N.stream_ptr())
    N.check(rc, "dgppo_graph_feats")


def sweep_axis(x, name: str, device) -> torch.Tensor:
    if torch.is_tensor(x):
        t_ = x.to(device=device, dtype=torch.float32).contiguous()
        ok = t_.ndim == 1 and t_.numel() > 0 and bool(torch.isfinite(t_).all())
    else:
        a = np.ascontiguousarray(np.asarray(x, dtype=np.float32))
        ok = a.ndim == 1 and a.size > 0 and bool(np.isfinite(a).all())
        t_ = torch.from_numpy(a).to(device) if ok else None
    if not ok:
        raise ValueError(f"graph_feats_sweep: {name} must be a non-empty 1-D array of finite coordinates")
    return t_


def _sweep_grid(fn: str, cfg: N.EnvCfg, frame_ids, n_frames, agent_id, xs, ys, frame_max, names=("xs", "ys")):
    n = cfg.n_agents
    if not 0 <= int(agent_id) < n:
        raise ValueError(f"{fn}: agent_id {agent_id} outside [0, {n})")
    for name, t_ in zip(names, (xs, ys)):
        if not (torch.is_tensor(t_) and t_.is_cuda and t_.dtype == torch.float32 and t_.ndim == 1 and t_.is_contiguous()):
            raise ValueError(f"{fn}: {name} must be a dense 1-D float32 CUDA tensor (sweep_axis)")
        if t_.numel() == 0:
            raise ValueError(f"{fn}: {name} is empty")
    ids = ids_dev = None
    if torch.is_tensor(frame_ids):
        if frame_max is None or n_frames < 1 or tuple(frame_ids.shape) != (n_frames,):
            raise ValueError(f"{fn}: a device frame_ids needs its shape (n_frames,) and frame_max")
        ids_dev, last = frame_ids, int(frame_max)
    elif frame_ids is not None:
        ids = np.asarray(frame_ids, dtype=np.int64).reshape(-1)
        if ids.size != n_frames or n_frames == 0 or ids.min() < 0:
            raise ValueError(f"{fn}: frame_ids must hold n_frames >= 1 frame numbers >= 0")
        last = int(ids.max())
    else:
        if n_frames < 1:
            raise ValueError(f"{fn}: n_frames must be >= 1")
        last = n_frames - 1
    return int(xs.numel()), int(ys.numel()), ids, ids_dev, last


def _sweep_record(fn: str, cfg: N.EnvCfg, agent, agent_st, obst, hits, hits_st, ray_cos, ray_sin, last, hits_out, G) -> bool:
    n = cfg.n_agents
    _check_strided(fn, "agent", agent, 0, agent_st, (n, cfg.state_dim), None, 1, last + 1)
    cast = cfg.is_lidar and cfg.n_obs > 0
    if cfg.n_obs > 0:
        if obst is None:
            raise ValueError(f"{fn}: obst is required when n_obs > 0")
        N.expect_shape(obst, (cfg.n_obs, cfg.obst_stride), "obst")
    if cast:
        if hits is None:
            raise ValueError(f"{fn}: hits is required for a LiDAR kind with obstacles")
        _check_strided(fn, "hits", hits, 0, hits_st, (n, cfg.top_k, 2), None, 1, last + 1)
        N.expect_shape(ray_cos, (cfg.n_rays,), "ray_cos")
        N.expect_shape(ray_sin, (cfg.n_rays,), "ray_sin")
        if hits_out is not None:
            N.expect_shape(hits_out, (G, cfg.top_k, 2), "hits_out")
    return cast


def graph_feats_sweep(cfg: N.EnvCfg, agent, agent_st, goal, obst, hits, hits_st, ray_cos, ray_sin, frame_ids, n_frames,
                      agent_id, xs, ys, Xa, Xo, efeat, emask, Fp, hits_out=None, frame_max=None):
    fn = "graph_feats_sweep"
    n, S = cfg.n_agents, cfg.fan_in
    nx, ny, ids, ids_dev, last = _sweep_grid(fn, cfg, frame_ids, n_frames, agent_id, xs, ys, frame_max)
    G = n_frames * ny * nx
    n_other = cfg.num_nodes - 1 - n
    N.expect_shape(Xa, (G * n, Fp), "Xa")
    if n_other > 0:
        N.expect_shape(Xo, (G * n_other, Fp), "Xo")
    N.expect_shape(efeat, (G * n, S, 4), "efeat")
    N.expect_shape(emask, (G * n, S), "emask")
    N.expect_shape(goal, (cfg.n_goals, cfg.state_dim), "goal")
    cast = _sweep_record(fn, cfg, agent, agent_st, obst, hits, hits_st, ray_cos, ray_sin, last, hits_out, G)
    if ids is not None:
        ids_dev = torch.from_numpy(ids.astype(np.int32)).to(agent.device)
    null = C.c_void_p(0)
    rc = N.lib().dgppo_graph_feats_sweep(
        C.byref(cfg), C.c_void_p(agent.data_ptr()), C.c_int64(agent_st), _p(goal, "goal"),
        _p(obst, "obst") if cfg.n_obs > 0 else null, C.c_void_p(hits.data_ptr()) if cast else null, C.c_int64(hits_st),
        _p(ray_cos, "ray_cos") if cast else null, _p(ray_sin, "ray_sin") if cast else null,
        _p(ids_dev, "frame_ids", torch.int32), C.c_int32(n_frames), C.c_int32(int(agent_id)), _p(xs, "xs"), C.c_int32(nx),
        _p(ys, "ys"), C.c_int32(ny), _p(Xa, "Xa"), _p(Xo, "Xo") if n_other > 0 else null, _p(efeat, "efeat"), _p(emask, "emask"),
        _p(hits_out, "hits_out") if (cast and hits_out is not None) else null, C.c_int32(Fp), N.stream_ptr())
    N.check(rc, "dgppo_graph_feats_sweep")


def cost_sweep(cfg: N.EnvCfg, agent, agent_st, obst, hits, hits_st, ray_cos, ray_sin, frame_ids, n_frames, agent_id, xs, ys,
               cost, hits_out=None, frame_max=None):
    fn = "cost_sweep"
    if cfg.is_vmas:
        raise ValueError(f"{fn}: VMASReverseTransport has no sweep entry point")
    if hits_out is not None and not (cfg.is_lidar and cfg.n_obs > 0):
        raise ValueError(f"{fn}: hits_out needs a LiDAR kind with obstacles (nothing is cast here)")
    nx, ny, ids, ids_dev, last = _sweep_grid(fn, cfg, frame_ids, n_frames, agent_id, xs, ys, frame_max)
    G = n_frames * ny * nx
    N.expect_shape(cost, (G, cfg.n_agents, cfg.n_cost), "cost")
    cast = _sweep_record(fn, cfg, agent, agent_st, obst, hits, hits_st, ray_cos, ray_sin, last, hits_out, G)
    if ids is not None:
        ids_dev = torch.from_numpy(ids.astype(np.int32)).to(agent.device)
    null = C.c_void_p(0)
    rc = N.lib().dgppo_cost_sweep(
        C.byref(cfg), C.c_void_p(agent.data_ptr()), C.c_int64(agent_st), _p(obst, "obst") if cfg.n_obs > 0 else null,
        C.c_void_p(hits.data_ptr()) if cast else null, C.c_int64(hits_st), _p(ray_cos, "ray_cos") if cast else null,
        _p(ray_sin, "ray_sin") if cast else null, _p(ids_dev, "frame_ids", torch.int32), C.c_int32(n_frames),
        C.c_int32(int(agent_id)), _p(xs, "xs"), C.c_int32(nx), _p(ys, "ys"), C.c_int32(ny), _p(cost, "cost"),
        _p(hits_out, "hits_out") if cast and hits_out is not None else null, N.stream_ptr())
    N.check(rc, "dgppo_cost_sweep")


ACTION_SWEEP_TILE = 64


def graph_feats_action_sweep(cfg: N.EnvCfg, agent, agent_st, goal, obst, hits, hits_st, frame_ids, n_frames, agent_id, us, vs,
                             Xa, Xo, efeat, emask, Fp, frame_max=None):
    fn = "graph_feats_action_sweep"
    if cfg.is_vmas:
        raise ValueError(f"{fn}: VMASReverseTransport has no sweep entry point")
    n, S = cfg.n_agents, cfg.fan_in
    nu, nv, ids, ids_dev, last = _sweep_grid(fn, cfg, frame_ids, n_frames, agent_id, us, vs, frame_max, ("us", "vs"))
    G = n_frames * nv * nu
    n_other = cfg.num_nodes - 1 - n
    N.expect_shape(Xa, (G * n, Fp), "Xa")
    if n_other > 0:
        N.expect_shape(Xo, (G * n_other, Fp), "Xo")
    N.expect_shape(efeat, (G * n, S, 4), "efeat")
    N.expect_shape(emask, (G * n, S), "emask")
    N.expect_shape(goal, (cfg.n_goals, cfg.state_dim), "goal")
    _check_strided(fn, "agent", agent, 0, agent_st, (n, cfg.state_dim), None, 1, last + 2)
    rec_hits = cfg.is_lidar and cfg.n_obs > 0
    discs = (not cfg.is_lidar) and cfg.n_obs > 0
    if rec_hits:
        if hits is None:
            raise ValueError(f"{fn}: hits is required for a LiDAR kind with obstacles")
        _check_strided(fn, "hits", hits, 0, hits_st, (n, cfg.top_k, 2), None, 1, last + 2)
    if discs:
        if obst is None:
            raise ValueError(f"{fn}: obst is required when n_obs > 0")
        N.expect_shape(obst, (cfg.n_obs, cfg.obst_stride), "obst")
    if ids is not None:
        ids_dev = torch.from_numpy(ids.astype(np.int32)).to(agent.device)
    null = C.c_void_p(0)
    rc = N.lib().dgppo_graph_feats_action_sweep(
        C.byref(cfg), C.c_void_p(agent.data_ptr()), C.c_int64(agent_st), _p(goal, "goal"), _p(obst, "obst") if discs else null,
        C.c_void_p(hits.data_ptr()) if rec_hits else null, C.c_int64(hits_st), _p(ids_dev, "frame_ids", torch.int32),
        C.c_int32(n_frames), C.c_int32(int(agent_id)), _p(us, "us"), C.c_int32(nu), _p(vs, "vs"), C.c_int32(nv), _p(Xa, "Xa"),
        _p(Xo, "Xo") if n_other > 0 else null, _p(efeat, "efeat"), _p(emask, "emask"), C.c_int32(Fp), N.stream_ptr())
    N.check(rc, "dgppo_graph_feats_action_sweep")


def _dense(fn: str, name: str, t_, shape, dtype=torch.float32):
    if not (torch.is_tensor(t_) and t_.is_cuda and t_.dtype == dtype and t_.is_contiguous()):
        raise ValueError(f"{fn}: {name} must be a contiguous {dtype} CUDA tensor")
    if tuple(t_.shape) != tuple(shape):
        raise ValueError(f"{fn}: {name}: expected shape {tuple(shape)}, got {tuple(t_.shape)}")


def _shield_axes(fn: str, us, vs):
    for name, t_ in (("us", us), ("vs", vs)):
        if not (torch.is_tensor(t_) and t_.is_cuda and t_.dtype == torch.float32 and t_.ndim == 1 and t_.is_contiguous()):
            raise ValueError(f"{fn}: {name} must be a dense 1-D float32 CUDA tensor (sweep_axis)")
        if t_.numel() == 0:
            raise ValueError(f"{fn}: {name} is empty")
    return int(us.numel()), int(vs.numel())


def graph_feats_team_action_sweep(cfg: N.EnvCfg, agent, next_agent, goal, obst, next_hits, a_pol, us, vs, Xa, Xo, efeat, emask,
                                  Fp):
    fn = "graph_feats_team_action_sweep"
    if cfg.is_vmas:
        raise ValueError(f"{fn}: VMASReverseTransport has no sweep entry point")
    n, S, sd = cfg.n_agents, cfg.fan_in, cfg.state_dim
    nu, nv = _shield_axes(fn, us, vs)
    if not (torch.is_tensor(agent) and agent.ndim == 3):
        raise ValueError(f"{fn}: agent must be a [B, n, state_dim] tensor")
    B = int(agent.shape[0])
    G = B * n * (1 + nu * nv)
    n_other = cfg.num_nodes - 1 - n
    _dense(fn, "agent", agent, (B, n, sd))
    _dense(fn, "next_agent", next_agent, (B, n, sd))
    _dense(fn, "goal", goal, (B, cfg.n_goals, sd))
    _dense(fn, "a_pol", a_pol, (B, n, 2))
    _dense(fn, "Xa", Xa, (G * n, Fp))
    if n_other > 0:
        _dense(fn, "Xo", Xo, (G * n_other, Fp))
    _dense(fn, "efeat", efeat, (G * n, S, 4))
    _dense(fn, "emask", emask, (G * n, S))
    rec_hits = cfg.is_lidar and cfg.n_obs > 0
    discs = (not cfg.is_lidar) and cfg.n_obs > 0
    if rec_hits:
        if next_hits is None:
            raise ValueError(f"{fn}: next_hits is required for a LiDAR kind with obstacles")
        _dense(fn, "next_hits", next_hits, (B, n, cfg.top_k, 2))
    if discs:
        if obst is None:
            raise ValueError(f"{fn}: obst is required when n_obs > 0")
        _dense(fn, "obst", obst, (B, cfg.n_obs, cfg.obst_stride))
    null = C.c_void_p(0)
    rc = N.lib().dgppo_graph_feats_team_action_sweep(
        C.byref(cfg), _p(agent, "agent"), _p(next_agent, "next_agent"), _p(goal, "goal"), _p(obst, "obst") if discs else null,
        _p(next_hits, "next_hits") if rec_hits else null, _p(a_pol, "a_pol"), C.c_int32(B), _p(us, "us"), C.c_int32(nu),
        _p(vs, "vs"), C.c_int32(nv), _p(Xa, "Xa"), _p(Xo, "Xo") if n_other > 0 else null, _p(efeat, "efeat"), _p(emask, "emask"),
        C.c_int32(Fp), N.stream_ptr())
    N.check(rc, "dgppo_graph_feats_team_action_sweep")


def shield_select(Vh_next, Vh_t, a_pol, us, vs, dt: float, alpha: float, margin: float, action, index, flag, h=None):
    fn = "shield_select"
    nu, nv = _shield_axes(fn, us, vs)
    P = 1 + nu * nv
    if not (torch.is_tensor(Vh_t) and Vh_t.ndim == 3):
        raise ValueError(f"{fn}: Vh_t must be a [E, n, n_cost] tensor")
    E, n, nh = (int(s) for s in Vh_t.shape)
    if n < 1 or nh < 1:
        raise ValueError(f"{fn}: Vh_t must have at least one agent and one cost component")
    for name, v in (("dt", dt), ("alpha", alpha), ("margin", margin)):
        if not np.isfinite(float(v)):
            raise ValueError(f"{fn}: {name} must be finite")
    if not float(dt) > 0.0:
        raise ValueError(f"{fn}: dt must be > 0")
    _dense(fn, "Vh_t", Vh_t, (E, n, nh))
    _dense(fn, "Vh_next", Vh_next, (E * n * P * n, nh))
    _dense(fn, "a_pol", a_pol, (E, n, 2))
    _dense(fn, "action", action, (E, n, 2))
    _dense(fn, "index", index, (E, n), torch.int32)
    _dense(fn, "flag", flag, (E, n), torch.int32)
    if h is not None:
        _dense(fn, "h", h, (E, n, P))
    rc = N.lib().dgppo_shield_select(
        _p(Vh_next, "Vh_next"), _p(Vh_t, "Vh_t"), _p(a_pol, "a_pol"), C.c_int32(E), C.c_int32(n), C.c_int32(nh), _p(us, "us"),
        C.c_int32(nu), _p(vs, "vs"), C.c_int32(nv), C.c_float(float(dt)), C.c_float(float(alpha)), C.c_float(float(margin)),
        _p(action, "action"), _p(index, "index", torch.int32), _p(flag, "flag", torch.int32), _p(h, "h"), N.stream_ptr())
    N.check(rc, "dgppo_shield_select")


def _shaped(fn: str, operands):
    for name, t_, shape, *_ in operands:
        if not torch.is_tensor(t_) or tuple(t_.shape) != tuple(shape):
            got = tuple(t_.shape) if torch.is_tensor(t_) else type(t_).__name__
            raise ValueError(f"{fn}: {name}: expected shape {tuple(shape)}, got {got}")
    for name, t_, shape, *dtype in operands:
        _dense(fn, name, t_, shape, *dtype)


def lookahead_select(cost_tm, a_pol, us, vs, margin: float, action, index, flag, s=None):
    fn = "lookahead_select"
    if not (torch.is_tensor(a_pol) and a_pol.ndim == 3 and a_pol.shape[2] == 2 and a_pol.shape[1] >= 1):
        raise ValueError(f"{fn}: a_pol must be a [E, n, 2] tensor")
    E, n = int(a_pol.shape[0]), int(a_pol.shape[1])
    if not (torch.is_tensor(cost_tm) and cost_tm.ndim == 4):
        raise ValueError(f"{fn}: cost_tm must be a [K, G, n, nh] tensor")
    K_, nh = int(cost_tm.shape[0]), int(cost_tm.shape[3])
    if K_ < 1:
        raise ValueError(f"{fn}: K must be >= 1")
    if not 1 <= nh <= 3:
        raise ValueError(f"{fn}: n_cost {nh} outside [1, 3]")
    for name, t_ in (("us", us), ("vs", vs)):
        if not (torch.is_tensor(t_) and t_.ndim == 1 and t_.numel() > 0):
            raise ValueError(f"{fn}: {name} must be a non-empty 1-D tensor (sweep_axis)")
    P = 1 + int(us.numel()) * int(vs.numel())
    G = E * n * P
    if tuple(cost_tm.shape[1:]) != (G, n, nh):
        raise ValueError(f"{fn}: cost_tm: expected shape (K, {G}, {n}, {nh}), got {tuple(cost_tm.shape)}")
    if np.isnan(float(margin)):
        raise ValueError(f"{fn}: margin must not be NaN")
    _shaped(fn, [("a_pol", a_pol, (E, n, 2)), ("cost_tm[0]", cost_tm[0], (G, n, nh)), ("action", action, (E, n, 2)),
                 ("index", index, (E, n), torch.int32), ("flag", flag, (E, n), torch.int32)]
            + ([("s", s, (E, n, P))] if s is not None else []))
    nu, nv = _shield_axes(fn, us, vs)
    cost_st = int(cost_tm.stride(0)) if K_ > 1 else G * n * nh
    if cost_st < G * n * nh:
        raise ValueError(f"{fn}: the steps of cost_tm overlap (stride {cost_st} < {G * n * nh})")
    rc = N.lib().dgppo_lookahead_select(
        _p(cost_tm[0], "cost"), cost_st, K_, E, n, nh, _p(a_pol, "a_pol"), _p(us, "us"), nu, _p(vs, "vs"), nv, float(margin),
        _p(action, "action"), _p(index, "index", torch.int32), _p(flag, "flag", torch.int32), _p(s, "s"), N.stream_ptr())
    N.check(rc, "dgppo_lookahead_select")


def vmas_graph_feats(cfg: N.EnvCfg, agent, agent_se, agent_st, body, body_se, body_st, scene, env_ids, n_env, n_time,
                     Xa, efeat, emask, Fp):
    G = n_env * n_time
    n = cfg.n_agents
    N.expect_shape(Xa, (G * n, Fp), "Xa")
    N.expect_shape(efeat, (G * n, n, 4), "efeat")
    N.expect_shape(emask, (G * n, n), "emask")
    _check_strided("vmas_graph_feats", "agent", agent, agent_se, agent_st, (n, 4), env_ids, n_env, n_time)
    _check_strided("vmas_graph_feats", "body", body, body_se, body_st, (4,), env_ids, n_env, n_time)
    rc = N.lib().dgppo_vmas_graph_feats(
        C.byref(cfg), C.c_void_p(agent.data_ptr()), C.c_int64(agent_se), C.c_int64(agent_st), C.c_void_p(body.data_ptr()),
        C.c_int64(body_se), C.c_int64(body_st), _p(scene, "scene"), _p(env_ids, "env_ids", torch.int32), C.c_int32(n_env),
        C.c_int32(n_time), _p(Xa, "Xa"), _p(efeat, "efeat"), _p(emask, "emask"), C.c_int32(Fp), N.stream_ptr())
    N.check(rc, "dgppo_vmas_graph_feats")
# ... 435 lines not shown
```

Before: 4.653 million.

## Skip unused GAE columns and edge features in value-only feature passes

GAE now accepts a null Qh or Ql and skips the corresponding column computation, loads and reductions. The training path requests only the Ql of the stochastic rollout and only the Qh of the deterministic one. Graph features can also be built without the edge-feature tensor when the Vh network's lean first layer never reads it, so that write is templated out. This reduces memory traffic and compute in the prepass and minibatch feature construction, at the cost of extra null-handling paths.

```diff
diff --git a/dgppo_amd/csrc/gae.hip b/dgppo_amd/csrc/gae.hip
--- a/dgppo_amd/csrc/gae.hip
+++ b/dgppo_amd/csrc/gae.hip
@@ -19,34 +19,36 @@
   float* rowL = rowH + (T + 1) * AH;
   float* hcur = rowL + (T + 1);
   float* hdis = hcur + AH;
+  const bool doL = a.Ql != nullptr;
+  const int AHc = a.Qh != nullptr ? AH : 0;
   const float* costs = a.costs + (size_t)b * T * AH;
   const float* Vh = a.Vh + (size_t)b * (T + 1) * AH;
   const float* Vl = a.Vl + (size_t)b * (T + 1);
   const float* rew = a.rewards + (size_t)b * T;
-  for (int i = tid; i < (T + 1) * AH; i += nt) rowH[i] = 0.0f;
+  for (int i = tid; i < (T + 1) * AHc; i += nt) rowH[i] = 0.0f;
   for (int i = tid; i < T + 1; i += nt) rowL[i] = 0.0f;
   __syncthreads();
-  for (int i = tid; i < AH; i += nt) rowH[i] = Vh[(size_t)T * AH + i];
-  if (tid == 0) rowL[0] = Vl[T];
+  for (int i = tid; i < AHc; i += nt) rowH[i] = Vh[(size_t)T * AH + i];
+  if (tid == 0 && doL) rowL[0] = Vl[T];
   __syncthreads();
   for (int ii = 0; ii < T; ++ii) {
     const int t = T - 1 - ii;
-    for (int i = tid; i < AH; i += nt) hcur[i] = costs[(size_t)t * AH + i];
-    __syncthreads();
-    for (int ag = tid; ag < n; ag += nt) {
+    for (int i = tid; i < AHc; i += nt) hcur[i] = costs[(size_t)t * AH + i];
+    __syncthreads();
+    for (int ag = tid; ag < (AHc ? n : 0); ag += nt) {
       float m = hcur[ag * nh];
       for (int h = 1; h < nh; ++h) m = nanmax(m, hcur[ag * nh + h]);
       for (int h = 0; h < nh; ++h) hdis[ag * nh + h] = a.one_minus_gamma * m;
     }
     __syncthreads();
-    const float l = -rew[t];
-    for (int idx = tid; idx < (ii + 1) * AH; idx += nt) {
+    const float l = doL ? -rew[t] : 0.0f;
+    for (int idx = tid; idx < (ii + 1) * AHc; idx += nt) {
       const int c = idx % AH;
       rowH[idx] = nanmax(hcur[c], hdis[c] + a.gamma * rowH[idx]);
     }
-    for (int j = tid; j <= ii; j += nt) rowL[j] = l + a.gamma * rowL[j];
-    __syncthreads();
-    for (int c = tid; c < AH + 1; c += nt) {
+    for (int j = tid; j <= (doL ? ii : -1); j += nt) rowL[j] = l + a.gamma * rowL[j];
+    __syncthreads();
+    for (int c = tid + (AHc ? 0 : AH); c < AH + (doL ? 1 : 0); c += nt) {
       float acc = 0.0f;
       if (c < AH) {
         for (int j = 0; j <= ii; ++j) {
@@ -63,8 +65,8 @@
       }
     }
     __syncthreads();
-    for (int i = tid; i < AH; i += nt) rowH[(ii + 1) * AH + i] = Vh[(size_t)t * AH + i];
-    if (tid == 0) rowL[ii + 1] = Vl[t];
+    for (int i = tid; i < AHc; i += nt) rowH[(ii + 1) * AH + i] = Vh[(size_t)t * AH + i];
+    if (tid == 0 && doL) rowL[ii + 1] = Vl[t];
     __syncthreads();
   }
 }
@@ -90,31 +92,36 @@
   float* s_part = s_rew + T;
   const float* costs = a.costs + (size_t)b * T * AH;
   const float* Vh = a.Vh + (size_t)b * (T + 1) * AH;
-  for (int i = tid; i < T * AH; i += 256) s_cost[i] = costs[i];
-  for (int i = tid; i < (T + 1) * AH; i += 256) s_Vh[i] = Vh[i];
-  for (int i = tid; i < T + 1; i += 256) s_Vl[i] = a.Vl[(size_t)b * (T + 1) + i];
-  for (int i = tid; i < T; i += 256) s_rew[i] = a.rewards[(size_t)b * T + i];
+  const bool doH = a.Qh != nullptr, doL = a.Ql != nullptr;
+  if (doH) {
+    for (int i = tid; i < T * AH; i += 256) s_cost[i] = costs[i];
+    for (int i = tid; i < (T + 1) * AH; i += 256) s_Vh[i] = Vh[i];
+  }
+  if (doL) {
+    for (int i = tid; i < T + 1; i += 256) s_Vl[i] = a.Vl[(size_t)b * (T + 1) + i];
+    for (int i = tid; i < T; i += 256) s_rew[i] = a.rewards[(size_t)b * T + i];
+  }
   __syncthreads();
   const int j = tid;
   float row[AHP];
   float rowl = 0.0f;
 #pragma unroll
-  for (int c = 0; c < AHP; ++c) row[c] = (j == 0 && c < AH) ? s_Vh[T * AH + c] : 0.0f;
-  if (j == 0) rowl = s_Vl[T];
+  for (int c = 0; c < AHP; ++c) row[c] = (doH && j == 0 && c < AH) ? s_Vh[T * AH + c] : 0.0f;
+  if (doL && j == 0) rowl = s_Vl[T];
   for (int ii = 0; ii < T; ++ii) {
     const int t = T - 1 - ii;
     const bool act = j <= ii;
     float contrib[AHP];
     float cl = 0.0f;
     const float cj = (j == 0) ? a.lam_pow[ii] : ((j <= ii) ? a.lam_pow[ii - j] * a.one_minus_lam : 0.0f);
-    if (act) {
+    if (act && doL) {
       const float l = -s_rew[t];
       rowl = l + a.gamma * rowl;
       cl = cj * rowl;
     }
 #pragma unroll
     for (int ag = 0; ag < AHP; ag += 1) {
-      if (ag < AH) {
+      if (doH && ag < AH) {
         const int agent = ag / nh;
         float m = s_cost[t * AH + agent * nh];
         for (int h = 1; h < nh; ++h) m = nanmax(m, s_cost[t * AH + agent * nh + h]);
@@ -124,23 +131,29 @@
         contrib[ag] = 0.0f;
       }
     }
-#pragma unroll
-    for (int c = 0; c < AHP; ++c) contrib[c] = gae_row16_sum(contrib[c]);
-    cl = gae_row16_sum(cl);
+    if (doH) {
+#pragma unroll
+      for (int c = 0; c < AHP; ++c) contrib[c] = gae_row16_sum(contrib[c]);
+    }
+    if (doL) cl = gae_row16_sum(cl);
     float* part = s_part + (ii & 1) * 16 * (AHP + 1);
     if ((lane & 15) == 0) {
       float* dst = part + (tid >> 4) * (AHP + 1);
-#pragma unroll
-      for (int c = 0; c < AHP; ++c) dst[c] = contrib[c];
-      dst[AHP] = cl;
+      if (doH) {
+#pragma unroll
+        for (int c = 0; c < AHP; ++c) dst[c] = contrib[c];
+      }
+      if (doL) dst[AHP] = cl;
     }
     if (j == ii + 1) {
-#pragma unroll
-      for (int c = 0; c < AHP; ++c) row[c] = (c < AH) ? s_Vh[t * AH + c] : 0.0f;
-      rowl = s_Vl[t];
-    }
-    __syncthreads();
-    if (tid <= AH) {
+      if (doH) {
+#pragma unroll
+        for (int c = 0; c < AHP; ++c) row[c] = (c < AH) ? s_Vh[t * AH + c] : 0.0f;
+      }
+      if (doL) rowl = s_Vl[t];
+    }
+    __syncthreads();
+    if (tid < AH ? doH : (tid == AH && doL)) {
       const int c = (tid < AH) ? tid : AHP;
       float q = 0.0f;
 #pragma unroll
@@ -160,12 +173,13 @@
 
 template <int RPG, int NRG>
 __global__ void __launch_bounds__(256) gae_cols_kernel(GaeArgs a) {
-  const int T = a.T, AH = a.AH, nh = a.nh, C = AH + 1;
+  const int T = a.T, AH = a.AH, nh = a.nh;
+  const int c0 = a.Qh != nullptr ? 0 : AH, C = AH + (a.Ql != nullptr ? 1 : 0) - c0;
   const int rg = threadIdx.x % NRG;
   const long item = (long)blockIdx.x * (256 / NRG) + threadIdx.x / NRG;
   const bool valid = item < (long)a.B * C;
   const long it = valid ? item : 0;
-  const int b = (int)(it / C), col = (int)(it - (long)b * C);
+  const int b = (int)(it / C), col = c0 + (int)(it - (long)b * C);
   const bool is_l = (col == AH);
   const int agent = is_l ? 0 : col / nh;
   const float* costs = a.costs + (size_t)b * T * AH + agent * nh;
@@ -240,7 +254,7 @@
 
 template <int RPG, int NRG>
 static void launch_gae_cols(const GaeArgs& a, hipStream_t st) {
-  const long items = (long)a.B * (a.AH + 1);
+  const long items = (long)a.B * ((a.Qh ? a.AH : 0) + (a.Ql ? 1 : 0));
   const int per_block = 256 / NRG;
   hipLaunchKernelGGL((gae_cols_kernel<RPG, NRG>), dim3((unsigned)((items + per_block - 1) / per_block)), dim3(256), 0, st, a);
 }
@@ -250,7 +264,8 @@
                              float* Ql, int32_t B, int32_t T, int32_t n, int32_t nh, void* stream) {
   DGPPO_REQUIRE(B >= 0 && T >= 1 && n >= 1 && nh >= 1, "gae: bad sizes");
   if (B == 0) return 0;
-  DGPPO_REQUIRE(costs && rewards && Vh && Vl && lam_pow && Qh && Ql, "gae: NULL operand");
+  DGPPO_REQUIRE(Qh || Ql, "gae: Qh and Ql are both NULL: nothing to compute");
+  DGPPO_REQUIRE(lam_pow && (!Qh || (costs && Vh)) && (!Ql || (rewards && Vl)), "gae: NULL operand");
   GaeArgs a{costs, rewards, Vh, Vl, lam_pow, Qh, Ql, B, T, n * nh, n, nh, gamma, one_minus_gamma, one_minus_lam};
   if (T <= 256 && one_minus_lam <= 0.5f && one_minus_lam >= 0.0f) {
     hipStream_t st = (hipStream_t)stream;
diff --git a/dgppo_amd/csrc/graph_feats.hip b/dgppo_amd/csrc/graph_feats.hip
--- a/dgppo_amd/csrc/graph_feats.hip
+++ b/dgppo_amd/csrc/graph_feats.hip
@@ -38,7 +38,7 @@
   }
 }
 
-template <int SD>
+template <int SD, bool EF>
 __global__ void __launch_bounds__(256) graph_feats_kernel(FeatArgs a) {
   extern __shared__ float sm[];
   const dgppo_env_cfg& c = a.cfg;
@@ -148,7 +148,7 @@
             mask = dist_rn(__fsub_rn(xi[0], xo[0]), __fsub_rn(xi[1], xo[1])) < c.obs_mask_radius;
           }
         }
-        reinterpret_cast<float4*>(a.efeat)[(size_t)g * nE + idx] = f;
+        if constexpr (EF) reinterpret_cast<float4*>(a.efeat)[(size_t)g * nE + idx] = f;
         if (!a.vecM) a.emask[(size_t)g * nE + idx] = mask ? 1.0f : 0.0f;
       }
       if (a.vecM) {
@@ -193,7 +193,7 @@
   DGPPO_REFUSE_VMAS(cfg, "dgppo_graph_feats", "dgppo_vmas_graph_feats");
   DGPPO_REQUIRE(n_env >= 0 && n_time >= 0, "graph_feats: negative counts");
   if (n_env == 0 || n_time == 0) return 0;
-  DGPPO_REQUIRE(agent && goal && Xa && efeat && emask, "graph_feats: NULL operand");
+  DGPPO_REQUIRE(agent && goal && Xa && emask, "graph_feats: NULL operand");
   DGPPO_REQUIRE(Fp >= cfg->node_dim && Fp <= 32, "graph_feats: Fp must be in [node_dim, 32]");
   FeatArgs a;
   a.cfg = *cfg; a.t = make_topo(*cfg);
@@ -219,12 +219,13 @@
   int wpb = 4;
   while (wpb > 1 && rec * wpb > 65536) wpb >>= 1;
   const long G = (long)n_env * n_time;
-  const void* fn = SD == 5 ? reinterpret_cast<const void*>(&graph_feats_kernel<5>) : reinterpret_cast<const void*>(&graph_feats_kernel<4>);
+  void (*kern)(FeatArgs) = SD == 5 ? (efeat ? graph_feats_kernel<5, true> : graph_feats_kernel<5, false>)
+                                   : (efeat ? graph_feats_kernel<4, true> : graph_feats_kernel<4, false>);
+  const void* fn = reinterpret_cast<const void*>(kern);
   const int cap = feats_grid_cap(fn, wpb, rec * wpb);
   const long wgs = (G + wpb - 1) / wpb;
   const dim3 grid((unsigned)(wgs < cap ? wgs : cap)), block(64 * wpb);
-  if (SD == 5) hipLaunchKernelGGL(graph_feats_kernel<5>, grid, block, rec * wpb, (hipStream_t)stream, a);
-  else hipLaunchKernelGGL(graph_feats_kernel<4>, grid, block, rec * wpb, (hipStream_t)stream, a);
+  hipLaunchKernelGGL(kern, grid, block, rec * wpb, (hipStream_t)stream, a);
   DGPPO_LAUNCH_CHECK();
   return 0;
 }
diff --git a/dgppo_amd/engine.py b/dgppo_amd/engine.py
--- a/dgppo_amd/engine.py
+++ b/dgppo_amd/engine.py
@@ -111,7 +111,7 @@
     def __init__(self, cfg: N.EnvCfg, hyper: Hyper, device, T: int = 128,
                  allreduce: Optional[Callable[[torch.Tensor], None]] = None, world: int = 1, prepass_graphs: int = 1 << 20,
                  use_graphs: bool = False, multi_stream: bool = False, algo: str = "dgppo", rank: int = 0,
-                 fused_step: bool = True, lean_attn0: bool = True):
+                 fused_step: bool = True, lean_attn0: bool = True, vh_lean: bool = True):
         self.cfg, self.hp, self.device, self.T = cfg, hyper, device, T
         assert algo in ("dgppo", "informarl", "hcbfcrpo", "informarl_lagr"), algo
         self.algo = algo
@@ -120,6 +120,7 @@
         self._side_streams = None
         self.fused_step = bool(fused_step) and OE.act_step_feats_supported(cfg, nets.input_width(cfg), nets.H_HEADS)
         self.lean_attn0 = bool(lean_attn0)
+        self.vh_lean = bool(vh_lean)
         self._ro_cache: Dict[tuple, dict] = {}
         self._upd_graph: dict = {}
         self.n_cost = cfg.n_cost
@@ -225,8 +226,8 @@
         for net in self.nets.values():
             net.prepare()
 
-    def _feats(self, tag, st: OE.State, n_env, n_time=1, slots=1, env_ids=None):
-        f = nets.GraphFeats(self.cfg, n_env * n_time, self.arena, tag)
+    def _feats(self, tag, st: OE.State, n_env, n_time=1, slots=1, env_ids=None, efeat=True):
+        f = nets.GraphFeats(self.cfg, n_env * n_time, self.arena, tag, efeat=efeat)
         return f.compute_record(st.step, slots, st.env, env_ids, n_env, n_time)
 
     def _rollout_steps(self, ro: RolloutData, eps, B: int, stochastic: bool, start: int = 0):
@@ -327,10 +328,15 @@
         main.wait_stream(s1)
         return out[0], out[1]
 
-    def _block_feats(self, tag, ro: RolloutData, e0, Eb, t0, n_time, env_ids=None):
+    def _vh_only_feats_need_efeat(self) -> bool:
+        if not (self.vh_lean and self.algo == "dgppo") or self.cfg.is_vmas:
+            return True
+        return self.Vh.kind != "Vh" or self.Vh.reads_efeat(self.cfg.state_dim == 4)
+
+    def _block_feats(self, tag, ro: RolloutData, e0, Eb, t0, n_time, env_ids=None, efeat=True):
         envs = slice(e0, None) if env_ids is None else slice(None)
         st = OE.State({k: v[envs, t0] for k, v in ro.step.items()}, {k: v[envs] for k, v in ro.env.items()})
-        return self._feats(tag, st, Eb, n_time, self.T + 1, env_ids)
+        return self._feats(tag, st, Eb, n_time, self.T + 1, env_ids, efeat)
 
     def _vh_carry(self, ro: RolloutData, e0: int, Eb: int) -> torch.Tensor:
         return ro.rnn_states[e0:e0 + Eb][..., :nets.HID]
@@ -351,9 +357,10 @@
         Vl_buf = self.arena.get(f"tg.Vl.{kind}", B, T + 1) if want_Vl else None
         Vh_buf = self.arena.get(f"tg.Vh.{kind}", B, T + 1, n, nh) if want_Vh else None
         block = max(1, min(B, self.prepass_graphs // (T + 1)))
+        efeat = want_Vl or self._vh_only_feats_need_efeat()
         for e0 in range(0, B, block):
             Eb = min(block, B - e0)
-            feats = self._block_feats("pre", ro, e0, Eb, 0, T + 1)
+            feats = self._block_feats("pre", ro, e0, Eb, 0, T + 1, efeat=efeat)
             if want_Vl:
                 act = self.Vl.forward(feats, n_seq=Eb, T=T + 1, h0=None, tag="pre", train=False)
                 Vl_buf[e0:e0 + Eb].copy_(act["v"].view(Eb, T + 1))
@@ -925,17 +932,18 @@
                           grad_scale=1.0 / self.world)
         net.prepare()
 
-    def targets(self, ro: RolloutData, det: RolloutData, step: int):
+    def targets(self, ro: RolloutData, det: RolloutData, step: int, all_columns: bool = True):
         cfg, T, B, hp = self.cfg, self.T, ro.B, self.hp
         n, nh = cfg.n_agents, self.n_cost
         Vl, Vh = self.values_prepass(ro, want_Vl=True)
         _, Vh_det = self.values_prepass(det, want_Vl=False)
         A = self.arena
-        Qh = A.get("tg.Qh", B, T, n, nh)
+        full = all_columns or not self.vh_lean
+        Qh = A.get("tg.Qh", B, T, n, nh) if full else None
         Ql = A.get("tg.Ql", B, T)
         OA.gae(ro.costs, ro.rewards, Vh, Vl, self.lam_pow, hp.gamma, hp.gae_lambda, Qh, Ql)
         Qh_det = A.get("tg.Qh_det", B, T, n, nh)
-        Ql_det = A.get("tg.Ql_det", B, T)
+        Ql_det = A.get("tg.Ql_det", B, T) if full else None
         OA.gae(det.costs, det.rewards, Vh_det, Vl, self.lam_pow, hp.gamma, hp.gae_lambda, Qh_det, Ql_det)
         adv = A.get("tg.adv", B, T, n)
         self.stats.zero_()
@@ -958,7 +966,7 @@
         C = T // hp.rnn_step
         tg = (self.targets_informarl(ro, step) if self.algo == "informarl" else
               self.targets_hcbfcrpo(ro, step) if self.algo == "hcbfcrpo" else
-              self.targets_lagr(ro, step) if lagr else self.targets(ro, det, step))
+              self.targets_lagr(ro, step) if lagr else self.targets(ro, det, step, all_columns=False))
         th.append(_time.perf_counter())
         perm = np.asarray(perm)
         assert perm.size == 0 or (0 <= int(perm.min()) and int(perm.max()) < B), "perm holds env ids outside [0, B)"
@@ -1000,7 +1008,7 @@
             feats = ctx["feats"] = self._block_feats("mb", ro, 0, Eb, 0, T, env_ids=mb_idx32)
             pairs = [(tg["Ql"], Ql_mb)]
             if self.algo == "dgppo":
-                feats_det = self._block_feats("mbd", det, 0, Eb, 0, T, env_ids=mb_idx32)
+                feats_det = self._block_feats("mbd", det, 0, Eb, 0, T, env_ids=mb_idx32, efeat=self._vh_only_feats_need_efeat())
                 full = None
                 if self.HC == H:
                     pairs.append((det.rnn_states, h0_det))
diff --git a/dgppo_amd/nets.py b/dgppo_amd/nets.py
--- a/dgppo_amd/nets.py
+++ b/dgppo_amd/nets.py
@@ -95,14 +95,14 @@
 
 class GraphFeats:
 
-    def __init__(self, cfg: N.EnvCfg, G: int, arena: Arena, tag: str):
+    def __init__(self, cfg: N.EnvCfg, G: int, arena: Arena, tag: str, efeat: bool = True):
         self.cfg, self.G = cfg, G
         n, S = cfg.n_agents, cfg.fan_in
         self.n_other = cfg.num_nodes - 1 - n
         self.Fp = input_width(cfg)
         self.Xa = arena.get(f"{tag}.Xa0", G * n, self.Fp)
         self.Xo = arena.get(f"{tag}.Xo0", max(G * self.n_other, 1), self.Fp)[:G * self.n_other]
-        self.efeat = arena.get(f"{tag}.efeat", G * n, S, 4)
+        self.efeat = arena.get(f"{tag}.efeat", G * n, S, 4) if efeat else None
         self.emask = arena.get(f"{tag}.emask", G * n, S)
         self.edges_from_rows = False
 
@@ -117,17 +117,23 @@
         cfg, n = self.cfg, self.cfg.n_agents
         se, st = slots, int(slots > 1)
         if cfg.is_vmas:
+            self._need_efeat("compute_vmas")
             return self.compute_vmas(step["agent"], se * n * 4, st * n * 4, step["body"], se * 4, st * 4, env["scene"], env_ids,
                                      n_env, n_time)
         ia, ih = n * cfg.state_dim, n * cfg.top_k * 2
         return self.compute(step["agent"], se * ia, st * ia, env["goal"], env.get("obst"), step.get("hits"), se * ih, st * ih,
                             env_ids, n_env, n_time)
 
+    def _need_efeat(self, who: str):
+        if self.efeat is None:
+            raise ValueError(f"{who}: these GraphFeats were built without efeat; only compute / compute_record serve them")
+
     def compute_sweep(self, step, env, frame_ids, n_frames, agent_id, xs, ys, ray_cos=None, ray_sin=None, hits_out=None,
                       frame_max=None):
         cfg, n = self.cfg, self.cfg.n_agents
         if cfg.is_vmas:
             raise ValueError("compute_sweep: VMASReverseTransport has no sweep entry point")
+        self._need_efeat("compute_sweep")
         K.graph_feats_sweep(cfg, step["agent"], n * cfg.state_dim, env["goal"], env.get("obst"), step.get("hits"),
                             n * cfg.top_k * 2, ray_cos, ray_sin, frame_ids, n_frames, agent_id, xs, ys, self.Xa,
                             self.Xo if self.n_other > 0 else None, self.efeat, self.emask, self.Fp, hits_out, frame_max)
@@ -138,6 +144,7 @@
         cfg, n = self.cfg, self.cfg.n_agents
         if cfg.is_vmas:
             raise ValueError("compute_action_sweep: VMASReverseTransport has no sweep entry point")
+        self._need_efeat("compute_action_sweep")
         K.graph_feats_action_sweep(cfg, step["agent"], n * cfg.state_dim, env["goal"], env.get("obst"), step.get("hits"),
                                    n * cfg.top_k * 2, frame_ids, n_frames, agent_id, us, vs, self.Xa,
                                    self.Xo if self.n_other > 0 else None, self.efeat, self.emask, self.Fp, frame_max)
@@ -147,6 +154,7 @@
     def compute_team_action_sweep(self, st, nst, a_pol, us, vs):
         if self.cfg.is_vmas:
             raise ValueError("compute_team_action_sweep: VMASReverseTransport has no sweep entry point")
+        self._need_efeat("compute_team_action_sweep")
         K.graph_feats_team_action_sweep(self.cfg, st.step["agent"], nst.step["agent"], st.env["goal"], st.env.get("obst"),
                                         nst.step.get("hits"), a_pol, us, vs, self.Xa, self.Xo if self.n_other > 0 else None,
                                         self.efeat, self.emask, self.Fp)
@@ -234,6 +242,16 @@
                     K.attn_xo_supported(self.cfg, fp1, H_HEADS, kp1))
         return getattr(self, key)
 
+    def reads_efeat(self, edges_from_rows: bool) -> bool:
+        return not (self.gnn_layers == 1 and self.lean_attn0 and edges_from_rows)
+
+    @staticmethod
+    def _efeat_of(feats: GraphFeats, l: int):
+        if feats.efeat is None:
+            raise ValueError(f"GNN layer {l} reads efeat, but these GraphFeats were built without it (efeat=False serves only "
+                             f"a lean first layer: lean_attn0 on features with edges_from_rows)")
+        return feats.efeat
+
     def zero_grads(self):
         self.grads.zero_()
 
@@ -244,6 +262,8 @@
         R = G * n
         Ro = G * feats.n_other
         act = {"feats": feats, "G": G, "n_seq": n_seq, "T": T}
+        if feats.efeat is None and self.reads_efeat(feats.edges_from_rows):
+            self._efeat_of(feats, 1 if (self.lean_attn0 and feats.edges_from_rows) else 0)
         Xa, Xo = feats.Xa, feats.Xo
         xo_fused = None
         for l, (f, fp, d, kp) in enumerate(self.dims):
@@ -255,13 +275,14 @@
                 K.dense_fwd(Xa, self.pp(f"gnn{l}.Mcat"), self.pp(f"gnn{l}.cvec"), qt)
             zcat = A.get(f"{tag}.zcat{l}", R, kp)
             lean = l == 0 and self.lean_attn0 and feats.edges_from_rows
+            efeat = None if lean else self._efeat_of(feats, l)
             attn = A.get(f"{tag}.attn{l}", R, cfg.fan_in, H_HEADS) if train and not lean else None
             if lean:
                 K.attn_fwd_rows(cfg, fp, H_HEADS, kp, qt, Xa, Xo if Ro > 0 else None, feats.emask, zcat, None, G)
             elif xo_fused is not None:
-                K.attn_fwd_xo(cfg, fp, H_HEADS, kp, qt, Xa, xo_fused[0], xo_fused[1], xo_fused[2], feats.efeat, feats.emask, zcat, attn, G)
+                K.attn_fwd_xo(cfg, fp, H_HEADS, kp, qt, Xa, xo_fused[0], xo_fused[1], xo_fused[2], efeat, feats.emask, zcat, attn, G)
             else:
-                K.attn_fwd(cfg, fp, H_HEADS, kp, qt, Xa, Xo if Ro > 0 else None, feats.efeat, feats.emask, zcat, attn, G)
+                K.attn_fwd(cfg, fp, H_HEADS, kp, qt, Xa, Xo if Ro > 0 else None, efeat, feats.emask, zcat, attn, G)
             act[f"xo_fused{l}"] = xo_fused
             xo_fused = None
             Xa_n = A.get(f"{tag}.Xa{l + 1}", R, d)
@@ -556,20 +577,21 @@
             dXo_l = A.get(f"{tag}.dXo{l}", Ro, fp) if (need_dx and Ro > 0) else None
             more_dXo = dXo_prev is not None and dXo_l is not None
             xf = act.get(f"xo_fused{l}")
+            efeat = None if act.get(f"lean{l}") else self._efeat_of(feats, l)
             if act.get(f"lean{l}"):
                 K.attn_bwd_rows(cfg, fp, H_HEADS, kp, dz, None, act[f"qt{l}"], feats.emask, act[f"Xa{l}"],
                                 act[f"Xo{l}"] if Ro > 0 else None, dqt, G)
             elif xf is not None and dXa_l is not None and not more_dXo:
                 ws = A.get(f"{tag}.xo_ws", K.attn_xo_workspace_floats(G), 1).view(-1)
                 K.attn_bwd_xo_dw(cfg, fp, H_HEADS, kp, dz, act[f"attn{l}"], act[f"qt{l}"], act[f"Xa{l}"], xf[0], xf[1], xf[2],
-                                 feats.efeat, dqt, dXa_l, self.pg(f"gnn{l - 1}.Wout")[:self.dims[l - 1][1]], self.g(f"gnn{l - 1}.bu"), ws, G)
+                                 efeat, dqt, dXa_l, self.pg(f"gnn{l - 1}.Wout")[:self.dims[l - 1][1]], self.g(f"gnn{l - 1}.bu"), ws, G)
                 dXo_l = None
             elif xf is not None:
                 K.attn_bwd_xo(cfg, fp, H_HEADS, kp, dz, act[f"attn{l}"], act[f"qt{l}"], act[f"Xa{l}"], xf[0], xf[1], xf[2],
-                              feats.efeat, dqt, dXa_l, dXo_l, G, relu_xo=(dXo_l is not None and not more_dXo))
+                              efeat, dqt, dXa_l, dXo_l, G, relu_xo=(dXo_l is not None and not more_dXo))
             else:
                 K.attn_bwd(cfg, fp, H_HEADS, kp, dz, act[f"attn{l}"], act[f"qt{l}"], act[f"Xa{l}"],
-                           act[f"Xo{l}"] if Ro > 0 else None, feats.efeat, dqt, dXa_l, dXo_l, G,
+                           act[f"Xo{l}"] if Ro > 0 else None, efeat, dqt, dXa_l, dXo_l, G,
                            relu_xo=(dXo_l is not None and not more_dXo))
             if need_dx:
                 K.dense_bwd_xw(act[f"Xa{l}"], dqt, self.pp(f"gnn{l}.Mcat"), dXa_l, self.pg(f"gnn{l}.Mcat"), self.pg(f"gnn{l}.cvec"),
diff --git a/dgppo_amd/ops_algo.py b/dgppo_amd/ops_algo.py
--- a/dgppo_amd/ops_algo.py
+++ b/dgppo_amd/ops_algo.py
@@ -13,13 +13,21 @@
 
 
 def gae(costs, rewards, Vh, Vl, lam_pow, gamma: float, gae_lambda: float, Qh, Ql):
-    B, T, n, nh = costs.shape
-    N.expect_shape(rewards, (B, T), "rewards")
-    N.expect_shape(Vh, (B, T + 1, n, nh), "Vh")
-    N.expect_shape(Vl, (B, T + 1), "Vl")
+    if Qh is None and Ql is None:
+        raise ValueError("gae: Qh and Ql are both None: nothing to compute")
+    if Qh is not None and (costs is None or Vh is None):
+        raise ValueError("gae: Qh needs costs and Vh")
+    if Ql is not None and (rewards is None or Vl is None):
+        raise ValueError("gae: Ql needs rewards and Vl")
+    if costs is not None:
+        B, T, n, nh = costs.shape
+    else:
+        (B, T), n, nh = rewards.shape, 1, 1
+    for t, shape, name in ((rewards, (B, T), "rewards"), (Vh, (B, T + 1, n, nh), "Vh"), (Vl, (B, T + 1), "Vl"),
+                           (Qh, (B, T, n, nh), "Qh"), (Ql, (B, T), "Ql")):
+        if t is not None and not (name == "Vh" and costs is None):
+            N.expect_shape(t, shape, name)
     N.expect_shape(lam_pow, (T + 1,), "lam_pow")
-    N.expect_shape(Qh, (B, T, n, nh), "Qh")
-    N.expect_shape(Ql, (B, T), "Ql")
     rc = N.lib().dgppo_gae(N.ptr(costs), N.ptr(rewards), N.ptr(Vh), N.ptr(Vl), N.ptr(lam_pow), C.c_float(gamma),
                            C.c_float(1 - gamma), C.c_float(1 - gae_lambda), N.ptr(Qh), N.ptr(Ql), B, T, n, nh,
                            N.stream_ptr())
diff --git a/dgppo_amd/ops_nn.py b/dgppo_amd/ops_nn.py
--- a/dgppo_amd/ops_nn.py
+++ b/dgppo_amd/ops_nn.py
@@ -253,7 +253,8 @@
     N.expect_shape(Xa, (G * n, Fp), "Xa")
     if n_other > 0:
         N.expect_shape(Xo, (G * n_other, Fp), "Xo")
-    N.expect_shape(efeat, (G * n, S, 4), "efeat")
+    if efeat is not None:
+        N.expect_shape(efeat, (G * n, S, 4), "efeat")
     N.expect_shape(emask, (G * n, S), "emask")
     _check_strided("graph_feats", "agent", agent, agent_se, agent_st, (n, cfg.state_dim), env_ids, n_env, n_time)
     if hits is not None:
```

New measurement: 4.672 million, median of 4. No clear change (+0.4%).
